# jason-huang03/SPH_Project

Hardware: AMD Instinct MI355X
Metric: particle-updates/sec (higher is better)
Workload: dtype f32

## Files before the change

### sph_project_amd/csrc/sph_api.hip

```cpp
#include "../../include/sph_hip.h"
#include "sph_common.hpp"
#include "sph_comm.hpp"

#include <math.h>
#include <stdarg.h>
#include <stdio.h>
#include <string.h>
#include <string>
#include <vector>
#include <stdlib.h>
#include <utility>
#include <array>
#include <algorithm>
#include "sph_voxel.hpp"
#include "sph_export.hpp"
#include "sph_devobj.hpp"

struct ProfSlot {
    bool on = false;
    int64_t launches = 0;
    double ms = 0.0;
    std::vector<std::pair<hipEvent_t, hipEvent_t>> pending;
};

struct SphHandle : ErrSink {
    SphParams prm = {};
    State st;
    const Launch *L = nullptr;
    int device = 0;
    int n = 0;
    bool n_exact = true;
    int n_fluid = 0;
    int n_nonfluid = 0;
    bool fluid_mass_seen = false, fluid_mass_uniform = true; float fluid_mass0 = 0.0f;
    bool any_rigid_object = false;
    int64_t steps = 0;
    int pbf_bank = 0;
    SphPbfParams pbf = {SPH_PBF_VARIANT_REFERENCE, 1, 50, 1e-3f, 1e-6f};
    SphPbfStats pbf_last = {SPH_PBF_VARIANT_REFERENCE, 0, 0.0f};
    int steps_to_follow = 0;
    bool whole_step = false;
    double total_time = 0.0;
    bool prepared = false;
    bool pose_dirty = false;
    int loop_hint[4] = {0, 0, 0, 0};
    struct LoopPub *loop_pub = nullptr;
    unsigned loop_seq = 0, stats_seq = 0;
    bool loop_flags_clean = false;
    int dev_cus = 256;
    bool pose_given = false;
    bool rigid_volume_done = false;
    bool sort_dirty = false;
    bool in_step = false;
    int n_mark = 0;
    int fresh_state = 0;
    RigidPose pose_h = {};
    RigidBodyDev rb_h[SPH_NOBJ] = {};
    int rb_cap[SPH_NOBJ] = {};
    bool rb_pose_stale = false;
    SphStats last = {};
    ProfSlot prof[SPH_K_COUNT_];
    std::vector<hipEvent_t> ev_pool;
    std::vector<void *> allocs;
    DevScalars *scal_h = nullptr;
    SlabComm comm;
    long long comm_n_global = 0;
    long long comm_nfluid_global = 0;
    int swap_axis = 0;
    int perm[3] = {0, 1, 2};
    int inv[3] = {0, 1, 2};
    float axial = 1.0f;
    int slab_axis = 2;
};

static inline int slab_layers_glob(const Consts &c) { return c.slab_axis == 0 ? c.nx_glob : c.nz_glob; }
static inline void slab_set_window(Consts &c, int z_lo, int z_hi) {
    const int glob = slab_layers_glob(c);
    const int off = z_lo > 0 ? z_lo - 1 : 0;
    const int top = z_hi < glob ? z_hi + 1 : glob;
    if (c.slab_axis == 0) { c.cx_off = off; c.nx = top - off; } else { c.cz_off = off; c.nz = top - off; }
    c.G = c.nx * c.ny * c.nz;
}

static bool set_axis_order(SphHandle *h, const char *order) {
    int p[3], seen = 0;
    for (int k = 0; k < 3; ++k) {
        const char ch = order ? order[k] : 0;
        p[k] = (ch == 'x' || ch == 'X') ? 0 : (ch == 'y' || ch == 'Y') ? 1 : (ch == 'z' || ch == 'Z') ? 2 : -1;
        if (p[k] < 0) return false;
        seen |= 1 << p[k];
    }
    if (seen != 7 || order[3]) return false;
    for (int k = 0; k < 3; ++k) { h->perm[k] = p[k]; h->inv[p[k]] = k; }
    const bool even = (p[0] == 0 && p[1] == 1) || (p[0] == 1 && p[1] == 2) || (p[0] == 2 && p[1] == 0);
    h->axial = even ? 1.0f : -1.0f;
    h->swap_axis = !(p[0] == 0 && p[1] == 1 && p[2] == 2);
    return true;
}

template <class T> static int dalloc(SphHandle *h, T **p, size_t count) {
    void *q = nullptr;
    if (count == 0) count = 1;
    HIPCHK(h, hipMalloc(&q, count * sizeof(T)));
    HIPCHK(h, hipMemset(q, 0, count * sizeof(T)));
    h->allocs.push_back(q);
    *p = (T *)q;
    return SPH_OK;
}

static float host_kernel_W(double hd, float r) {
    float res = 0.0f;
    float k = (float)(8.0 / M_PI);
    k /= (float)(hd * hd * hd);
    float q = r / (float)hd;
    if (q <= 1.0f) {
        if (q <= 0.5f) { float q2 = q * q; float q3 = q2 * q; res = k * (6.0f * q3 - 6.0f * q2 + 1.0f); }
        else res = k * 2.0f * powf(1.0f - q, 3.0f);
    }
    return res;
}

static void fill_consts(SphHandle *h) {
    const SphParams &p = h->prm;
    Consts &c = h->st.c;
    memset(&c, 0, sizeof(c));
    const int *ix = h->perm;
    c.nx = c.nx_glob = p.grid_num[ix[0]]; c.ny = p.grid_num[ix[1]]; c.nz = c.nz_glob = p.grid_num[ix[2]];
    c.cx_off = c.cz_off = 0;
    c.slab_axis = h->slab_axis;
    c.G = c.nx * c.ny * c.nz;
    const double hd = p.support_radius;
    c.grid_size = (float)hd;
    c.h = (float)hd;
    {
        float t = c.h * c.h;
        while (sqrtf(nextafterf(t, 0.0f)) >= c.h) t = nextafterf(t, 0.0f);
        while (sqrtf(t) < c.h) t = nextafterf(t, INFINITY);
        c.h2 = t;
    }
    c.inv_h = 1.0f / c.h;
    float k = (float)(8.0 / M_PI);
    c.kW = k / (float)(hd * hd * hd);
    c.kG = 6.0f * k / (float)(hd * hd * hd);
    c.W0 = host_kernel_W(hd, 0.0f);
    const float d = (float)(2.0 * p.particle_radius);
    c.Wd = host_kernel_W(hd, sqrtf(d * d + 0.0f + 0.0f));
    c.kGh = c.kG * c.inv_h;
    c.inv_h2 = c.inv_h * c.inv_h;
    c.Wd_poly = c.Wd / c.kW;
    const double dd = 2.0 * p.particle_radius;
    c.diameter2 = (float)(dd * dd);
    c.dt = (float)p.dt;
    c.inv_dt = 1.0f / c.dt;
    c.rho0 = (float)p.density_0;
    c.inv_rho0 = 1.0f / c.rho0;
    c.g_upper = (float)p.g_upper;
    c.up_axis = h->inv[1];
    c.gx = (float)p.gravity[ix[0]]; c.gy = (float)p.gravity[ix[1]]; c.gz = (float)p.gravity[ix[2]];
    c.st = (float)p.surface_tension;
    c.cv = (float)(2 * (3 + 2) * p.viscosity);
    c.cvb = (float)(2 * (3 + 2) * p.viscosity_b);
    c.visc_eps = (float)(0.01 * hd * hd);
    c.pad = (float)p.padding;
    c.hix = (float)(p.domain_size[ix[0]] - p.padding);
    c.hiy = (float)(p.domain_size[ix[1]] - p.padding);
    c.hiz = (float)(p.domain_size[ix[2]] - p.padding);
    c.thr_kappa = (float)1e-5 * c.dt;
    c.V0 = (float)p.V0;
    c.force_global = p.force_global;
    c.stat_bank = 0;
    c.run_grouping = 0;
    c.xcd_chunk = 0;
    c.ghosts = 0;
}

static void refresh_counts(SphHandle *h) {
    h->st.c.n = h->n;
    h->st.has_emitter = h->prm.g_upper < 9999.0;
    h->st.c.all_fluid = (h->n_nonfluid == 0 && !h->st.has_emitter && !(h->st.slab_active && h->any_rigid_object)) ? 1 : 0;
    h->st.c.ghosts = h->st.slab_active ? 1 : 0;
    h->st.c.run_grouping = (h->prm.fast_math && !h->st.slab_active && h->st.c.nz >= 40) ? 1 : 0;
    h->st.has_rigid = h->n_nonfluid > 0;
    h->st.uniform_mass = (h->st.c.all_fluid && h->fluid_mass_uniform && !h->st.slab_active && !getenv("SPH_NO_UNIFORM_MASS")) ? 1 : 0;
}

extern "C" const char *sph_last_error(SphHandle *h) { return last_error(h); }

extern "C" const char *sph_kernel_name(int k) {
    static const char *names[SPH_K_COUNT_] = {
        "hash_count", "scan", "scatter", "density", "non_pressure", "pressure_integrate", "rigid_volume",
        "dfsph_density_alpha", "dfsph_rho_adv", "dfsph_correct", "reduce", "pcisph_rho_star",
        "pcisph_pressure_accel", "cg_prepare", "cg_ap", "cg_vector", "misc", "halo", "wcsph_forces",
        "iisph_prepare", "iisph_dij_pj", "iisph_sum_i", "pbf_density_lambda", "pbf_fix_position", "pbf_update",
        "rigid_contact", "rigid_integrate", "rigid_contact_solve", "pbfc_density_lambda", "pbfc_delta"};
    return (k >= 0 && k < SPH_K_COUNT_) ? names[k] : "?";
}

static void slab_comm_destroy(SlabComm &c);
static int slab_settle(SphHandle *h);
static inline int slab_settle_if_needed(SphHandle *h) { return h->n_exact ? SPH_OK : slab_settle(h); }

extern "C" void sph_destroy(SphHandle *h) {
    if (!h) return;
    hipSetDevice(h->device);
    if (h->st.stream) hipStreamSynchronize(h->st.stream);
    slab_comm_destroy(h->comm);
    if (h->st.push.mirror) { hipHostFree(h->st.push.mirror); h->st.push.mirror = nullptr; }
    for (auto &s : h->prof) for (auto &pr : s.pending) { hipEventDestroy(pr.first); hipEventDestroy(pr.second); }
    for (auto e : h->ev_pool) hipEventDestroy(e);
    for (void *p : h->allocs) hipFree(p);
    if (h->scal_h) hipHostFree(h->scal_h);
    if (h->loop_pub) hipHostFree((void *)h->loop_pub);
    if (h->st.list_count_pinned) { hipHostFree((void *)h->st.list_count_pinned); h->st.list_count_pinned = nullptr; }
    if (h->st.list_count_event) { hipEventDestroy(h->st.list_count_event); h->st.list_count_event = nullptr; }
    if (h->st.stream) hipStreamDestroy(h->st.stream);
    delete h;
}

extern "C" int sph_create(const SphParams *params, SphHandle **out) {
    if (!params || !out) return fail(nullptr, SPH_ERR_INVALID, "sph_create: null argument");
    *out = nullptr;
    const SphParams &p = *params;
    if (p.particle_max_num < 0 || p.grid_num[0] <= 0 || p.grid_num[1] <= 0 || p.grid_num[2] <= 0 ||
        !(p.support_radius > 0) || !(p.dt > 0))
        return fail(nullptr, SPH_ERR_INVALID, "sph_create: invalid parameters");
    if ((double)p.grid_num[0] * p.grid_num[1] * p.grid_num[2] > 2.0e9)
        return fail(nullptr, SPH_ERR_INVALID, "sph_create: grid too large");
    if (p.particle_max_num > 0x0fffffff)
        return fail(nullptr, SPH_ERR_CAPACITY, "sph_create: particle_max_num %d exceeds 268435455 per GPU; shard the scene (sph_comm_set_slab)", p.particle_max_num);
    if (p.method < 0 || p.method > SPH_METHOD_PBF) return fail(nullptr, SPH_ERR_INVALID, "sph_create: unknown method %d", p.method);
    int dev = 0;
    { int rc = pick_device("sph_create", p.device, &dev); if (rc) return rc; }
    SphHandle *h = new SphHandle();
    h->prm = p;
    h->device = dev;
    { int cus = 0; if (hipDeviceGetAttribute(&cus, hipDeviceAttributeMultiprocessorCount, dev) == hipSuccess && cus > 0) h->dev_cus = cus; }
#define CHK_CREATE(call)                                                                   \
    do {                                                                                   \
        int rc_ = (call);                                                                  \
        if (rc_ != SPH_OK) { g_create_error = h->err; sph_destroy(h); return rc_; }        \
    } while (0)
#define HIP_CREATE(call)                                                                   \
    do {                                                                                   \
        hipError_t e_ = (call);                                                            \
        if (e_ != hipSuccess) {                                                            \
            fail(nullptr, SPH_ERR_HIP, "%s failed: %s", #call, hipGetErrorString(e_));     \
            sph_destroy(h);                                                                \
            return SPH_ERR_HIP;                                                            \
        }                                                                                  \
    } while (0)
    h->L = p.fast_math ? sph_launch_fast() : sph_launch_strict();
    State &s = h->st;
    HIP_CREATE(hipStreamCreateWithFlags(&s.stream, hipStreamNonBlocking));
    fill_consts(h);
    const size_t cap = (size_t)p.particle_max_num;
    s.cap = p.particle_max_num;
    for (int k = 0; k < 2; ++k) {
        CHK_CREATE(dalloc(h, &s.posv.b[k], cap)); CHK_CREATE(dalloc(h, &s.velm.b[k], cap));
        CHK_CREATE(dalloc(h, &s.meta.b[k], cap)); CHK_CREATE(dalloc(h, &s.pid.b[k], cap));
        CHK_CREATE(dalloc(h, &s.color.b[k], cap)); CHK_CREATE(dalloc(h, &s.rho.b[k], cap));
    }
    const size_t G = (size_t)s.c.G;
    CHK_CREATE(dalloc(h, &s.cell_count, G + SPH_NGRAVE + 1)); CHK_CREATE(dalloc(h, &s.cell_start, G + SPH_NGRAVE + 1));
    CHK_CREATE(dalloc(h, &s.cellid, cap)); CHK_CREATE(dalloc(h, &s.rank, cap)); CHK_CREATE(dalloc(h, &s.tmp_idx, 2 * cap));
    if (h->prm.deterministic && !getenv("SPH_NO_RUN_LISTS")) { CHK_CREATE(dalloc(h, &s.run_head, G + 1)); CHK_CREATE(dalloc(h, &s.run_rec, cap + G + 1)); CHK_CREATE(dalloc(h, &s.sort_inv, cap)); CHK_CREATE(dalloc(h, &s.color_home, cap)); s.color_home_ok = 1; }
    s.scan_blocks = (int)((G + SPH_NGRAVE + 2047) / 2048);
    if (s.scan_blocks < SPH_STAT_SLOTS / 256) s.scan_blocks = SPH_STAT_SLOTS / 256;
    CHK_CREATE(dalloc(h, &s.scan_tile_state, (size_t)s.scan_blocks + 1));
    CHK_CREATE(dalloc(h, &s.scan_partial, 2 * ((size_t)s.scan_blocks + 1) * 8));
    CHK_CREATE(dalloc(h, &s.rho_raw, cap)); CHK_CREATE(dalloc(h, &s.prs, cap)); CHK_CREATE(dalloc(h, &s.ptm, cap));
    CHK_CREATE(dalloc(h, &s.acc, cap));
    CHK_CREATE(dalloc(h, &s.nbr_mask, cap * 9 + 256)); CHK_CREATE(dalloc(h, &s.nbr_mask_hi, cap * 9 + 256));
    CHK_CREATE(dalloc(h, &s.blk_hdr, (cap + 255) / 256 * (20 + 256)));
    if (!getenv("SPH_NO_BLOCK_LIST")) {
        CHK_CREATE(dalloc(h, &s.blk_flag, (cap + 255) / 256)); CHK_CREATE(dalloc(h, &s.blk_list, (cap + 255) / 256)); CHK_CREATE(dalloc(h, &s.blk_count, 1));
    }
    CHK_CREATE(dalloc(h, &s.lane_perm, (cap + 255) / 256 * 256));
    if (p.method == SPH_METHOD_DFSPH) {
        CHK_CREATE(dalloc(h, &s.alpha, cap)); CHK_CREATE(dalloc(h, &s.kappa, cap)); CHK_CREATE(dalloc(h, &s.kappa_v, cap));
        CHK_CREATE(dalloc(h, &s.rho_star, cap)); CHK_CREATE(dalloc(h, &s.rho_deriv, cap)); CHK_CREATE(dalloc(h, &s.kr, cap));
        CHK_CREATE(dalloc(h, &s.kappa_next, cap)); CHK_CREATE(dalloc(h, &s.kappa_v_next, cap));
    }
    if (p.method == SPH_METHOD_PCISPH) {
        CHK_CREATE(dalloc(h, &s.pacc, cap)); CHK_CREATE(dalloc(h, &s.pvel, cap)); CHK_CREATE(dalloc(h, &s.ppos, cap));
        CHK_CREATE(dalloc(h, &s.rho_star, cap)); CHK_CREATE(dalloc(h, &s.acc_np, cap));
        s.np_acc_out = s.acc_np;
    }
    if (p.method == SPH_METHOD_IISPH) {
        CHK_CREATE(dalloc(h, &s.iisph_dii, cap)); CHK_CREATE(dalloc(h, &s.iisph_dij, cap)); CHK_CREATE(dalloc(h, &s.iisph_w, cap));
        CHK_CREATE(dalloc(h, &s.rho_star, cap));
    }
    if (p.method == SPH_METHOD_PBF) {
        CHK_CREATE(dalloc(h, &s.pbf_old, cap)); CHK_CREATE(dalloc(h, &s.pbf_pos, cap)); CHK_CREATE(dalloc(h, &s.pbf_lambda, cap));
        CHK_CREATE(dalloc(h, &s.pbf_recentred, 2));
        s.poly6 = 1;
    }
    if (p.viscosity_implicit) {
        CHK_CREATE(dalloc(h, &s.cg_p, cap)); CHK_CREATE(dalloc(h, &s.cg_Ap, cap)); CHK_CREATE(dalloc(h, &s.cg_x, cap));
        CHK_CREATE(dalloc(h, &s.cg_b, cap)); CHK_CREATE(dalloc(h, &s.cg_r, cap)); CHK_CREATE(dalloc(h, &s.cg_v0, cap));
        CHK_CREATE(dalloc(h, &s.cg_dinv, cap * 9));
        CHK_CREATE(dalloc(h, &s.cg_part, cap * 3));
        CHK_CREATE(dalloc(h, &s.cg_p2, cap));
    }
    s.red_blocks = (int)((cap + 255) / 256) + 1;
    CHK_CREATE(dalloc(h, &s.red_partial, (size_t)s.red_blocks * 8));
    CHK_CREATE(dalloc(h, &s.scal, 1)); CHK_CREATE(dalloc(h, &s.pose, 1));
    HIP_CREATE(hipHostMalloc((void **)&h->scal_h, sizeof(DevScalars), hipHostMallocDefault));
    { void *lp = nullptr; HIP_CREATE(hipHostMalloc(&lp, 128, hipHostMallocDefault)); memset(lp, 0, 128); h->loop_pub = (struct LoopPub *)lp; }
    { int *lc = nullptr; HIP_CREATE(hipHostMalloc((void **)&lc, 64, hipHostMallocDefault)); *lc = 0; s.list_count_pinned = lc; }
    HIP_CREATE(hipEventCreateWithFlags(&s.list_count_event, hipEventDisableTiming));
    memset(h->scal_h, 0, sizeof(DevScalars));
    for (int o = 0; o < SPH_NOBJ; ++o) { h->pose_h.rot[o][0] = h->pose_h.rot[o][4] = h->pose_h.rot[o][8] = 1.0f; }
    s.z_hi = slab_layers_glob(s.c);
    s.visc_rho_raw = (p.method == SPH_METHOD_WCSPH);
    refresh_counts(h);
    *out = h;
    return SPH_OK;
}

static int ensure_orig(SphHandle *h) {
    State &s = h->st;
    if (!s.orig.b[0]) {
        int rc = dalloc(h, &s.orig.b[0], (size_t)s.cap); if (rc) return rc;
        rc = dalloc(h, &s.orig.b[1], (size_t)s.cap); if (rc) return rc;
        HIPCHK(h, hipMemcpyAsync(s.orig.cur(), s.posv.cur(), sizeof(float4) * (size_t)h->n, hipMemcpyDeviceToDevice, s.stream));
    }
    s.has_dynamic_rigid = 1;
    return SPH_OK;
}

extern "C" int sph_append_particles(SphHandle *h, int object_id, int n, const float *pos, const float *vel,
                                    const float *density, const float *pressure, const int32_t *material,
                                    const int32_t *is_dynamic, const int32_t *color) {
    if (!h) return SPH_ERR_INVALID;
    if (n < 0 || object_id < -1 || object_id >= SPH_MAX_OBJECTS) return fail(h, SPH_ERR_INVALID, "append: bad object id / count");
    if (n == 0) return SPH_OK;
    if (!pos || !vel || !density || !material || !is_dynamic) return fail(h, SPH_ERR_INVALID, "append: null array");
    { int rc = slab_settle_if_needed(h); if (rc) return rc; }
    if (h->n + n > h->st.cap) return fail(h, SPH_ERR_CAPACITY, "append: %d + %d exceeds particle_max_num %d", h->n, n, h->st.cap);
    HIPCHK(h, hipSetDevice(h->device));
    State &s = h->st;
    const float V0 = (float)h->prm.V0;
    std::vector<float4> hp(n), hv(n), ho;
    std::vector<int> hm(n), hid(n);
    std::vector<unsigned> hc(n);
    std::vector<float> hr(n), hpr(n);
    bool any_dyn_rigid = false;
    int nfl = 0;
    const int ix0 = h->perm[0], ix1 = h->perm[1], ix2 = h->perm[2];
    for (int k = 0; k < n; ++k) {
        hp[k] = make_float4(pos[3 * k + ix0], pos[3 * k + ix1], pos[3 * k + ix2], V0);
        hv[k] = make_float4(vel[3 * k + ix0], vel[3 * k + ix1], vel[3 * k + ix2], V0 * density[k]);
        hm[k] = META_PACK(object_id, material[k], is_dynamic[k] ? 1 : 0);
        if (h->prepared && material[k] == SPH_MAT_RIGID) { hm[k] |= META_FRESH_BIT; h->fresh_state = 1; }
        hid[k] = h->n + k;
        unsigned r = color ? (unsigned)(color[3 * k] & 0xff) : 0, g = color ? (unsigned)(color[3 * k + 1] & 0xff) : 0,
                 b = color ? (unsigned)(color[3 * k + 2] & 0xff) : 0;
        hc[k] = r | (g << 8) | (b << 16);
        hr[k] = density[k];
        hpr[k] = pressure ? pressure[k] : 0.0f;
        if (material[k] == SPH_MAT_FLUID) {
            nfl++;
            if (!h->fluid_mass_seen) { h->fluid_mass_seen = true; h->fluid_mass0 = hv[k].w; }
            else if (hv[k].w != h->fluid_mass0) h->fluid_mass_uniform = false;
        }
        if (material[k] == SPH_MAT_RIGID && is_dynamic[k]) any_dyn_rigid = true;
    }
    if (any_dyn_rigid) { int rc = ensure_orig(h); if (rc) return rc; }
    HIPCHK(h, hipStreamSynchronize(s.stream));
    const size_t off = (size_t)h->n;
    HIPCHK(h, hipMemcpy(s.posv.cur() + off, hp.data(), sizeof(float4) * n, hipMemcpyHostToDevice));
    HIPCHK(h, hipMemcpy(s.velm.cur() + off, hv.data(), sizeof(float4) * n, hipMemcpyHostToDevice));
    HIPCHK(h, hipMemcpy(s.meta.cur() + off, hm.data(), sizeof(int) * n, hipMemcpyHostToDevice));
    HIPCHK(h, hipMemcpy(s.pid.cur() + off, hid.data(), sizeof(int) * n, hipMemcpyHostToDevice));
    HIPCHK(h, hipMemcpy(s.color.cur() + off, hc.data(), sizeof(unsigned) * n, hipMemcpyHostToDevice));
    if (s.color_home) HIPCHK(h, hipMemcpy(s.color_home + off, hc.data(), sizeof(unsigned) * n, hipMemcpyHostToDevice));
    HIPCHK(h, hipMemcpy(s.rho.cur() + off, hr.data(), sizeof(float) * n, hipMemcpyHostToDevice));
    HIPCHK(h, hipMemcpy(s.prs + off, hpr.data(), sizeof(float) * n, hipMemcpyHostToDevice));
    if (s.orig.cur()) HIPCHK(h, hipMemcpy(s.orig.cur() + off, hp.data(), sizeof(float4) * n, hipMemcpyHostToDevice));
    h->n += n;
    h->n_fluid += nfl;
    h->n_nonfluid += n - nfl;
    if (!h->prepared) h->rigid_volume_done = false;
    if (h->prepared) h->sort_dirty = true;
    s.masks_valid = 0;
    s.perm_n = -1; s.list_n = -1;
    refresh_counts(h);
    return SPH_OK;
}

static void colors_leave_home(SphHandle *h) { h->L->sorted_color(h->st); h->st.color_home_ok = 0; }

extern "C" int sph_set_appended_ids(SphHandle *h, int n, const int32_t *ids) {
// ... 255 lines not shown
    const int m = std::min(n, capacity);
    if (m == 0) return SPH_OK;
    std::vector<double> dev((size_t)m * SPH_CS_ROW);
    HIPCHK(h, hipMemcpyAsync(dev.data(), s.contact_rows, dev.size() * sizeof(double), hipMemcpyDeviceToHost, s.stream));
    HIPCHK(h, hipStreamSynchronize(s.stream));
    for (int r = 0; r < m; ++r)
        memcpy(rows + (size_t)r * SPH_CONTACT_ROW_VALUES, dev.data() + (size_t)r * SPH_CS_ROW, sizeof(double) * SPH_CONTACT_ROW_VALUES);
    return SPH_OK;
}

static void contact_to_scene(const SphHandle *h, const unsigned long long *dev, double *out) {
    const size_t row = SPH_CT_VALUES;
    for (int A = 0; A < SPH_NOBJ; ++A)
        for (int B = 0; B < SPH_CT_PARTNERS; ++B)
            for (int b = 0; b < SPH_CT_BINS; ++b) {
                const int bs = 2 * h->perm[b / 2] + (b & 1);
                const int Bs = B >= 20 ? 20 + (2 * h->perm[(B - 20) / 2] + ((B - 20) & 1)) : B;
                const long long *v = (const long long *)dev + ((size_t)(A * SPH_CT_PARTNERS + B) * SPH_CT_BINS + b) * row;
                double *o = out + ((size_t)(A * SPH_CT_PARTNERS + Bs) * SPH_CT_BINS + bs) * row;
                o[0] = (double)v[0];
                for (int a = 0; a < 3; ++a) {
                    o[1 + a] = (double)v[1 + h->inv[a]] / SPH_WRENCH_SCALE;
                    o[4 + a] = (double)v[4 + h->inv[a]] / SPH_WRENCH_SCALE;
                }
                o[7] = (double)(unsigned long long)v[7] / SPH_WRENCH_SCALE;
            }
}

extern "C" int sph_get_rigid_contacts(SphHandle *h, double *table, int reset) {
    if (!h || !table) return fail(h, SPH_ERR_INVALID, "get_rigid_contacts: null");
    State &s = h->st;
    const size_t words = (size_t)SPH_CT_KEYS * SPH_CT_VALUES;
    if (!s.contact_table) return fail(h, SPH_ERR_INVALID, "get_rigid_contacts: sph_set_rigid_contact was never enabled");
    HIPCHK(h, hipSetDevice(h->device));
    std::vector<unsigned long long> dev(words);
    HIPCHK(h, hipMemcpyAsync(dev.data(), s.contact_table, words * 8, hipMemcpyDeviceToHost, s.stream));
    HIPCHK(h, hipStreamSynchronize(s.stream));
    contact_to_scene(h, dev.data(), table);
    if (s.slab_active && h->comm.nranks > 1) {
        if (h->comm.nranks > 15) return fail(h, SPH_ERR_UNSUPPORTED, "get_rigid_contacts: more than 15 ranks");
        const int per = 12, nd = (SPH_CT_KEYS + per - 1) / per;
        std::vector<double> dig(nd, 0.0);
        for (int k = 0; k < SPH_CT_KEYS; ++k) if (table[(size_t)k * 8] > 0.0) dig[k / per] += (double)(1ll << (4 * (k % per)));
        for (int o = 0; o < nd; o += SHM_RED_MAX) { int rc = sph_comm_allreduce(h, dig.data() + o, std::min(SHM_RED_MAX, nd - o), 0); if (rc) return rc; }
        std::vector<int> keys;
        for (int k = 0; k < SPH_CT_KEYS; ++k) if (((long long)dig[k / per] >> (4 * (k % per))) & 15) keys.push_back(k);
        std::vector<double> sum(keys.size() * 7), mx(keys.size());
        for (size_t q = 0; q < keys.size(); ++q) {
            for (int v = 0; v < 7; ++v) sum[7 * q + v] = table[(size_t)keys[q] * 8 + v];
            mx[q] = table[(size_t)keys[q] * 8 + 7];
        }
        for (size_t o = 0; o < sum.size(); o += SHM_RED_MAX) { int rc = sph_comm_allreduce(h, sum.data() + o, (int)std::min((size_t)SHM_RED_MAX, sum.size() - o), 0); if (rc) return rc; }
        for (size_t o = 0; o < mx.size(); o += SHM_RED_MAX) { int rc = sph_comm_allreduce(h, mx.data() + o, (int)std::min((size_t)SHM_RED_MAX, mx.size() - o), 1); if (rc) return rc; }
        for (size_t q = 0; q < keys.size(); ++q) {
            for (int v = 0; v < 7; ++v) table[(size_t)keys[q] * 8 + v] = sum[7 * q + v];
            table[(size_t)keys[q] * 8 + 7] = mx[q];
        }
    }
    if (reset) HIPCHK(h, hipMemsetAsync(s.contact_table, 0, words * 8, s.stream));
    return SPH_OK;
}

extern "C" int sph_get_rigid_contact_pairs(SphHandle *h, int64_t *pairs) {
    if (!h || !pairs) return fail(h, SPH_ERR_INVALID, "get_rigid_contact_pairs: null");
    *pairs = 0;
    if (!h->st.contact_pairs) return SPH_OK;
    HIPCHK(h, hipSetDevice(h->device));
    unsigned long long r = 0;
    HIPCHK(h, hipMemcpyAsync(&r, h->st.contact_pairs, sizeof(r), hipMemcpyDeviceToHost, h->st.stream));
    HIPCHK(h, hipStreamSynchronize(h->st.stream));
    *pairs = (int64_t)r;
    return SPH_OK;
}

static hipEvent_t get_event(SphHandle *h) {
    if (!h->ev_pool.empty()) { hipEvent_t e = h->ev_pool.back(); h->ev_pool.pop_back(); return e; }
    hipEvent_t e;
    hipEventCreate(&e);
    return e;
}

static void prof_resolve(SphHandle *h) {
    hipStreamSynchronize(h->st.stream);
    for (auto &s : h->prof) {
        for (auto &pr : s.pending) {
            float ms = 0.0f;
            if (hipEventElapsedTime(&ms, pr.first, pr.second) == hipSuccess) { s.ms += ms; s.launches++; }
            h->ev_pool.push_back(pr.first); h->ev_pool.push_back(pr.second);
        }
        s.pending.clear();
    }
}

struct ProfScope {
    SphHandle *h; int k; hipEvent_t e1 = nullptr;
    ProfScope(SphHandle *h_, int k_) : h(h_), k(k_) {
        if (h->prof[k].on) {
            if (h->prof[k].pending.size() > 8192) prof_resolve(h);
            hipEvent_t e0 = get_event(h); e1 = get_event(h);
            hipEventRecord(e0, h->st.stream);
            h->prof[k].pending.push_back({e0, e1});
        }
    }
    ~ProfScope() { if (e1) hipEventRecord(e1, h->st.stream); }
};

extern "C" int sph_profile_enable(SphHandle *h, int kernel_id, int on) {
    if (!h || kernel_id >= SPH_K_COUNT_) return SPH_ERR_INVALID;
    for (int k = 0; k < SPH_K_COUNT_; ++k) if (kernel_id < 0 || kernel_id == k) h->prof[k].on = on != 0;
    return SPH_OK;
}
extern "C" int sph_profile_reset(SphHandle *h) {
    if (!h) return SPH_ERR_INVALID;
    hipSetDevice(h->device);
    prof_resolve(h);
    for (auto &s : h->prof) { s.launches = 0; s.ms = 0.0; }
    return SPH_OK;
}
extern "C" int sph_profile_read(SphHandle *h, int kernel_id, int64_t *launches, double *total_ms) {
    if (!h || kernel_id < 0 || kernel_id >= SPH_K_COUNT_) return SPH_ERR_INVALID;
    hipSetDevice(h->device);
    prof_resolve(h);
    if (launches) *launches = h->prof[kernel_id].launches;
    if (total_ms) *total_ms = h->prof[kernel_id].ms;
    return SPH_OK;
}

extern "C" int sph_device_info(SphHandle *h, char *name256, int *cu_count, int64_t *hbm_bytes) {
    if (!h) return SPH_ERR_INVALID;
    hipDeviceProp_t prop;
    HIPCHK(h, hipGetDeviceProperties(&prop, h->device));
    if (name256) { if (prop.name[0]) snprintf(name256, 256, "%s (%s)", prop.name, prop.gcnArchName); else snprintf(name256, 256, "%s, %d CUs", prop.gcnArchName, prop.multiProcessorCount); }
    if (cu_count) *cu_count = prop.multiProcessorCount;
    if (hbm_bytes) *hbm_bytes = (int64_t)prop.totalGlobalMem;
    return SPH_OK;
}

extern "C" int sph_measure_copy_rate(SphHandle *h, size_t bytes, int reps, double *gb_per_s) {
    if (!h || !gb_per_s || bytes < 4096 || reps < 1) return fail(h, SPH_ERR_INVALID, "measure_copy_rate: bad arguments");
    HIPCHK(h, hipSetDevice(h->device));
    void *a = nullptr, *b = nullptr;
    if (hipMalloc(&a, bytes) != hipSuccess || hipMalloc(&b, bytes) != hipSuccess) {
        if (a) hipFree(a);
        return fail(h, SPH_ERR_HIP, "measure_copy_rate: cannot allocate 2 x %zu bytes", bytes);
    }
    hipStream_t st = h->st.stream;
    hipEvent_t e0 = get_event(h), e1 = get_event(h);
    hipError_t e = hipMemsetAsync(a, 1, bytes, st);
    if (e == hipSuccess) e = hipMemcpyAsync(b, a, bytes, hipMemcpyDeviceToDevice, st);
    if (e == hipSuccess) e = hipEventRecord(e0, st);
    for (int k = 0; k < reps && e == hipSuccess; ++k) e = hipMemcpyAsync((k & 1) ? a : b, (k & 1) ? b : a, bytes, hipMemcpyDeviceToDevice, st);
    if (e == hipSuccess) e = hipEventRecord(e1, st);
    if (e == hipSuccess) e = hipStreamSynchronize(st);
    float ms = 0.0f;
    if (e == hipSuccess) e = hipEventElapsedTime(&ms, e0, e1);
    h->ev_pool.push_back(e0); h->ev_pool.push_back(e1);
    hipFree(a); hipFree(b);
    if (e != hipSuccess || !(ms > 0.0f)) return fail(h, SPH_ERR_HIP, "measure_copy_rate: %s", hipGetErrorString(e));
    *gb_per_s = 2.0 * (double)bytes * reps / ((double)ms * 1e-3) / 1e9;
    return SPH_OK;
}

static int check_async(SphHandle *h) {
    if (h->st.state_error) { const int se = h->st.state_error; h->st.state_error = 0; return fail(h, SPH_ERR_INVALID, "internal state error %d (bit 0: a sort was scanned without a histogram of its own; bit 1: a density launch could not move the arrays its sort left to it)", se); }
    hipError_t e = hipGetLastError();
    if (e != hipSuccess) return fail(h, SPH_ERR_HIP, "kernel launch failed: %s", hipGetErrorString(e));
    return SPH_OK;
}

static SortCarry ph_neighbor_search(SphHandle *h, bool rho_dead = false, bool density_next = false) {
    State &s = h->st;
    SortCarry carry;
    { ProfScope p(h, SPH_K_HASH_COUNT); h->L->hash_count(s); }
    { ProfScope p(h, SPH_K_SCAN); h->L->scan(s); }
    { ProfScope p(h, SPH_K_SCATTER); if (h->prm.deterministic) carry = h->L->scatter_stable(s, rho_dead, density_next && !getenv("SPH_NO_SORT_CARRY")); else h->L->scatter(s); }
    h->sort_dirty = false;
    return carry;
}

static void ph_sort_hashed(SphHandle *h) {
    State &s = h->st;
    { ProfScope p(h, SPH_K_SCAN); h->L->scan(s); }
    { ProfScope p(h, SPH_K_SCATTER); if (h->prm.deterministic) h->L->scatter_stable(s, false, false); else h->L->scatter(s); }
    h->sort_dirty = false;
}

static void ph_rigid_volume(SphHandle *h) {
    if (!h->st.has_rigid) return;
    bool force = false;
    if (h->fresh_state == 2) { h->L->clear_fresh(h->st); h->fresh_state = 0; force = true; }
    else if (h->fresh_state == 1 && h->prm.method != SPH_METHOD_DFSPH) h->fresh_state = 2;
    if (!force && h->rigid_volume_done && !h->st.has_dynamic_rigid) return;
    ProfScope p(h, SPH_K_RIGID_VOLUME);
    h->L->rigid_volume(h->st);
    h->rigid_volume_done = true;
}

static void step_begin(SphHandle *h) {
    State &s = h->st;
    s.c.stat_bank = (int)(h->steps & 1);
}

#include "sph_comm_api.hpp"
#include "sph_steps.hpp"

static int read_scalars(SphHandle *h) {
    { int rc = slab_settle_if_needed(h); if (rc) return rc; }
    if (h->loop_pub) {
        StatsPub *pub = (StatsPub *)((char *)h->loop_pub + 64);
        const unsigned want = ++h->stats_seq;
        const int bank_d = h->steps > 0 ? (int)((h->steps - 1) & 1) : 0;
        hipLaunchKernelGGL(k_publish_stats, dim3(1), dim3(256), 0, h->st.stream, h->st.scal, bank_d, pub, want);
        if (spin_for(h->st, &pub->seq, want)) {
            h->last.pair_interactions = (int64_t)pub->pairs;
            h->last.pair_evaluations = (int64_t)pub->evals;
            h->last.lds_fallback_blocks = (int64_t)pub->fallback;
            return SPH_OK;
        }
    }
    HIPCHK(h, hipMemcpyAsync(h->scal_h, h->st.scal, sizeof(DevScalars), hipMemcpyDeviceToHost, h->st.stream));
    HIPCHK(h, hipStreamSynchronize(h->st.stream));
    unsigned long long pairs = 0, evals = 0, fb = 0;
    const int bank = h->steps > 0 ? (int)((h->steps - 1) & 1) : 0;
    for (int k = 0; k < SPH_STAT_SLOTS; ++k) {
        pairs += h->scal_h->pairs[bank][k]; evals += h->scal_h->evals[bank][k];
        fb += h->scal_h->fallback[bank][k];
    }
    h->last.pair_interactions = (int64_t)pairs;
    h->last.pair_evaluations = (int64_t)evals;
    h->last.lds_fallback_blocks = (int64_t)fb;
    return SPH_OK;
}

static int finish_sync(SphHandle *h) {
    { int rc = slab_settle_if_needed(h); if (rc) return rc; }
    HIPCHK(h, hipStreamSynchronize(h->st.stream));
    return SPH_OK;
}

extern "C" int sph_prepare(SphHandle *h) {
    if (!h) return SPH_ERR_INVALID;
    HIPCHK(h, hipSetDevice(h->device));
    refresh_counts(h);
    State &s = h->st;
    if (s.slab_active && h->prm.method == SPH_METHOD_IISPH)
        return fail(h, SPH_ERR_UNSUPPORTED, "sph_prepare: IISPH runs on one GPU only (no sharded IISPH solve: sph_comm_set_slab)");
    if (s.slab_active && h->prm.method == SPH_METHOD_PBF)
        return fail(h, SPH_ERR_UNSUPPORTED, "sph_prepare: PBF runs on one GPU only (no sharded PBF step: sph_comm_set_slab)");
    if (h->prm.viscosity_implicit && h->prm.method == SPH_METHOD_PBF)
        return fail(h, SPH_ERR_UNSUPPORTED, "sph_prepare: PBF with implicit viscosity is not supported (its CG walks would need the spiky gradient)");
    int rc = pose_refresh(h); if (rc) return rc;
    rc = upload_pose(h); if (rc) return rc;
    { ProfScope p(h, SPH_K_MISC); h->L->prepare_emitter(s); h->L->renew_rigid(s); }
    h->pose_dirty = false;
    if (s.slab_active) {
        double n_own[2] = {(double)h->n, (double)h->n_fluid};
        rc = sph_comm_allreduce(h, n_own, 2, 0); if (rc) return rc;
        h->comm_n_global = (long long)n_own[0];
        h->comm_nfluid_global = (long long)n_own[1];
        double dyn_rigid[1] = {s.orig.cur() ? 1.0 : 0.0};
        rc = sph_comm_allreduce(h, dyn_rigid, 1, 1); if (rc) return rc;
        if (dyn_rigid[0] > 0.0 && !s.orig.cur()) { rc = ensure_orig(h); if (rc) return rc; }
        rc = slab_neighbor_search(h); if (rc) return rc;
    }
    else ph_neighbor_search(h);
    h->rigid_volume_done = false;
    ph_rigid_volume(h);
    if (s.slab_active && s.has_rigid) {
        rc = slab_neighbor_search(h); if (rc) return rc;
    }
    rc = method_prepare(h); if (rc) return rc;
    HIPCHK(h, hipMemsetAsync(s.scal, 0, sizeof(unsigned long long) * SPH_STAT_SLOTS, s.stream));
    HIPCHK(h, hipMemsetAsync((char *)s.scal + offsetof(DevScalars, evals), 0, sizeof(unsigned long long) * SPH_STAT_SLOTS, s.stream));
    HIPCHK(h, hipMemsetAsync((char *)s.scal + offsetof(DevScalars, fallback), 0, sizeof(unsigned long long) * SPH_STAT_SLOTS, s.stream));
    rc = check_async(h); if (rc) return rc;
    HIPCHK(h, hipStreamSynchronize(s.stream));
    h->prepared = true;
    return SPH_OK;
}

static void ph_rigid_integrate(SphHandle *h) {
    if (!h->st.rigid_int_on || h->st.rigid_int.nbodies <= 0) return;
    if (h->st.contact_solve_on) { ProfScope p(h, SPH_K_RIGID_CONTACT_SOLVE); h->L->rigid_contact_solve(h->st); }
    else { ProfScope p(h, SPH_K_RIGID_INTEGRATE); h->L->rigid_integrate(h->st); }
    h->pose_dirty = true;
    h->rb_pose_stale = true;
}

extern "C" int sph_rigid_integrate(SphHandle *h) {
    if (!h) return SPH_ERR_INVALID;
    if (!h->in_step) return fail(h, SPH_ERR_INVALID, "sph_rigid_integrate outside sph_step_begin / sph_step_end");
    if (!h->st.rigid_int_on) return fail(h, SPH_ERR_INVALID, "sph_rigid_integrate: sph_set_rigid_integrator is off");
    { int rc = rigid_int_supported(h, "sph_rigid_integrate"); if (rc) return rc; }
    HIPCHK(h, hipSetDevice(h->device));
    ph_rigid_integrate(h);
    return check_async(h);
}

static int step_first_half(SphHandle *h) {
    if (h->in_step) return fail(h, SPH_ERR_INVALID, "sph_step_begin: the previous step was not ended");
    step_begin(h);
    int rc;
    switch (h->prm.method) {
        case SPH_METHOD_WCSPH: rc = wcsph_step(h); break;
        case SPH_METHOD_DFSPH: rc = dfsph_step_begin(h); break;
        case SPH_METHOD_IISPH: rc = iisph_step(h); break;
        case SPH_METHOD_PBF:
            rc = h->pbf.variant == SPH_PBF_VARIANT_CONSISTENT ? pbfc_step(h) : pbf_step(h); break;
        default: rc = pcisph_step(h); break;
    }
    if (rc) return rc;
    if (h->st.contact_on) { ProfScope p(h, SPH_K_RIGID_CONTACT); h->L->rigid_contact(h->st); }
    h->n_mark = h->n;
    h->in_step = true;
    return SPH_OK;
}

static int step_second_half(SphHandle *h) {
    if (!h->in_step) return fail(h, SPH_ERR_INVALID, "sph_step_end without sph_step_begin");
    State &s = h->st;
    h->in_step = false;
    if (h->pose_dirty || h->fresh_state || h->prm.method != SPH_METHOD_WCSPH) { int rc = slab_settle_if_needed(h); if (rc) return rc; }
    if (h->pose_dirty) { ProfScope p(h, SPH_K_MISC); h->L->renew_rigid(s); h->pose_dirty = false; }
    if (h->n > h->n_mark) {
        ProfScope p(h, SPH_K_MISC);
        h->L->post_insert(s, h->n_mark, h->prm.method != SPH_METHOD_DFSPH);
    }
    if (h->prm.method == SPH_METHOD_DFSPH) {
        int rc = dfsph_step_end(h); if (rc) return rc;
        if (h->fresh_state == 1) { h->fresh_state = 2; ph_rigid_volume(h); }
    } else if (h->fresh_state == 2) {
        ph_rigid_volume(h);
    }
    h->total_time += (double)s.c.dt;
    h->steps++;
    return SPH_OK;
}

static int step_once(SphHandle *h) {
    h->whole_step = true;
    int rc = step_first_half(h);
    h->whole_step = false;
#ifdef SPH_TEST_HOOKS
    {
        static int fail_at = getenv("SPH_TEST_FAIL_STEP") ? atoi(getenv("SPH_TEST_FAIL_STEP")) : -1;
        if (!rc && fail_at >= 0 && h->steps == fail_at) { fail_at = -1; h->in_step = false; rc = fail(h, SPH_ERR_INVALID, "SPH_TEST_FAIL_STEP: injected failure"); }
    }
#endif
    if (!rc) ph_rigid_integrate(h);
    if (!rc) rc = step_second_half(h);
    if (rc && h->st.prehashed) { h->st.prehashed = 0; h->st.cell_count_clean = 0; h->st.hist_taken = 0; h->st.run_lists_filed = 0; }
    return rc;
}

extern "C" int sph_step_begin(SphHandle *h) {
    if (!h) return SPH_ERR_INVALID;
    if (!h->prepared) return fail(h, SPH_ERR_INVALID, "sph_step_begin before sph_prepare");
    HIPCHK(h, hipSetDevice(h->device));
    refresh_counts(h);
    int rc = step_first_half(h); if (rc) return rc;
    rc = slab_settle_if_needed(h); if (rc) return rc;
    h->n_mark = h->n;
    return check_async(h);
}

extern "C" int sph_step_end(SphHandle *h) {
    if (!h) return SPH_ERR_INVALID;
    HIPCHK(h, hipSetDevice(h->device));
    refresh_counts(h);
    int rc = step_second_half(h); if (rc) return rc;
    rc = check_async(h); if (rc) return rc;
    return finish_sync(h);
}

extern "C" int sph_step_async(SphHandle *h, int nsteps) {
    if (!h || nsteps < 0) return SPH_ERR_INVALID;
    if (!h->prepared) return fail(h, SPH_ERR_INVALID, "sph_step before sph_prepare");
    if (h->prm.method != SPH_METHOD_WCSPH && h->prm.method != SPH_METHOD_PBF && h->prm.fixed_iterations <= 0)
        return fail(h, SPH_ERR_UNSUPPORTED, "sph_step_async needs wcsph, pbf or fixed_iterations > 0");
    if (h->prm.method == SPH_METHOD_PBF && h->pbf.variant == SPH_PBF_VARIANT_CONSISTENT && h->prm.fixed_iterations <= 0)
        return fail(h, SPH_ERR_UNSUPPORTED, "sph_step_async: the consistent PBF variant needs fixed_iterations > 0 (its stop test reads back)");
    HIPCHK(h, hipSetDevice(h->device));
    refresh_counts(h);
    for (int k = 0; k < nsteps; ++k) {
        h->steps_to_follow = nsteps - 1 - k;
        int rc = step_once(h);
        h->steps_to_follow = 0;
        if (rc) return rc;
    }
    return check_async(h);
}

extern "C" int sph_synchronize(SphHandle *h) {
    if (!h) return SPH_ERR_INVALID;
    HIPCHK(h, hipSetDevice(h->device));
    if (!h->n_exact) return slab_settle(h);
    return loop_readback(h);
}

extern "C" int sph_step(SphHandle *h, int nsteps) {
    if (!h || nsteps < 0) return SPH_ERR_INVALID;
    if (!h->prepared) return fail(h, SPH_ERR_INVALID, "sph_step before sph_prepare");
    HIPCHK(h, hipSetDevice(h->device));
    refresh_counts(h);
    for (int k = 0; k < nsteps; ++k) { int rc = step_once(h); if (rc) return rc; }
    int rc = check_async(h); if (rc) return rc;
    return finish_sync(h);
}

extern "C" int sph_run_phase(SphHandle *h, int phase) {
    if (!h) return SPH_ERR_INVALID;
    HIPCHK(h, hipSetDevice(h->device));
    { int rc = slab_settle_if_needed(h); if (rc) return rc; }
    refresh_counts(h);
    State &s = h->st;
    switch (phase) {
        case SPH_PH_NEIGHBOR_SEARCH: ph_neighbor_search(h); break;
        case SPH_PH_RIGID_VOLUME: h->rigid_volume_done = false; ph_rigid_volume(h); break;
        case SPH_PH_DENSITY: { ProfScope p(h, SPH_K_DENSITY); h->L->density(s, h->prm.method == SPH_METHOD_WCSPH, {}); } break;
        case SPH_PH_NON_PRESSURE: { int rc = run_non_pressure(h); if (rc) return rc; } break;
        case SPH_PH_PRESSURE_INTEGRATE: { ProfScope p(h, SPH_K_PRESSURE_INTEGRATE); h->L->pressure_integrate(s); } break;
        case SPH_PH_RIGID_CONTACT: {
            if (!s.contact_on) return fail(h, SPH_ERR_INVALID, "SPH_PH_RIGID_CONTACT: sph_set_rigid_contact is off");
            HIPCHK(h, hipMemsetAsync(s.contact_part, 0, sizeof(float4) * (size_t)s.cap, s.stream));
            ProfScope p(h, SPH_K_RIGID_CONTACT); h->L->rigid_contact(s);
        } break;
        case SPH_PH_CG_PREPARE: case SPH_PH_CG_AP: case SPH_PH_CG_UPDATE_XR: case SPH_PH_CG_UPDATE_P: case SPH_PH_CG_END:
            { int rc = cg_run_phase(h, phase); if (rc) return rc; } break;
        default: { int rc = method_run_phase(h, phase); if (rc) return rc; }
    }
    int rc = check_async(h); if (rc) return rc;
    HIPCHK(h, hipStreamSynchronize(s.stream));
    return SPH_OK;
}

extern "C" int sph_particle_num(SphHandle *h) {
    if (!h) return SPH_ERR_INVALID;
    if (!h->n_exact) { hipSetDevice(h->device); const int rc = slab_settle(h); if (rc) return rc; }
    return h->n;
}
extern "C" int sph_fluid_particle_num(SphHandle *h) { return h ? h->n_fluid : SPH_ERR_INVALID; }

extern "C" int sph_get_stats(SphHandle *h, SphStats *out) {
    if (!h || !out) return SPH_ERR_INVALID;
    HIPCHK(h, hipSetDevice(h->device));
    int rc = read_scalars(h); if (rc) return rc;
    h->last.steps = h->steps;
    h->last.particle_num = h->n;
    h->last.fluid_particle_num = h->n_fluid;
    h->last.total_time = h->total_time;
    h->last.hash_launches = h->st.n_hash_launches;
    h->last.prehashed_sorts = h->st.n_prehashed_sorts;
    h->last.list_sorts = h->st.n_list_sorts;
    h->last.carried_sorts = h->st.n_carried_sorts;
    if (h->st.pbf_recentred) {
        unsigned long long r[2];
        HIPCHK(h, hipMemcpy(r, h->st.pbf_recentred, sizeof(r), hipMemcpyDeviceToHost));
        h->last.pbf_recentred = (int64_t)r[h->pbf_bank];
    }
    *out = h->last;
    return SPH_OK;
}

extern "C" int sph_get_cg_scalars(SphHandle *h, float *out) {
    if (!h || !out) return SPH_ERR_INVALID;
    if (!h->prm.viscosity_implicit) return fail(h, SPH_ERR_UNSUPPORTED, "sph_get_cg_scalars: no implicit viscosity on this handle");
    HIPCHK(h, hipSetDevice(h->device));
    State &s = h->st;
    HIPCHK(h, hipStreamSynchronize(s.stream));
    float red[8];
    HIPCHK(h, hipMemcpy(red, &s.scal->red[0], sizeof(red), hipMemcpyDeviceToHost));
    out[0] = red[4]; out[1] = red[5]; out[2] = red[3];
    return SPH_OK;
}

static const float4 *vec_field(SphHandle *h, int field) {
    State &s = h->st;
    switch (field) {
        case SPH_F_POSITION: case SPH_F_REST_VOLUME: return s.posv.cur();
        case SPH_F_VELOCITY: case SPH_F_MASS: return s.velm.cur();
        case SPH_F_ACCELERATION: return s.acc;
        case SPH_F_PRESSURE_ACCEL: return s.pacc;
        case SPH_F_PREDICTED_VEL: return s.pvel;
        case SPH_F_PREDICTED_POS: return h->pbf.variant == SPH_PBF_VARIANT_CONSISTENT ? s.pbf_old : s.ppos;
        case SPH_F_CG_X: return s.cg_x;
        case SPH_F_ORIG_POSITION: return s.orig.cur() ? s.orig.cur() : s.posv.cur();
        case SPH_F_IISPH_DII: case SPH_F_IISPH_AII: return s.iisph_dii;
        case SPH_F_IISPH_DIJ_PJ: case SPH_F_IISPH_SUM_I: return s.iisph_dij;
        case SPH_F_PBF_OLD_POSITION: return h->pbf.variant == SPH_PBF_VARIANT_CONSISTENT ? nullptr : s.pbf_old;
        case SPH_F_RIGID_CONTACT_DN: case SPH_F_RIGID_CONTACT_COUNT: return s.contact_part;
        case SPH_F_NON_PRESSURE_ACCEL: return s.acc_np;
        case SPH_F_CG_B: return s.cg_b;
        case SPH_F_CG_R: return s.cg_r;
        case SPH_F_CG_P: return s.cg_p;
        case SPH_F_CG_AP: return s.cg_Ap;
        case SPH_F_CG_V0: return s.cg_v0;
        default: return nullptr;
    }
}
static const float *scalar_field(SphHandle *h, int field) {
    State &s = h->st;
    switch (field) {
        case SPH_F_DENSITY: return s.rho.cur();
        case SPH_F_PRESSURE: return s.prs;
        case SPH_F_DFSPH_ALPHA: return s.alpha;
        case SPH_F_DFSPH_KAPPA: return s.kappa;
        case SPH_F_DFSPH_KAPPA_V: return s.kappa_v;
        case SPH_F_DENSITY_STAR: return s.rho_star;
        case SPH_F_DENSITY_DERIV: return s.rho_deriv;
        case SPH_F_DFSPH_KAPPA_NEXT: return s.kappa_next;
        case SPH_F_DFSPH_KAPPA_V_NEXT: return s.kappa_v_next;
        case SPH_F_DEBUG_CAPTURE: return s.rho_raw;
        case SPH_F_PBF_LAMBDA: return s.pbf_lambda;
        default: return nullptr;
    }
}

extern "C" int sph_download(SphHandle *h, int field, void *dst, size_t bytes) {
    if (!h || !dst) return SPH_ERR_INVALID;
    HIPCHK(h, hipSetDevice(h->device));
    { int rc = slab_settle_if_needed(h); if (rc) return rc; }
    State &s = h->st;
    const size_t n = (size_t)h->n;
    HIPCHK(h, hipStreamSynchronize(s.stream));
    const bool is_vec3 = field == SPH_F_POSITION || field == SPH_F_VELOCITY || field == SPH_F_ACCELERATION ||
                         field == SPH_F_PRESSURE_ACCEL || field == SPH_F_PREDICTED_VEL || field == SPH_F_PREDICTED_POS ||
                         field == SPH_F_CG_X || field == SPH_F_ORIG_POSITION || field == SPH_F_IISPH_DII || field == SPH_F_IISPH_DIJ_PJ ||
                         field == SPH_F_PBF_OLD_POSITION || field == SPH_F_RIGID_CONTACT_DN || field == SPH_F_NON_PRESSURE_ACCEL ||
                         (field >= SPH_F_CG_B && field <= SPH_F_CG_V0);
    if (is_vec3) {
        const float4 *src = vec_field(h, field);
        if (!src) return fail(h, SPH_ERR_UNSUPPORTED, "download: field %d not allocated for this method", field);
        if (bytes != n * 12) return fail(h, SPH_ERR_INVALID, "download: field %d needs %zu bytes, got %zu", field, n * 12, bytes);
        std::vector<float4> tmp(n);
        HIPCHK(h, hipMemcpy(tmp.data(), src, n * sizeof(float4), hipMemcpyDeviceToHost));
        float *d = (float *)dst;
        const int ix0 = h->inv[0], ix1 = h->inv[1], ix2 = h->inv[2];
        for (size_t i = 0; i < n; ++i) { const float v[3] = {tmp[i].x, tmp[i].y, tmp[i].z}; d[3 * i] = v[ix0]; d[3 * i + 1] = v[ix1]; d[3 * i + 2] = v[ix2]; }
        return SPH_OK;
    }
    if (field == SPH_F_CG_DINV) {
        if (!s.cg_dinv) return fail(h, SPH_ERR_UNSUPPORTED, "download: field %d not allocated for this method", field);
        if (bytes != n * 36) return fail(h, SPH_ERR_INVALID, "download: field %d needs %zu bytes, got %zu", field, n * 36, bytes);
        std::vector<float> tmp(n * 9);
        HIPCHK(h, hipMemcpy(tmp.data(), s.cg_dinv, n * 36, hipMemcpyDeviceToHost));
        float *d = (float *)dst;
        for (size_t i = 0; i < n; ++i)
            for (int a = 0; a < 3; ++a)
                for (int b = 0; b < 3; ++b) d[9 * i + 3 * a + b] = tmp[9 * i + 3 * h->inv[a] + h->inv[b]];
        return SPH_OK;
    }
    if (field == SPH_F_CG_AP_PARTS) {
        if (!s.cg_part) return fail(h, SPH_ERR_UNSUPPORTED, "download: field %d not allocated for this method", field);
        if (bytes != n * 36) return fail(h, SPH_ERR_INVALID, "download: field %d needs %zu bytes, got %zu", field, n * 36, bytes);
        std::vector<float4> tmp(n);
        float *d = (float *)dst;
        const int ix0 = h->inv[0], ix1 = h->inv[1], ix2 = h->inv[2];
        for (int g = 0; g < 3; ++g) {
            HIPCHK(h, hipMemcpy(tmp.data(), s.cg_part + (size_t)g * s.cap, n * sizeof(float4), hipMemcpyDeviceToHost));
            float *dg = d + (size_t)g * n * 3;
            for (size_t i = 0; i < n; ++i) { const float v[3] = {tmp[i].x, tmp[i].y, tmp[i].z}; dg[3 * i] = v[ix0]; dg[3 * i + 1] = v[ix1]; dg[3 * i + 2] = v[ix2]; }
        }
        return SPH_OK;
    }
    if (field == SPH_F_REST_VOLUME || field == SPH_F_MASS || field == SPH_F_IISPH_AII || field == SPH_F_IISPH_SUM_I ||
        field == SPH_F_RIGID_CONTACT_COUNT) {
        if (bytes != n * 4) return fail(h, SPH_ERR_INVALID, "download: size mismatch");
        const float4 *src = vec_field(h, field);
        if (!src) return fail(h, SPH_ERR_UNSUPPORTED, "download: field %d not allocated for this method", field);
        std::vector<float4> tmp(n);
        HIPCHK(h, hipMemcpy(tmp.data(), src, n * sizeof(float4), hipMemcpyDeviceToHost));
        float *d = (float *)dst;
        for (size_t i = 0; i < n; ++i) d[i] = tmp[i].w;
        return SPH_OK;
    }
    if (const float *src = scalar_field(h, field)) {
        if (bytes != n * 4) return fail(h, SPH_ERR_INVALID, "download: size mismatch");
        HIPCHK(h, hipMemcpy(dst, src, n * 4, hipMemcpyDeviceToHost));
        return SPH_OK;
    }
    if (field == SPH_F_MATERIAL || field == SPH_F_OBJECT_ID || field == SPH_F_IS_DYNAMIC || field == SPH_F_GHOST) {
        if (bytes != n * 4) return fail(h, SPH_ERR_INVALID, "download: size mismatch");
        std::vector<int> tmp(n);
        HIPCHK(h, hipMemcpy(tmp.data(), s.meta.cur(), n * 4, hipMemcpyDeviceToHost));
        int32_t *d = (int32_t *)dst;
        for (size_t i = 0; i < n; ++i)
            d[i] = field == SPH_F_MATERIAL ? META_MAT(tmp[i]) : field == SPH_F_OBJECT_ID ? META_OBJ(tmp[i]) :
                   field == SPH_F_GHOST ? META_GHOST(tmp[i]) : META_DYN(tmp[i]);
        return SPH_OK;
    }
    if (field == SPH_F_PARTICLE_ID) {
        if (bytes != n * 4) return fail(h, SPH_ERR_INVALID, "download: size mismatch");
        HIPCHK(h, hipMemcpy(dst, s.pid.cur(), n * 4, hipMemcpyDeviceToHost));
        return SPH_OK;
    }
    if (field == SPH_F_COLOR) {
        if (bytes != n * 12) return fail(h, SPH_ERR_INVALID, "download: size mismatch");
        const unsigned *col = h->L->sorted_color(s); HIPCHK(h, hipStreamSynchronize(s.stream));
        std::vector<unsigned> tmp(n);
        HIPCHK(h, hipMemcpy(tmp.data(), col, n * 4, hipMemcpyDeviceToHost));
        int32_t *d = (int32_t *)dst;
        for (size_t i = 0; i < n; ++i) { d[3 * i] = tmp[i] & 0xff; d[3 * i + 1] = (tmp[i] >> 8) & 0xff; d[3 * i + 2] = (tmp[i] >> 16) & 0xff; }
        return SPH_OK;
    }
    if (field == SPH_F_GRID_ID) {
        if (bytes != n * 4) return fail(h, SPH_ERR_INVALID, "download: size mismatch");
        std::vector<float4> tmp(n);
// ... 112 lines not shown
```

### sph_project_amd/csrc/sph_common.hpp

```cpp
#pragma once
#include <hip/hip_runtime.h>
#include <stdint.h>

#define SPH_NOBJ 20
#define SPH_IISPH_OMEGA 0.2f
#define SPH_IISPH_ETA 0.001
#define SPH_IISPH_MAX_ITER 20
#define SPH_PBF_LAMBDA_EPS 100.0f
#define SPH_PBF_CORR_K 0.001f
#define SPH_PBF_CORR_DQ 0.3f
#define SPH_PBF_ITERATIONS 5

#define META_OBJ(m) (((m) & 0xff) - 1)
#define META_MAT(m) (((m) >> 8) & 0x3)
#define META_DYN(m) (((m) >> 10) & 0x1)
#define META_PACK(obj, mat, dyn) ((((obj) + 1) & 0xff) | (((mat) & 0x3) << 8) | (((dyn) & 1) << 10))
#define META_GHOST(m) (((m) >> 11) & 0x1)
#define META_DEAD(m) (((m) >> 12) & 0x1)
#define META_FRESH(m) (((m) >> 13) & 0x1)
#define META_FRESH_BIT (1 << 13)
#define META_ACTIVE_FLUID(m) ((((m) >> 8) & 0xB) == 1)
#define META_SET_MAT(m, mat) (((m) & ~(0x3 << 8)) | (((mat) & 0x3) << 8))

struct Consts {
    int nx, ny, nz, G;
    int nx_glob, cx_off, nz_glob, cz_off, slab_axis;
    float grid_size;
    float h, h2, inv_h;
    float kW, kG;
    float kGh, Wd_poly;
    float inv_h2;
    float W0, Wd;
    float diameter2;
    float dt, inv_dt, rho0, inv_rho0, g_upper;
    int up_axis;
    float gx, gy, gz;
    float st;
    float cv, cvb, visc_eps;
    float pad, hix, hiy, hiz;
    float thr_kappa;
    float V0;
    float pcisph_k;
    int   n;
    int   all_fluid;
    int   force_global;
    int   ghosts;
    int   stat_bank;
    int   xcd_chunk;
    int   run_grouping;
    const int *n_dev;
};

__device__ __forceinline__ int live_n(const Consts &c) { return c.n_dev ? *c.n_dev : c.n; }

#define SPH_NGRAVE 64
#define HC(k) ((k) * 32)
#define HC_BANK 128
struct SlabDyn {
    int n_app;
    int n_live;
    int n_send[2];
    int n_recv[2];
    int dropped;
    int longest;
    int status;
    unsigned seq;
    int n_btiles;
    unsigned wseq;
};
struct HaloRecHdr {
    unsigned seq;
    int count, status, stride;
};
struct HaloCtl {
    HaloRecHdr rec[2];
    unsigned fld_seq;
    int pad[55];
};
static_assert(sizeof(HaloCtl) == 256, "HaloCtl layout");
#define SLAB_ST_SEND_OVERFLOW 1
#define SLAB_ST_PEER 2
#define SLAB_ST_STRIDE 4
#define SLAB_ST_CAPACITY 8
#define SLAB_ST_TIMEOUT 16
#define SLAB_ST_BOUND 32
// ... 214 lines not shown
#define PNG_SEG 4096
#define PNG_NCNT 14
#define PNG_SIDE 320
#define PNG_WSIDE 672
#define PNG_WINDOW 32768
#define PNG_FAR 4096
#define PNG_NONE 0xFFFFFFFFu
#define PNG_SORT_TILE 4096
#define PNG_ND 5
#define PNG_DIST_LIST {1, 2, 3, 4, 6}
#define PNG_CRC_PIECE 17
static_assert(256 * PNG_CRC_PIECE >= 4 + 2 + 5 + PNG_SEG, "the CRC pieces cover the longest chunk");
#define PNG_CRC_POLY 0xEDB88320u
__host__ __device__ static inline unsigned png_crc_mul(unsigned a, unsigned b) {
    unsigned p = 0u;
    for (int k = 0; k < 32; ++k) {
        if (a & (0x80000000u >> k)) p ^= b;
        b = (b >> 1) ^ (PNG_CRC_POLY & (0u - (b & 1u)));
    }
    return p;
}
struct PngDev {
    int W, H, filter;
    int stride, raw, nseg;
    const unsigned char *rgb;
    unsigned char *flt;
    int *len;
    unsigned *adler;
    unsigned long long *cnt;
    unsigned *sum;
    unsigned crc_pow[8];
    unsigned char *out;
    hipStream_t stream;
    unsigned char *side;
    unsigned *prev;
    unsigned *sort_key[2], *sort_pos[2];
    int *hist;
    int nsort;
};

struct TextDev {
    int kind;
    const unsigned *xyz;
    const unsigned *nrm;
    const int *tri;
    long long nv, nt;
    long long row0;
    int rows;
    int *len;
    int *scan_tmp;
    int *longest;
    unsigned char *out;
    hipStream_t stream;
};

template <class T> struct DBuf {
    T *b[2] = {nullptr, nullptr};
    int c = 0;
    T *cur() const { return b[c]; }
    T *alt() const { return b[1 - c]; }
    void flip() { c = 1 - c; }
};

struct State {
    Consts c = {};
    hipStream_t stream = nullptr;
    int cap = 0;
    DBuf<float4> posv, velm, orig;
    DBuf<int> meta, pid;
    DBuf<unsigned> color;
    DBuf<float> rho;
    int *cell_count = nullptr;
    int *cell_start = nullptr;
    int *cellid = nullptr, *rank = nullptr;
    unsigned long long *run_head = nullptr;
    int2 *run_rec = nullptr;
    unsigned sort_epoch = 0u;
    int run_lists_filed = 0;
    int *sort_inv = nullptr;
    long long n_list_sorts = 0;
    long long n_carried_sorts = 0;
    unsigned *color_home = nullptr;
    int color_home_ok = 0, color_stale = 0;
    int *tmp_idx = nullptr;
    int *scan_partial = nullptr;
    int scan_blocks = 0;
    int *scan_tile_state = nullptr;
    int scan_bank = 0;
    int skip_residual = 0;
    int tile_sums_ready = 0;
    int cell_count_clean = 1;
    int hist_taken = 0;
    int state_error = 0;
    float *rho_raw = nullptr, *prs = nullptr, *ptm = nullptr;
    float4 *acc = nullptr;
    float *alpha = nullptr, *kappa = nullptr, *kappa_v = nullptr, *rho_star = nullptr, *rho_deriv = nullptr;
    float *kappa_next = nullptr, *kappa_v_next = nullptr;
    float2 *kr = nullptr;
    float4 *pacc = nullptr, *pvel = nullptr, *ppos = nullptr, *acc_np = nullptr;
    float4 *iisph_dii = nullptr, *iisph_dij = nullptr, *iisph_w = nullptr;
    float4 *pbf_old = nullptr, *pbf_pos = nullptr; float *pbf_lambda = nullptr; unsigned long long *pbf_recentred = nullptr;
    int poly6 = 0;
    float pbf_eps = 1e-6f;
    int contact_on = 0;
    ContactArgs contact = {};
    unsigned long long *contact_table = nullptr, *contact_pairs = nullptr;
    float4 *contact_part = nullptr;
    int rigid_int_on = 0;
    RigidIntArgs rigid_int = {};
    RigidBodyDev *rigid_bodies = nullptr;
    int contact_solve_on = 0;
    ContactSolveArgs contact_solve = {};
    double *contact_rows = nullptr;
    int *contact_nrows = nullptr;
    float4 *cg_p = nullptr, *cg_Ap = nullptr, *cg_x = nullptr, *cg_b = nullptr, *cg_r = nullptr, *cg_v0 = nullptr;
    float4 *cg_p2 = nullptr;
    int cg_fused_loop = 0;
    float *cg_dinv = nullptr;
    float4 *cg_part = nullptr;
    int cg_nocombine = 0;
    int cg_split = 0;
    int cg_parity = 0;
    int cg_first = 1;
    float *red_partial = nullptr;
    int red_blocks = 0;
    DevScalars *scal = nullptr;
    RigidPose *pose = nullptr;
    int has_dynamic_rigid = 0;
    int has_rigid = 0;
    int *xidx[2] = {};
    int xcur = 0;
    int *halo_tab[8] = {};
    float4 *sendbuf[2] = {}, *recvbuf[2] = {};
    int *halo_counts = nullptr;
    SlabDyn *dyn = nullptr;
    SlabDyn *dyn_cur = nullptr;
    int tables_pending = 0;
    int async_counts = 0;
    struct PushState {
        int on = 0;
        char *inbox = nullptr;
        char *peer[2] = {};
        int rec_cap = 0;
        size_t rec_bytes = 0, fld_bytes = 0;
        unsigned rec_seq = 0, fld_seq = 0;
        long long timeout_ticks = 0;
        SlabDyn *mirror = nullptr;
    } push;
    int *tile_list[2] = {};
    int *tile_cnt = nullptr;
    unsigned char *tile_class = nullptr;
    int tile_plan_n = -1;
    int tile_bound_b = 0;
    HaloSend presend = {};
    HaloFieldSend fieldsend = {};
    int preclassified = 0;
    int prehashed = 0;
    long long n_hash_launches = 0, n_prehashed_sorts = 0;
    int halo_cap = 0;
    int halo_longest = 0;
    int slab_active = 0, z_lo = 0, z_hi = 0, has_down = 0, has_up = 0;
    unsigned *nbr_mask = nullptr;
    unsigned *nbr_mask_hi = nullptr;
    int masks_valid = 0;
    int uniform_mass = 0;
    const int *loop_flag = nullptr;
    int loop_slot = 0;
    int loop_kind = 0;
    float loop_denom = 1.0f; double loop_thr = 0.0;
    unsigned char *lane_perm = nullptr;
    int *blk_flag = nullptr, *blk_list = nullptr, *blk_count = nullptr;
    int list_n = -1;
    volatile int *list_count_pinned = nullptr;
    hipEvent_t list_count_event = nullptr;
    int list_count_known = -1;
    int last_pass_listed = 0;
    int *blk_hdr = nullptr;
    int perm_n = -1;
    int has_emitter = 0;
    int visc_rho_raw = 0;
    int skip_viscosity = 0;
    float4 *np_acc_out = nullptr;
};

struct SortCarry {
    const int *inv = nullptr;
    const float4 *velm_in = nullptr; float4 *velm_out = nullptr;
    const int *meta_in = nullptr; int *meta_out = nullptr;
    const int *pid_in = nullptr; int *pid_out = nullptr;
    int on = 0;
};
template <bool ON> struct SortCarryOf { SortCarry carry; };
template <> struct SortCarryOf<false> {};

struct DensityOpts {
    int tiles = 0;
    bool books_forces = false;
    SortCarry carry = {};
};
struct ForceOpts {
    bool booked_by_density = false;
    bool hash_next = false;
};

struct Launch {
    unsigned *(*sorted_color)(State &);
    void (*hash_count)(State &);
    void (*scan)(State &);
    void (*scatter)(State &);
    SortCarry (*scatter_stable)(State &, bool rho_dead, bool density_next);
    void (*density)(State &, int eos, DensityOpts o);
    void (*non_pressure)(State &, const float4 *visc_vel);
    void (*pressure_integrate)(State &);
    void (*wcsph_forces)(State &, ForceOpts o);
    void (*rigid_volume)(State &);
    void (*renew_rigid)(State &);
    void (*prepare_emitter)(State &);
    void (*post_insert)(State &, int first, int stale_volume);
    void (*clear_fresh)(State &);
    void (*dfsph_density_alpha)(State &);
    void (*dfsph_density_alpha_div)(State &);
    void (*dfsph_rho_adv)(State &, int mode);
    void (*dfsph_correct)(State &, int mode);
    void (*advect_boundary)(State &, bool hash_next);
    void (*pcisph_init)(State &);
    void (*pcisph_rho_star)(State &);
    void (*pcisph_pressure_accel)(State &);
    void (*pcisph_reduce_error)(State &);
    void (*iisph_prepare)(State &);
    void (*iisph_dij_pj)(State &);
    void (*iisph_sum_i)(State &);
    void (*pbf_predict)(State &);
    void (*pbf_density_lambda)(State &);
    void (*pbf_fix_position)(State &);
    void (*pbf_finish)(State &);
    void (*pbfc_predict)(State &);
    void (*pbfc_density_lambda)(State &, int reduce);
    void (*pbfc_delta)(State &, int reduce);
    void (*pbfc_finish)(State &);
    void (*rigid_contact)(State &);
    void (*rigid_integrate)(State &);
    void (*rigid_contact_solve)(State &);
    void (*halo_classify_pack)(State &, int n);
    void (*halo_unpack_append)(State &, int side, int count, int offset);
    void (*halo_build_tables)(State &);
    void (*halo_pack_fields)(State &, int side, int n_send, int n_recv);
    void (*halo_unpack_fields)(State &, int side, int n_recv, int n_send);
    void (*halo_pack_scalar)(State &, int side, int n_send, int n_recv, const float *src);
    void (*halo_unpack_scalar)(State &, int side, int n_recv, int n_send, float *dst);
    void (*halo_pack_vel)(State &, int side, int n_send, int n_recv, const float4 *arr);
    void (*halo_unpack_vel)(State &, int side, int n_recv, int n_send, float4 *arr);
    void (*count_ghosts)(State &, int *out);
    void (*surf_compact)(SurfDev &, const float4 *posv, const int *meta, int n, int object_id);
    void (*surf_bounds)(SurfDev &);
    void (*surf_bin)(SurfDev &);
    void (*surf_flags)(SurfDev &);
    void (*surf_field)(SurfDev &);
    void (*surf_count)(SurfDev &);
    void (*surf_emit)(SurfDev &);
    void (*surf_normals)(SurfDev &, int nv);
    void (*surf_aniso_moments)(SurfDev &, SurfAniso &);
    void (*surf_aniso_volume)(SurfDev &, SurfAniso &);
    void (*surf_field_aniso)(SurfDev &, SurfAniso &);
    void (*surf_normals_aniso)(SurfDev &, SurfAniso &, int nv);
    void (*surf_post_adjacency)(SurfDev &, SurfPost &);
    void (*surf_post_compact)(SurfDev &, SurfPost &);
    void (*surf_post_weights)(SurfDev &, SurfPost &);
    void (*surf_post_smooth)(SurfDev &, SurfPost &, int iters);
    void (*surf_post_nsmooth)(SurfDev &, SurfPost &, int iters);
    void (*render_splat)(RenderDev &);
    void (*render_shade)(RenderDev &);
    void (*render_merge)(RenderDev &, const unsigned long long *, const unsigned char *);
    void (*render_finish)(RenderDev &);
    void (*render_surface_base)(RenderDev &, RenderSurfDev &);
    void (*render_surface_quantise)(RenderDev &, RenderSurfDev &);
    void (*render_surface_smooth)(RenderDev &, RenderSurfDev &, int it);
    void (*render_surface_shade)(RenderDev &, RenderSurfDev &, int plane);
    void (*render_thick_opaque)(RenderDev &, RenderSurfDev &, RenderThickDev &);
    void (*render_thick_splat)(RenderDev &, RenderSurfDev &, RenderThickDev &);
    void (*render_thick_smooth)(RenderDev &, RenderSurfDev &, RenderThickDev &, const unsigned *Q, const unsigned *in, unsigned *out);
    void (*render_thick_shade)(RenderDev &, RenderSurfDev &, RenderThickDev &, const unsigned *Q, const unsigned *T);
    void (*render_foam_splat)(RenderDev &, RenderSurfDev &, RenderFoamDev &);
    void (*render_foam_under)(RenderDev &, RenderSurfDev &, RenderThickDev &, RenderFoamDev &, const unsigned *Q, const unsigned *T);
    void (*render_foam_over)(RenderDev &, RenderFoamDev &);
    void (*render_mesh_depth)(RenderDev &, MeshDev &);
    void (*render_mesh_shade)(RenderDev &, MeshDev &);
    void (*render_mesh_finish)(RenderDev &);
    void (*video_count)(VideoDev &);
    void (*video_scan)(VideoDev &);
    void (*video_write)(VideoDev &);
    void (*png_filter)(PngDev &);
    void (*png_candidates)(PngDev &);
    void (*png_count)(PngDev &);
// ... 36 lines not shown
```

### sph_project_amd/csrc/sph_device.hpp

```cpp
#pragma once
#include "sph_common.hpp"
#include <limits.h>

#ifndef SPH_FAST
#define SPH_FAST 0
#endif

__device__ __forceinline__ float fdiv(float a, float b) {
#if SPH_FAST
    return a * __builtin_amdgcn_rcpf(b);
#else
    return a / b;
#endif
}
__device__ __forceinline__ float fdiv2(float a, float b, float c) {
#if SPH_FAST
    return a * __builtin_amdgcn_rcpf(b * c);
#else
    return (a / b) / c;
#endif
}
__device__ __forceinline__ float fsqrt(float a) {
#if SPH_FAST
    return __builtin_amdgcn_sqrtf(a);
// ... 383 lines not shown
            const unsigned long long hd = rl.head[cell];
            int p = (unsigned)(hd >> 32) == rl.epoch ? (int)(unsigned)(hd & 0xffffffffull) : -1;
            for (int hops = 0; p >= 0 && hops < e - s; ++hops) {
                const int2 rec = rl.rec[p];
                r0 += p < i ? rec.y : 0;
                p = rec.x;
            }
        }
        d0 = s + r0;
    }
    d0 = __shfl(d0, hl, 64);
    if (valid) inv[d0 + (lane - hl)] = i;
}

#define NBR_PAD 40
typedef float v2f __attribute__((ext_vector_type(2)));
template <int ZW_OFF>
__device__ __forceinline__ void lds_load_chunk_imm(unsigned a, v2f (&xy)[8], float (&z)[8]) {
    asm volatile(
        "ds_read_b64 %0, %16\n\tds_read_b32 %8, %16 offset:%17\n\t"
        "ds_read_b64 %1, %16 offset:8\n\tds_read_b32 %9, %16 offset:%17+8\n\t"
        "ds_read_b64 %2, %16 offset:16\n\tds_read_b32 %10, %16 offset:%17+16\n\t"
        "ds_read_b64 %3, %16 offset:24\n\tds_read_b32 %11, %16 offset:%17+24\n\t"
        "ds_read_b64 %4, %16 offset:32\n\tds_read_b32 %12, %16 offset:%17+32\n\t"
        "ds_read_b64 %5, %16 offset:40\n\tds_read_b32 %13, %16 offset:%17+40\n\t"
        "ds_read_b64 %6, %16 offset:48\n\tds_read_b32 %14, %16 offset:%17+48\n\t"
        "ds_read_b64 %7, %16 offset:56\n\tds_read_b32 %15, %16 offset:%17+56\n\t"
        "s_waitcnt lgkmcnt(0)"
        : "=&v"(xy[0]), "=&v"(xy[1]), "=&v"(xy[2]), "=&v"(xy[3]), "=&v"(xy[4]), "=&v"(xy[5]), "=&v"(xy[6]), "=&v"(xy[7]),
          "=&v"(z[0]), "=&v"(z[1]), "=&v"(z[2]), "=&v"(z[3]), "=&v"(z[4]), "=&v"(z[5]), "=&v"(z[6]), "=&v"(z[7])
        : "v"(a), "n"(ZW_OFF)
        : "memory");
}
template <int ZW_OFF>
__device__ __forceinline__ void lds_load_half_imm(unsigned a, v2f (&xy)[4], float (&z)[4]) {
    asm volatile(
        "ds_read_b64 %0, %8\n\tds_read_b32 %4, %8 offset:%9\n\t"
        "ds_read_b64 %1, %8 offset:8\n\tds_read_b32 %5, %8 offset:%9+8\n\t"
        "ds_read_b64 %2, %8 offset:16\n\tds_read_b32 %6, %8 offset:%9+16\n\t"
        "ds_read_b64 %3, %8 offset:24\n\tds_read_b32 %7, %8 offset:%9+24\n\t"
        "s_waitcnt lgkmcnt(0)"
        : "=&v"(xy[0]), "=&v"(xy[1]), "=&v"(xy[2]), "=&v"(xy[3]), "=&v"(z[0]), "=&v"(z[1]), "=&v"(z[2]), "=&v"(z[3])
        : "v"(a), "n"(ZW_OFF)
        : "memory");
}
constexpr int SPH_P1_CHUNK = 4;
constexpr int SPH_P1_TRIP = 4;
typedef __attribute__((address_space(3))) const unsigned long long lds_cu64;
typedef __attribute__((address_space(3))) const int lds_ci32;
__device__ __forceinline__ int lds_ld_i32(const int *p) { return *(lds_ci32 *)p; }
typedef __attribute__((address_space(3))) const unsigned short lds_cu16;
__device__ __forceinline__ int lds_ld_u16(const unsigned short *p) { return (int)*(lds_cu16 *)p; }
__device__ __forceinline__ unsigned lds_addr(const float2 *p) { return (unsigned)(size_t)(lds_cu64 *)p; }
__device__ __forceinline__ float2 lds_ld2a(unsigned byte_addr) {
    const unsigned long long v = *(lds_cu64 *)(size_t)byte_addr;
    return make_float2(__uint_as_float((unsigned)v), __uint_as_float((unsigned)(v >> 32)));
}
template <class P, class = void> struct PassFluidOnly { static constexpr bool value = false; };
template <class P> struct PassFluidOnly<P, decltype((void)P::FLUID_BLOCKS_ONLY)> { static constexpr bool value = P::FLUID_BLOCKS_ONLY; };

template <class P, class = void> struct PassSplit { static constexpr bool value = false; };
template <class P> struct PassSplit<P, decltype((void)P::SPLIT3)> { static constexpr bool value = P::SPLIT3; };

template <class P, class = void> struct PassModes { static constexpr int value = 0b101; };
template <class P> struct PassModes<P, decltype((void)P::MODES)> { static constexpr int value = P::MODES; };
template <class P> constexpr bool pass_builds_masks() { return (PassModes<P>::value & 0b010) != 0; }
template <class P> constexpr bool pass_reuses_masks() { return (PassModes<P>::value & 0b100) != 0; }

template <class P, class = void> struct PassMaskPipe { static constexpr bool value = true; };
template <class P> struct PassMaskPipe<P, decltype((void)P::MASK_PIPELINE)> { static constexpr bool value = P::MASK_PIPELINE; };
template <class P, class = void> struct PassUsesJ0 { static constexpr bool value = true; };
template <class P> struct PassUsesJ0<P, decltype((void)P::USES_J)> { static constexpr bool value = P::USES_J; };
template <class P> constexpr bool pass_mask_pipe() { return PassMaskPipe<P>::value && !(P::HAS_B && PassUsesJ0<P>::value); }
template <class P, class = void> struct PassWrench { static constexpr bool value = false; };
template <class P> struct PassWrench<P, decltype((void)P::HAS_WRENCH)> { static constexpr bool value = P::HAS_WRENCH; };
__device__ __forceinline__ void wrench_init_all(const RigidPose *pose);
__device__ __forceinline__ void wrench_flush_all(DevScalars *scal);
template <class P, class = void> struct PassStatW { static constexpr bool value = false; };
template <class P> struct PassStatW<P, decltype((void)P::STAT_W)> { static constexpr bool value = P::STAT_W; };
template <class P, class = void> struct PassNextHash { static constexpr bool value = false; };
template <class P> struct PassNextHash<P, decltype((void)P::NEXT_HASH)> { static constexpr bool value = P::NEXT_HASH; };
template <class P, class = void> struct PassSortCarry { static constexpr bool value = false; };
template <class P> struct PassSortCarry<P, decltype((void)P::SORT_CARRY)> { static constexpr bool value = P::SORT_CARRY; };
template <class P, class = void> struct PassPrologue { static constexpr bool value = false; };
template <class P> struct PassPrologue<P, decltype((void)P::HAS_PROLOGUE)> { static constexpr bool value = P::HAS_PROLOGUE; };

template <class P, class = void> struct PassC { static constexpr bool value = false; typedef int type; };
template <class P> struct PassC<P, decltype((void)P::HAS_C)> { static constexpr bool value = P::HAS_C; typedef typename P::CT type; };

template <class P>
__device__ __forceinline__ float4 pass_stage(const P &p, const Consts &c, int j, typename P::BT &bj, typename PassC<P>::type &cj) {
    if constexpr (PassC<P>::value) return p.stage(c, j, bj, cj);
    else return p.stage(c, j, bj);
}
template <class P>
__device__ __forceinline__ void pass_pair(const P &p, const Consts &c, typename P::Own &own, float dx, float dy, float dz,
                                          float r2, const float4 &a, const typename P::BT &bj,
                                          const typename PassC<P>::type &cj, int j) {
    if constexpr (PassC<P>::value) p.pair(c, own, dx, dy, dz, r2, a, bj, cj, j);
    else p.pair(c, own, dx, dy, dz, r2, a, bj, j);
}


template <int ZW_OFF, bool LEAN = false>
__device__ __forceinline__ unsigned phase1_mask(const float2 *sXY, int base, int m, float xi, float yi, float zi,
                                                float h2) {
    if (LEAN) {
        unsigned nm = 0;
        const unsigned tile = lds_addr(&sXY[base]);
#pragma unroll 1
        for (int t = 0; __any(t < m); ++t) {
            const float2 xy = lds_ld2a(tile + 8u * t), zw = lds_ld2a(tile + 8u * t + ZW_OFF);
            const float dx = xi - xy.x, dy = yi - xy.y, dz = zi - zw.x;
            const float r2 = dx * dx + dy * dy + dz * dz;
            nm |= (t < m && r2 < h2) ? 1u << t : 0u;
        }
        return nm;
    }
    unsigned mask = 0;
    int S = 0;
    int t0 = 0;
    do {
        if constexpr (SPH_P1_CHUNK == 8) {
            v2f xy[8];
            float zz[8];
            lds_load_chunk_imm<ZW_OFF>(lds_addr(&sXY[base + t0]), xy, zz);
#pragma unroll
            for (int u = 0; u < 8; ++u) {
                const float dx = xi - xy[u].x, dy = yi - xy[u].y, dz = zi - zz[u];
                const float r2 = dx * dx + dy * dy + dz * dz;
                asm("v_cmp_gt_f32 vcc, %2, %1\n\tv_addc_co_u32 %0, vcc, %0, %0, vcc"
                    : "+v"(mask) : "v"(r2), "s"(h2) : "vcc");
            }
        } else {
#pragma unroll
            for (int hh = 0; hh < SPH_P1_TRIP / 4; ++hh) {
                v2f xy[4];
                float zz[4];
                lds_load_half_imm<ZW_OFF>(lds_addr(&sXY[base + t0 + 4 * hh]), xy, zz);
#pragma unroll
                for (int u = 0; u < 4; ++u) {
                    const float dx = xi - xy[u].x, dy = yi - xy[u].y, dz = zi - zz[u];
                    const float r2 = dx * dx + dy * dy + dz * dz;
                    asm("v_cmp_gt_f32 vcc, %2, %1\n\tv_addc_co_u32 %0, vcc, %0, %0, vcc"
                        : "+v"(mask) : "v"(r2), "s"(h2) : "vcc");
                }
            }
        }
        t0 += SPH_P1_CHUNK == 8 ? 8 : SPH_P1_TRIP;
    } while (__any(t0 < m));
    S = t0;
    unsigned nm = S > 0 ? __brev(mask) >> (32 - S) : 0u;
    nm &= m >= 32 ? 0xffffffffu : ((1u << m) - 1u);
    return nm;
}

template <int ZW_OFF, int MASKMODE, class P>
__device__ __forceinline__ void process_chunk(const Consts &c, const P &p, typename P::Own &own, int i, float xi, float yi, float zi,
                                              int js, int je, int cs, int ce, const float2 *sXY, const float2 *sZW,
                                              const typename P::BT *sB, const typename PassC<P>::type *sC, unsigned &npairs,
                                              unsigned long long &w01) {
    const int lo = js > cs ? js : cs, hi = je < ce ? je : ce;
    int k = lo > js ? (lo - js) >> 5 : 0;
    for (; __any(lo < hi && js + 32 * k < hi); ++k) {
        const int b0r = js + 32 * k;
        const int b0 = b0r > lo ? b0r : lo;
// ... 22 lines not shown
    }
}

constexpr bool SPH_P2_PAIR2_MEDIUM = true;
template <class P> constexpr bool pass_is_medium();
template <class P> constexpr bool pass_pair2() {
    return SPH_P2_PAIR2_MEDIUM && pass_is_medium<P>();
}

template <class P, class = void> struct PassUsesJ { static constexpr bool value = true; };
template <class P> struct PassUsesJ<P, decltype((void)P::USES_J)> { static constexpr bool value = P::USES_J; };

template <class P, int ZW_OFF, class M>
__device__ __forceinline__ void merged_phase2(const Consts &c, const P &p, typename P::Own &own, float xi, float yi,
                                              float zi, M m0, M m1, M m2, unsigned a0,
                                              unsigned a1, unsigned a2, const float2 *sXY,
                                              const typename P::BT *sB, const typename PassC<P>::type *sC,
                                              const int *s_loff3) {
    constexpr bool UJ = PassUsesJ<P>::value;
    int q0 = 0, q1 = 1, q2 = 2;
    if (m0 == 0) { m0 = m1; a0 = a1; q0 = q1; m1 = m2; a1 = a2; q1 = q2; m2 = 0; }
    if (m0 == 0) { m0 = m1; a0 = a1; q0 = q1; m1 = 0; }
    if (m1 == 0) { m1 = m2; a1 = a2; q1 = q2; m2 = 0; }
    M cur = m0;
    unsigned ca = a0;
    int cq = q0;
    const unsigned tile = lds_addr(sXY);
    if constexpr (pass_pair2<P>()) {
    while (cur) {
        const int t = (sizeof(M) == 8 ? __ffsll((long long)cur) : __ffs((int)cur)) - 1;
        cur &= cur - 1;
        const bool two = cur != 0;
        const int t2 = two ? (sizeof(M) == 8 ? __ffsll((long long)cur) : __ffs((int)cur)) - 1 : t;
        if (two) cur &= cur - 1;
        const unsigned ad = ca + ((unsigned)t << 3), ad2 = ca + ((unsigned)t2 << 3);
        const float2 xy = lds_ld2a(tile + ad), zw = lds_ld2a(tile + ad + ZW_OFF);
        const float2 xy2 = lds_ld2a(tile + ad2), zw2 = lds_ld2a(tile + ad2 + ZW_OFF);
        typename P::BT bj = typename P::BT(), bj2 = typename P::BT();
        if (P::HAS_B) { bj = sB[ad >> 3]; bj2 = sB[ad2 >> 3]; }
        typename PassC<P>::type cj = typename PassC<P>::type(), cj2 = typename PassC<P>::type();
        if (PassC<P>::value) { cj = sC[ad >> 3]; cj2 = sC[ad2 >> 3]; }
        {
            const float dx = xi - xy.x, dy = yi - xy.y, dz = zi - zw.x;
            int j = 0;
            if (UJ) j = (int)(ad >> 3) - s_loff3[cq];
            pass_pair(p, c, own, dx, dy, dz, dx * dx + dy * dy + dz * dz, make_float4(xy.x, xy.y, zw.x, zw.y), bj, cj, j);
        }
        if (two) {
            const float dx = xi - xy2.x, dy = yi - xy2.y, dz = zi - zw2.x;
            int j = 0;
            if (UJ) j = (int)(ad2 >> 3) - s_loff3[cq];
            pass_pair(p, c, own, dx, dy, dz, dx * dx + dy * dy + dz * dz, make_float4(xy2.x, xy2.y, zw2.x, zw2.y), bj2, cj2, j);
        }
        if (cur == 0) { cur = m1; ca = a1; m1 = m2; a1 = a2; m2 = 0; if (UJ) { cq = q1; q1 = q2; } }
    }
    } else {
    while (cur) {
        const int t = (sizeof(M) == 8 ? __ffsll((long long)cur) : __ffs((int)cur)) - 1;
        cur &= cur - 1;
        const unsigned ad = ca + ((unsigned)t << 3);
        const float2 xy = lds_ld2a(tile + ad);
        const float2 zw = lds_ld2a(tile + ad + ZW_OFF);
        typename P::BT bj = typename P::BT();
        if (P::HAS_B) bj = sB[ad >> 3];
        typename PassC<P>::type cj = typename PassC<P>::type();
        if (PassC<P>::value) cj = sC[ad >> 3];
        const float dx = xi - xy.x, dy = yi - xy.y, dz = zi - zw.x;
        const float r2 = dx * dx + dy * dy + dz * dz;
        int j = 0;
        if (UJ) j = (int)(ad >> 3) - s_loff3[cq];
        pass_pair(p, c, own, dx, dy, dz, r2, make_float4(xy.x, xy.y, zw.x, zw.y), bj, cj, j);
        if (cur == 0) { cur = m1; ca = a1; m1 = m2; a1 = a2; m2 = 0; if (UJ) { cq = q1; q1 = q2; } }
    }
    }
}

#define BLK_HDR_INTS 20
#define NBR_CS_SPAN 124
#define NBR_CS_PITCH (NBR_CS_SPAN + 4)
#define NBR_BLOCK 256

struct BlockPrepTables { int *tab[8]; };
struct TilePlanOut { int *list_b, *list_i, *cnt; unsigned char *cls; int lo_layers, hi_layers; int bound_b; int *status; volatile int *mirror_nb; };
__device__ __forceinline__ void block_prep_tile(const Consts &c, int n, const float4 p, int meta_i, const int *__restrict__ cell_start,
                                                int *__restrict__ blk_hdr, unsigned char *__restrict__ perm, int *__restrict__ blk_flag,
                                                unsigned *__restrict__ cellw, int (*s_cnt)[64], int *s_c) {
    const int tid = threadIdx.x, lane = tid & 63, w = tid >> 6;
    const int i0 = blockIdx.x * 256;
    const int i = i0 + tid;
    const int nvalid = (n - i0) < 256 ? (n - i0) : 256;
    int key = 63;
    int my_lin = 0, my_dz0 = 0, my_dz = 0;
    unsigned my_dom = 0u;
    if (i < n) {
        const int cxg = cell_coord(p.x, c.grid_size, c.nx_glob);
        const int k = (int)((p.x / c.grid_size - (float)cxg) * 62.0f);
        const int cx = cell_coord_x(c, p.x);
        key = k < 0 ? 0 : (k > 62 ? 62 : k);
        {
            const int cy = cell_coord(p.y, c.grid_size, c.ny);
            const int cz = cell_coord_z(c, p.z);
            const int lin = (cx * c.ny + cy) * c.nz + cz;
            if (tid == 0) s_c[0] = lin;
            if (tid == nvalid - 1) s_c[1] = lin;
            const int z0 = cz > 0 ? cz - 1 : 0;
            const int z1 = cz < c.nz - 1 ? cz + 1 : c.nz - 1;
            my_lin = lin; my_dz0 = z0 - cz; my_dz = z1 - z0;
            const unsigned by = (cy > 0 ? 1u : 0u) | 2u | (cy < c.ny - 1 ? 4u : 0u);
            my_dom = (cx > 0 ? by : 0u) | (by << 3) | (cx < c.nx - 1 ? by << 6 : 0u);
        }
    }
    (&s_cnt[0][0])[tid] = 0;
    if (blk_flag) {
        const int anyf = __syncthreads_or((i < n && META_ACTIVE_FLUID(meta_i)) ? 1 : 0);
        if (tid == 0) blk_flag[blockIdx.x] = anyf ? 1 : 0;
    }
    unsigned long long peers = ~0ull;
#pragma unroll
    for (int bit = 0; bit < 6; ++bit) {
        const bool on = (key >> bit) & 1;
        const unsigned long long bal = __ballot(on);
        peers &= on ? bal : ~bal;
    }
    const unsigned long long below = (1ull << lane) - 1ull;
    const int rank_in_wave = __popcll(peers & below);
    __syncthreads();
    if (cellw && i < n) {
        const int e0 = (my_lin - s_c[0]) + my_dz0 + 1;
        cellw[i] = (unsigned)(e0 & 0xff) | ((unsigned)(my_dz + 1) << 8) | (my_dom << 11);
    }
    if ((peers & below) == 0ull) s_cnt[w][key] = __popcll(peers);
    if (tid < 9) {
        const int cfirst = s_c[0], clast = s_c[1];
        const int shift = (tid / 3 - 1) * c.ny * c.nz + (tid % 3 - 1) * c.nz;
        int lo = cfirst + shift - 1, hi = clast + shift + 1;
        int rs = 0, re = 0;
        if (clast >= cfirst && hi >= 0 && lo <= c.G - 1) {
            lo = lo < 0 ? 0 : lo;
            hi = hi > c.G - 1 ? c.G - 1 : hi;
            rs = cell_start[lo];
            re = cell_start[hi + 1];
        }
        int *h = blk_hdr + (size_t)blockIdx.x * BLK_HDR_INTS;
        if (tid == 0) { h[0] = cfirst; h[1] = clast; }
        h[2 + tid] = rs;
        h[11 + tid] = re - rs;
    }
    __syncthreads();
    if (perm) {
        const int tot = s_cnt[0][lane] + s_cnt[1][lane] + s_cnt[2][lane] + s_cnt[3][lane];
        const int incl = wave_incl_scan(tot);
        int dest = __shfl(incl - tot, key, 64) + rank_in_wave;
        for (int k = 0; k < w; ++k) dest += s_cnt[k][key];
        perm[i0 + dest] = (unsigned char)tid;
    }
}

__global__ void __launch_bounds__(256)
k_block_prep(const Consts c, const float4 *__restrict__ posv, const int *__restrict__ meta,
             const int *__restrict__ cell_start, int *__restrict__ blk_hdr, unsigned char *__restrict__ perm,
             int *__restrict__ blk_flag, const int *__restrict__ xidx, BlockPrepTables tabs, TilePlanOut plan, unsigned *__restrict__ cellw) {
    __shared__ int s_cnt[4][64];
    __shared__ int s_c[2];
    const int tid = threadIdx.x;
    const int i0 = blockIdx.x * 256;
    const int i = i0 + tid;
    const int n = live_n(c);
    if (plan.list_b && tid == 64 && i0 < n) {
        const int layer = c.ny * c.nz;
        const int r1 = plan.lo_layers > 0 ? cell_start[(plan.lo_layers < c.nx ? plan.lo_layers : c.nx) * layer] : 0;
        const int r2 = plan.hi_layers > 0 ? cell_start[(c.nx - plan.hi_layers > 0 ? c.nx - plan.hi_layers : 0) * layer] : n;
        const int nt = (n + 255) >> 8;
        int t1 = (r1 + 255) >> 8, t2 = r2 >> 8;
        if (t2 > nt) t2 = nt;
        if (t2 < t1) t2 = t1 = nt;
        const int t = (int)blockIdx.x, ni = t2 - t1;
        if (t < t1) plan.list_b[t] = t;
        else if (t >= t2) plan.list_b[t1 + (t - t2)] = t;
        else plan.list_i[t - t1] = t1 + xcd_remap(t - t1, ni);
        plan.cls[t] = (t < t1 || t >= t2) ? 1 : 0;
        if (t == 0) {
            plan.cnt[0] = nt - ni; plan.cnt[1] = ni;
            if (nt - ni > plan.bound_b && plan.status) atomicOr(plan.status, SLAB_ST_BOUND);
            if (plan.mirror_nb) *plan.mirror_nb = nt - ni;
        }
    }
    if (i0 >= n) {
        if (blk_flag && tid == 0) blk_flag[blockIdx.x] = 0;
        return;
    }
    float4 p = make_float4(0.f, 0.f, 0.f, 0.f);
    int meta_i = 0;
    if (i < n) {
        if (xidx) {
            const int x = xidx[i];
            const int kind = (int)(((unsigned)x) >> 28);
            if (kind >= 1 && kind <= 8) tabs.tab[kind - 1][x & 0x0fffffff] = i;
        }
        p = posv[i];
        if (blk_flag) meta_i = meta[i];
    }
    block_prep_tile(c, n, p, meta_i, cell_start, blk_hdr, perm, blk_flag, cellw, s_cnt, s_c);
}

__global__ void __launch_bounds__(256)
k_gather_prep(const Consts c, int n, const int *__restrict__ inv, SortArrays a, const int *__restrict__ cell_start,
              int *__restrict__ blk_hdr, unsigned char *__restrict__ perm, int *__restrict__ blk_flag, unsigned *__restrict__ cellw) {
    __shared__ int s_cnt[4][64];
    __shared__ int s_c[2];
    const int d = blockIdx.x * 256 + threadIdx.x;
    float4 p = make_float4(0.f, 0.f, 0.f, 0.f);
    int meta_i = 0;
    if (d < n) {
        const int i = inv[d];
        p = a.posv_in[i];
        a.posv_out[d] = p;
        if (a.velm_in) {
            meta_i = a.meta_in[i];
            a.velm_out[d] = a.velm_in[i];
            a.meta_out[d] = meta_i;
            a.pid_out[d] = a.pid_in[i];
        }
        if (a.color_in) a.color_out[d] = a.color_in[i];
        if (a.rho_in) a.rho_out[d] = a.rho_in[i];
        if (a.orig_in) a.orig_out[d] = a.orig_in[i];
    }
    block_prep_tile(c, n, p, meta_i, cell_start, blk_hdr, perm, blk_flag, cellw, s_cnt, s_c);
}

__global__ void __launch_bounds__(256)
k_color_from_home(int n, const int *__restrict__ pid, const unsigned *__restrict__ home, unsigned *__restrict__ color) {
    const int i = blockIdx.x * 256 + threadIdx.x;
    if (i < n) color[i] = home[pid[i]];
}

__global__ void __launch_bounds__(256)
k_compact_blocks(const int *__restrict__ flag, int nb, int *__restrict__ list, int *__restrict__ count, volatile int *count_host) {
    __shared__ int s_w[4];
    const int per = (nb + 255) / 256;
    const int lo = threadIdx.x * per, hi = lo + per < nb ? lo + per : nb;
    int mine = 0;
    for (int b = lo; b < hi; ++b) mine += flag[b] ? 1 : 0;
    int tot;
    int at = block_excl_scan_256(mine, s_w, tot);
    for (int b = lo; b < hi; ++b) if (flag[b]) list[at++] = b;
    if (threadIdx.x == 0) { *count = tot; if (count_host) *count_host = tot; }
}

constexpr int SPH_NBR_LIGHT_CAP = 1280;
constexpr int SPH_NBR_HEAVY_BUDGET = 40960;
constexpr int SPH_NBR_MEDIUM_BYTES = 28;
constexpr int SPH_HEAVY_SB = 3;
constexpr int SPH_MEDIUM_SB = 3;
template <class P> constexpr int pass_slot_bytes() {
    return 16 + (P::HAS_B ? (int)sizeof(typename P::BT) : 0) + (PassC<P>::value ? (int)sizeof(typename PassC<P>::type) : 0);
}
template <class P, class = void> struct PassMediumOk { static constexpr bool value = false; };
template <class P> struct PassMediumOk<P, decltype((void)P::MEDIUM_OK)> { static constexpr bool value = P::MEDIUM_OK; };
template <class P> constexpr bool pass_is_medium() {
    return SPH_FAST && P::HAS_B && !pass_builds_masks<P>() &&
           (pass_slot_bytes<P>() <= SPH_NBR_MEDIUM_BYTES || (PassMediumOk<P>::value && pass_slot_bytes<P>() <= 32));
}
template <class P, class = void> struct PassFiveWg { static constexpr bool value = false; };
template <class P> struct PassFiveWg<P, decltype((void)P::FIVE_WG)> { static constexpr bool value = P::FIVE_WG; };
constexpr int SPH_FIVE_WG_SB = 2;
constexpr int SPH_LDS_GRANULE = 1280;
template <class P> constexpr int nbr_tile_cap() {
    const int per_slot = pass_slot_bytes<P>();
    const int budget = (pass_is_medium<P>() || PassFiveWg<P>::value) ? 32768 : SPH_NBR_HEAVY_BUDGET;
    const int pad = (PassFiveWg<P>::value && pass_reuses_masks<P>()) ? 0 : NBR_PAD;
    const int reserve = PassFiveWg<P>::value ? SPH_LDS_GRANULE : 1536;
    const int slots = (budget - 9 * NBR_CS_PITCH * 2 - reserve) / per_slot - pad;
    return slots > SPH_NBR_LIGHT_CAP ? SPH_NBR_LIGHT_CAP : slots / 8 * 8;
}
__device__ __forceinline__ int run_of(int grouping, int g, int q) {
    const int i = g * 3 + q;
    return grouping ? (int)((0x861543720ull >> (4 * i)) & 15ull) : i;
}

template <int CAP>
__device__ __forceinline__ void nbr_plan(const int *__restrict__ hdr, int g, int qa, int fg, int (&rs_)[3], int (&ln_)[3], int (&lo_)[3],
                                         int &total, int &qb, unsigned &rm, bool &overflow, int grouping) {
    total = 0; qb = 3; rm = 7u; overflow = false;
#pragma unroll
    for (int q = 0; q < 3; ++q) {
        const int k = run_of(grouping, g, q);
        rs_[q] = hdr[2 + k];
        ln_[q] = hdr[11 + k] > 0 ? hdr[11 + k] : 0;
    }
    const int ulen = rs_[2] + ln_[2] - rs_[0];
    const bool chain = !grouping && ln_[0] > 0 && ln_[1] > 0 && ln_[2] > 0 && rs_[1] >= rs_[0] && rs_[1] <= rs_[0] + ln_[0] &&
                       rs_[2] >= rs_[1] && rs_[2] <= rs_[1] + ln_[1] && ulen >= ln_[2];
    if (qa == 0 && chain && ulen <= CAP && fg != 1 && fg != 5) {
        lo_[0] = lo_[1] = lo_[2] = -rs_[0];
        total = ulen;
    } else if (qa == 0 && ln_[0] + ln_[1] + ln_[2] <= CAP && fg != 1) {
        lo_[0] = -rs_[0]; lo_[1] = ln_[0] - rs_[1]; lo_[2] = ln_[0] + ln_[1] - rs_[2];
        total = ln_[0] + ln_[1] + ln_[2];
    } else {
        rm = 0u; qb = qa;
#pragma unroll
        for (int q = 0; q < 3; ++q) {
            lo_[q] = INT_MIN;
            if (q >= qa && q == qb && !overflow) {
                if (fg != 1 && total + ln_[q] <= CAP) { lo_[q] = total - rs_[q]; total += ln_[q]; qb = q + 1; rm |= 1u << q; }
                else if (q == qa) { overflow = true; qb = q + 1; rm |= 1u << q; }
            }
        }
    }
}
#ifdef SPH_TIMELINE
#define NBR_STAMP(k) do { if (timeline && threadIdx.x == 0) timeline[(size_t)blockIdx.x * 16 + (k)] = __builtin_readcyclecounter(); } while (0)
#else
#define NBR_STAMP(k) do { } while (0)
#endif
template <class P, int MASKMODE> constexpr int nbr_lds_bytes() {
    return (nbr_tile_cap<P>() + ((MASKMODE == 2 || pass_reuses_masks<P>()) ? 0 : NBR_PAD)) * (16 + (P::HAS_B ? (int)sizeof(typename P::BT) : 0) + (PassC<P>::value ? (int)sizeof(typename PassC<P>::type) : 0)) + 9 * NBR_CS_PITCH * 2 + 64;
}
constexpr int SPH_NBR_WAVES_LIGHT = SPH_FAST ? 6 : 4;
constexpr int SPH_NBR_WAVES_HEAVY = SPH_FAST ? 4 : 3;
template <class P, class = void> struct PassMaxWaves { static constexpr int value = 8; };
template <class P> struct PassMaxWaves<P, decltype((void)P::MAX_WAVES)> { static constexpr int value = P::MAX_WAVES; };
template <class P, int MASKMODE> constexpr int nbr_waves_per_simd() {
    const int w = P::HAS_B ? ((pass_is_medium<P>() || PassFiveWg<P>::value) ? 5 : SPH_NBR_WAVES_HEAVY) : (sizeof(typename P::Own) <= 8 ? SPH_NBR_WAVES_LIGHT : 4);
    return w < PassMaxWaves<P>::value ? w : PassMaxWaves<P>::value;
}
__device__ __forceinline__ int split_lo(int ny, int y) { return ny == 3 ? y : (y == 0 ? 0 : 2); }
__device__ __forceinline__ int split_hi(int ny, int y) { return ny == 3 ? y + 1 : (y == 0 ? 2 : 3); }
template <class P, int MASKMODE>
__global__ void __launch_bounds__(P::BLOCK, (nbr_waves_per_simd<P, MASKMODE>()))
k_nbr_pass(const Consts c, const int *__restrict__ cell_start, const P p, DevScalars *__restrict__ scal,
           int nblocks, unsigned *__restrict__ nbr_mask, unsigned *__restrict__ nbr_mask_hi, int mask_stride,
           const int *__restrict__ blk_hdr, const unsigned char *__restrict__ lane_perm,
           unsigned long long *__restrict__ timeline, const int *__restrict__ stop_flag,
           const int *__restrict__ blk_list, const int *__restrict__ blk_count, const unsigned char *__restrict__ tile_skip) {
    const int stop_now = stop_flag ? *stop_flag : 0;
    const int list_len = blk_list ? *blk_count : INT_MAX;
    const int b_listed = blk_list ? blk_list[blockIdx.x] : 0;
    if (stop_now) return;
    if ((int)blockIdx.x >= list_len) {
        if constexpr (PassPrologue<P>::value) { if (blockIdx.x == 0 && blockIdx.y == 0) p.prologue(scal); }
        return;
    }
    constexpr int BLOCK = P::BLOCK;
    constexpr int CAP = nbr_tile_cap<P>();
    constexpr int NS = (CAP + BLOCK - 1) / BLOCK;
    constexpr int GROUPS = 3, RPG = 3;
    static_assert(P::GROUPS == 3 && BLOCK == 256, "lane permutation is stored as one byte per particle");
    typedef typename P::Own Own;
    typedef typename P::BT BT;
    constexpr int PAD = (MASKMODE == 2 || pass_reuses_masks<P>()) ? 0 : NBR_PAD;
    __shared__ float2 sT[2 * (CAP + PAD)];
    float2 *const sXY = sT;
    float2 *const sZW = sT + (CAP + PAD);
    constexpr int ZW_OFF = (CAP + PAD) * 8;
    __shared__ BT sB[P::HAS_B ? CAP + PAD : 1];
    __shared__ typename PassC<P>::type sC[PassC<P>::value ? CAP + PAD : 1];
    __shared__ unsigned short s_cs[9][NBR_CS_PITCH];
    __shared__ int s_loff[9];

    const int tid = threadIdx.x;
    NBR_STAMP(0);
    const int b = blk_list ? b_listed : xcd_remap(blockIdx.x, nblocks, c.xcd_chunk);
    const int i0 = b * BLOCK;
    const int who_early = lane_perm ? (int)lane_perm[i0 + tid] : tid;
    const int *hdr = blk_hdr + (size_t)b * BLK_HDR_INTS;
    const int cfirst = hdr[0], clast = hdr[1];
    const int skip_tile = tile_skip ? (int)tile_skip[b] : 0;
    const int n_live = live_n(c);
    int carry_d = 0;
    unsigned carry_src = 0u;
    if constexpr (PassSortCarry<P>::value) {
        if (p.carry.on) {
            carry_d = i0 + tid;
            carry_src = (unsigned)p.carry.inv[carry_d < c.n ? carry_d : c.n - 1];
        }
    }
    if constexpr (PassWrench<P>::value) wrench_init_all(p.pose);
    if constexpr (PassPrologue<P>::value) { if (!p.prologue(scal)) return; }
    if (i0 >= n_live) {
        if constexpr (P::HAS_REDUCE) {
            if (tid == 0) {
                const int bs = red_slot(blk_list, b);
                if constexpr (PassSplit<P>::value) {
                    if (gridDim.y > 1) {
                        if (float *o = p.split_out(split_lo((int)gridDim.y, (int)blockIdx.y))) o[bs] = 0.0f;
                        if (gridDim.y == 2 && blockIdx.y == 0) { if (float *o = p.split_out(1)) o[bs] = 0.0f; }
                    } else p.red_out[bs] = 0.0f;
                }
                else p.red_out[bs] = 0.0f;
            }
        }
        return;
    }
    const int who = who_early;
    const int i = i0 + who;
    const bool valid = i < n_live;

    const int span = clast - cfirst;
    bool cs_lds = span >= 0 && span <= NBR_CS_SPAN;
#pragma unroll
    for (int k = 0; k < 9; ++k) cs_lds = cs_lds && hdr[11 + k] < 65536;
    const int ic = valid ? i : i0;
    const unsigned cw = reinterpret_cast<const unsigned *>(blk_hdr + (size_t)((mask_stride + 255) >> 8) * BLK_HDR_INTS)[ic];
    const float4 pi = p.posv[ic];
    Own own;
    bool active = p.begin(c, ic, pi, own) && valid;
    float4 carry_v = make_float4(0.f, 0.f, 0.f, 0.f);
    int carry_m = 0, carry_p = 0;
    if constexpr (PassSortCarry<P>::value) {
        if (p.carry.on) { carry_v = p.carry.velm_in[carry_src]; carry_m = p.carry.meta_in[carry_src]; carry_p = p.carry.pid_in[carry_src]; }
    }
    unsigned mk0[3] = {0u, 0u, 0u};
    if (MASKMODE == 2 && pass_mask_pipe<P>()) {
        const int g0 = (PassSplit<P>::value && gridDim.y > 1) ? split_lo((int)gridDim.y, (int)blockIdx.y) : 0;
#pragma unroll
        for (int q = 0; q < 3; ++q) mk0[q] = nbr_mask[(size_t)run_of(c.run_grouping, g0, q) * mask_stride + i];
    }
    typedef typename PassC<P>::type CT;
    const int g_first = (PassSplit<P>::value && gridDim.y > 1) ? split_lo((int)gridDim.y, (int)blockIdx.y) : 0;
    (void)g_first;
    if (cs_lds && tid < NBR_CS_PITCH) {
        const int tc = tid < span + 4 ? tid : span + 3;
        int cs_[9];
#pragma unroll
        for (int k = 0; k < 9; ++k) {
            int cell = cfirst + (k / 3 - 1) * c.ny * c.nz + (k % 3 - 1) * c.nz - 1 + tc;
            cell = cell < 0 ? 0 : (cell > c.G ? c.G : cell);
            cs_[k] = cell_start[cell];
        }
        if (tid < span + 4) {
#pragma unroll
            for (int k = 0; k < 9; ++k) s_cs[k][tid] = (unsigned short)(cs_[k] - hdr[2 + k]);
        }
    }
    const int e0 = (int)(cw & 0xffu);
    const int e1 = e0 + (int)((cw >> 8) & 7u);
    const unsigned dom = cw >> 11;
    if (skip_tile) return;
    if constexpr (PassSortCarry<P>::value) {
        asm volatile("" :: "v"(cw), "v"(pi.w), "v"(carry_v.x), "v"(carry_m), "v"(carry_p));
    }
    const int any_active = __syncthreads_or(active ? 1 : 0);
    if constexpr (PassSortCarry<P>::value) {
        if (p.carry.on && carry_d < c.n) { p.carry.velm_out[carry_d] = carry_v; p.carry.meta_out[carry_d] = carry_m; p.carry.pid_out[carry_d] = carry_p; }
    }
// ... 294 lines not shown
```

### sph_project_amd/csrc/sph_kernels.hip

```cpp
#include "sph_common.hpp"

#if SPH_FAST
#define SPH_LAUNCH_FN sph_launch_fast
#define SPH_NS sph_fast_ns
#else
#define SPH_LAUNCH_FN sph_launch_strict
#define SPH_NS sph_strict_ns
#endif

#include <vector>
#include <cstdio>
#include <cstdint>
namespace SPH_NS {
#include "sph_device.hpp"
#include "sph_halo_defs.hpp"
#include "sph_passes.hpp"
#include "sph_solvers.hpp"
#include "sph_cg.hpp"
#include "sph_halo.hpp"

inline int cdiv(int a, int b) { return (a + b - 1) / b; }

static int *tile_sum_bank(State &s) {
    if (s.slab_active) return nullptr;
    return s.scan_partial + (size_t)s.scan_bank * (s.scan_blocks + 1) * SCAN_PARTIAL_STRIDE;
}
static void clear_histogram(State &s) {
    hipMemsetAsync(s.cell_count, 0, sizeof(int) * (size_t)(s.c.G + SPH_NGRAVE + 1), s.stream);
    hipMemsetAsync(s.scan_partial + (size_t)s.scan_bank * (s.scan_blocks + 1) * SCAN_PARTIAL_STRIDE, 0, sizeof(int) * (size_t)(s.scan_blocks + 1) * SCAN_PARTIAL_STRIDE, s.stream);
}

static RunList run_list_of(State &s, bool open_epoch) {
    if (!s.run_head || s.slab_active) { s.run_lists_filed = 0; return RunList{nullptr, nullptr, 0, 0u}; }
    if (open_epoch) { if (++s.sort_epoch == 0u) s.sort_epoch = 1u; }
    return RunList{s.run_head, s.run_rec, s.cap, s.sort_epoch};
}

void l_hash_count(State &s) {
    const int n = s.c.n;
    if (s.prehashed) {
        s.prehashed = 0;
        s.cell_count_clean = 0;
        s.n_prehashed_sorts++;
        return;
    }
    if (!s.cell_count_clean) clear_histogram(s);
    s.cell_count_clean = 0;
    int *ts = tile_sum_bank(s);
    s.tile_sums_ready = ts != nullptr;
    s.hist_taken = 1;
    s.run_lists_filed = 0;
    if (n == 0) return;
    s.n_hash_launches++;
    const RunList rl = run_list_of(s, true);
    hipLaunchKernelGGL(k_hash_count, dim3(cdiv(n, 256)), dim3(256), 0, s.stream, s.c, s.posv.cur(), s.cellid,
                       s.rank, s.cell_count, s.slab_active ? s.meta.cur() : nullptr, ts, rl);
    s.run_lists_filed = rl.head != nullptr;
}

void l_scan(State &s) {
    if (!s.hist_taken) s.state_error |= 1;
    s.hist_taken = 0;
    const int G = s.c.G + (s.slab_active ? SPH_NGRAVE : 0);
    int nb = cdiv(G, SCAN_TILE);
    if (nb < SPH_STAT_SLOTS / SCAN_TPB) nb = SPH_STAT_SLOTS / SCAN_TPB;
    int *part = s.scan_partial + (size_t)s.scan_bank * (s.scan_blocks + 1) * SCAN_PARTIAL_STRIDE;
    int *part_next = s.scan_partial + (size_t)(1 - s.scan_bank) * (s.scan_blocks + 1) * SCAN_PARTIAL_STRIDE;
    if (!s.tile_sums_ready) hipLaunchKernelGGL(k_scan_reduce, dim3(nb), dim3(SCAN_TPB), 0, s.stream, s.cell_count, G, part);
    hipLaunchKernelGGL(k_scan_final, dim3(nb), dim3(SCAN_TPB), 0, s.stream, s.cell_count, G, part,
                       s.cell_start, s.c.n, s.scal, 1 - s.c.stat_bank, s.c.n_dev, part_next,
                       s.slab_active ? nullptr : s.scan_tile_state);
    s.cell_count_clean = 1;
    s.scan_bank = 1 - s.scan_bank;
    s.tile_sums_ready = 0;
}

void l_block_prep(State &s, bool launch = true) {
    const int n = s.c.n;
    if (n == 0) return;
    const bool lst = !s.c.all_fluid && s.blk_list;
    BlockPrepTables tabs;
    for (int k = 0; k < 8; ++k) tabs.tab[k] = s.halo_tab[k];
    const int *xi = (s.slab_active && s.tables_pending) ? s.xidx[s.xcur] : nullptr;
    s.tables_pending = 0;
    TilePlanOut plan{nullptr, nullptr, nullptr, nullptr, 0, 0, 0, nullptr, nullptr};
    s.tile_plan_n = -1;
    if (s.slab_active && s.tile_list[0]) {
        const int nt = cdiv(n, 256);
        int known = s.push.mirror ? ((volatile SlabDyn *)s.push.mirror)->n_btiles : -1;
        if (known < 0) known = nt;
        s.tile_bound_b = std::min(nt, known + known / 4 + 64);
        plan = TilePlanOut{s.tile_list[0], s.tile_list[1], s.tile_cnt, s.tile_class, s.has_down ? 3 : 0, s.has_up ? 3 : 0, s.tile_bound_b,
                           s.dyn_cur ? &s.dyn_cur->status : nullptr, s.push.mirror ? &((volatile SlabDyn *)s.push.mirror)->n_btiles : nullptr};
        s.tile_plan_n = n;
    }
    if (launch)
    hipLaunchKernelGGL(k_block_prep, dim3(cdiv(n, 256)), dim3(256), 0, s.stream, s.c, s.posv.cur(), s.meta.cur(), s.cell_start,
                       s.blk_hdr, s.lane_perm, lst ? s.blk_flag : nullptr, xi, tabs, plan,
                       reinterpret_cast<unsigned *>(s.blk_hdr + (size_t)((s.cap + 255) / 256) * BLK_HDR_INTS));
    if (lst) {
        hipLaunchKernelGGL(k_compact_blocks, dim3(1), dim3(256), 0, s.stream, s.blk_flag, cdiv(n, 256), s.blk_list, s.blk_count, s.list_count_pinned);
        s.list_count_known = -1;
        if (s.list_count_event) hipEventRecord(s.list_count_event, s.stream);
    }
    s.list_n = lst ? n : -1;
    s.perm_n = n;
}

unsigned *l_sorted_color(State &s) {
    if (s.color_stale) {
        s.color_stale = 0;
        if (s.c.n > 0) hipLaunchKernelGGL(k_color_from_home, dim3(cdiv(s.c.n, 256)), dim3(256), 0, s.stream, s.c.n, s.pid.cur(), s.color_home, s.color.cur());
    }
    return s.color.cur();
}

SortCarry l_scatter_impl(State &s, bool stable, bool rho_dead, bool density_next) {
    const int n = s.c.n;
    SortCarry carry;
    if (n == 0) return carry;
    SortArrays a;
    a.G = s.c.G;
    a.posv_in = s.posv.cur(); a.posv_out = s.posv.alt();
    a.velm_in = s.velm.cur(); a.velm_out = s.velm.alt();
    a.meta_in = s.meta.cur(); a.meta_out = s.meta.alt();
    a.pid_in = s.pid.cur(); a.pid_out = s.pid.alt();
    a.color_out = s.color.alt();
    a.rho_in = s.rho.cur(); a.rho_out = s.rho.alt();
    a.orig_in = s.orig.cur(); a.orig_out = s.orig.alt();
    a.xidx_in = s.slab_active ? s.xidx[s.xcur] : nullptr; a.xidx_out = s.slab_active ? s.xidx[1 - s.xcur] : nullptr;
    const bool by_lists = stable && s.run_lists_filed && s.run_head && s.sort_inv && !s.slab_active;
    a.color_in = by_lists ? s.color.cur() : l_sorted_color(s);
    s.run_lists_filed = 0;
    const bool skip_rho = by_lists && rho_dead && s.c.all_fluid;
    carry.on = by_lists && density_next && s.c.all_fluid && !s.tile_list[0];
    if (by_lists) {
        if (s.color_home && s.color_home_ok) { a.color_in = nullptr; s.color_stale = 1; }
        if (skip_rho) a.rho_in = nullptr;
        if (carry.on) {
            carry.inv = s.sort_inv;
            carry.velm_in = a.velm_in; carry.velm_out = a.velm_out;
            carry.meta_in = a.meta_in; carry.meta_out = a.meta_out;
            carry.pid_in = a.pid_in; carry.pid_out = a.pid_out;
            a.velm_in = nullptr; a.meta_in = nullptr; a.pid_in = nullptr;
        }
        hipLaunchKernelGGL(k_sort_rank, dim3(cdiv(n, 256)), dim3(256), 0, s.stream, n, s.cellid, s.cell_start,
                           RunList{s.run_head, s.run_rec, s.cap, s.sort_epoch}, s.sort_inv);
        const bool lst = !s.c.all_fluid && s.blk_list;
        hipLaunchKernelGGL(k_gather_prep, dim3(cdiv(n, 256)), dim3(256), 0, s.stream, s.c, n, s.sort_inv, a, s.cell_start,
                           s.blk_hdr, s.lane_perm, lst ? s.blk_flag : nullptr,
                           reinterpret_cast<unsigned *>(s.blk_hdr + (size_t)((s.cap + 255) / 256) * BLK_HDR_INTS));
        s.n_list_sorts++;
    } else if (stable) {
        hipLaunchKernelGGL(k_scatter_index, dim3(cdiv(n, 256)), dim3(256), 0, s.stream, n, s.cellid, s.rank,
                           s.cell_start, (int2 *)s.tmp_idx, s.c.n_dev);
        hipLaunchKernelGGL(k_scatter<true>, dim3(cdiv(n, 256)), dim3(256), 0, s.stream, n, s.cellid, s.rank,
                           s.cell_start, (const int2 *)s.tmp_idx, a, s.c.n_dev);
    } else {
        hipLaunchKernelGGL(k_scatter<false>, dim3(cdiv(n, 256)), dim3(256), 0, s.stream, n, s.cellid, s.rank,
                           s.cell_start, (const int2 *)s.tmp_idx, a, s.c.n_dev);
    }
    s.posv.flip(); s.velm.flip(); s.meta.flip(); s.pid.flip(); s.color.flip(); s.rho.flip();
#ifdef SPH_TEST_HOOKS
    if (skip_rho) hipMemsetAsync(s.rho.cur(), 0xFF, sizeof(float) * (size_t)n, s.stream);
    if (carry.on) {
        hipMemsetAsync(s.velm.cur(), 0xFF, sizeof(float4) * (size_t)n, s.stream);
        hipMemsetAsync(s.meta.cur(), 0xFF, sizeof(int) * (size_t)n, s.stream);
        hipMemsetAsync(s.pid.cur(), 0xFF, sizeof(int) * (size_t)n, s.stream);
    }
#endif
    s.masks_valid = 0;
    if (!s.slab_active) l_block_prep(s, !by_lists);
    else s.perm_n = s.list_n = -1;
    if (s.orig.cur()) s.orig.flip();
    if (s.slab_active) s.xcur = 1 - s.xcur;
    return carry;
}
void l_scatter(State &s) { l_scatter_impl(s, false, false, false); }
SortCarry l_scatter_stable(State &s, bool rho_dead, bool density_next) { return l_scatter_impl(s, true, rho_dead, density_next); }

int list_grid(State &s, int nb) {
    if (!s.list_count_pinned) return nb;
    if (s.list_count_known < 0 && s.list_count_event) {
        const hipError_t q = hipEventQuery(s.list_count_event);
        if (q == hipSuccess) s.list_count_known = *s.list_count_pinned;
        else if (q == hipErrorNotReady && hipPeekAtLastError() == hipErrorNotReady) (void)hipGetLastError();
    }
    const int g = s.list_count_known >= 0 ? s.list_count_known : nb;
    return g < 1 ? 1 : (g > nb ? nb : g);
}

template <class P> void launch_pass(State &s, const P &p, int mask_mode = 0, int tiles = 0, int split = 0) {
    const int n = s.c.n;
    if (n == 0) return;
    const int nb = cdiv(n, P::BLOCK);
    if (s.c.force_global == 1) mask_mode = 0;
    if (mask_mode == 2 && !s.masks_valid) mask_mode = 0;
    if (s.perm_n != n) l_block_prep(s);
    if (!(PassModes<P>::value & (1 << mask_mode))) mask_mode = 0;
    const unsigned char *perm = mask_mode == 2 ? s.lane_perm : nullptr;
    const bool use_list = PassFluidOnly<P>::value && !s.c.all_fluid && s.list_n == n && s.c.force_global == 0;
    const int *bl = use_list ? s.blk_list : nullptr, *bc = use_list ? s.blk_count : nullptr;
    int nb_launch = nb;
    const unsigned char *skip = nullptr;
    if (tiles && s.tile_plan_n == n && !use_list) {
        if (tiles == 1) { bl = s.tile_list[0]; bc = s.tile_cnt; nb_launch = s.tile_bound_b > 0 ? s.tile_bound_b : 1; }
        else skip = s.tile_class;
    }
    if (use_list) nb_launch = list_grid(s, nb);
    if (P::HAS_REDUCE) s.last_pass_listed = use_list ? 1 : 0;
    unsigned long long *tl = (s.c.force_global == 20 && (size_t)nb * 16 * 8 <= (size_t)s.cap * 4) ? (unsigned long long *)s.tmp_idx : nullptr;
    if (tl) hipMemsetAsync(tl, 0, (size_t)nb * 16 * 8, s.stream);
    constexpr int MODES = PassModes<P>::value;
    if (!(MODES & (1 << mask_mode))) mask_mode = 0;
    const int gy = (PassSplit<P>::value && split) ? split : 1;
#define SPH_LAUNCH_NBR(M) hipLaunchKernelGGL((k_nbr_pass<P, M>), dim3(nb_launch, gy), dim3(P::BLOCK), 0, s.stream, s.c, s.cell_start, p, s.scal, nb, s.nbr_mask, s.nbr_mask_hi, s.cap, s.blk_hdr, perm, tl, s.loop_flag, bl, bc, skip)
    if (mask_mode == 1) {
        if constexpr ((MODES & 0b010) != 0) { SPH_LAUNCH_NBR(1); s.masks_valid = 1; }
    } else if (mask_mode == 2) {
        if constexpr ((MODES & 0b100) != 0) { SPH_LAUNCH_NBR(2); }
    } else {
        SPH_LAUNCH_NBR(0);
    }
#undef SPH_LAUNCH_NBR
    if (tl) {
        static int shown = 0;
        hipStreamSynchronize(s.stream);
        std::vector<unsigned long long> hbuf((size_t)nb * 16);
        hipMemcpy(hbuf.data(), tl, hbuf.size() * 8, hipMemcpyDeviceToHost);
        if (shown++ % 8 < 2) {
            double d[16] = {0}; double cnt[16] = {0};
            unsigned long long tmin = ~0ull, tmax = 0;
            for (int b = 0; b < nb; ++b) {
                const unsigned long long *t = &hbuf[(size_t)b * 16];
                int prev = 0;
                for (int k = 1; k < 16; ++k) if (t[k]) { d[k] += (double)(t[k] - t[prev]); cnt[k] += 1; prev = k; }
                if (t[0] && t[0] < tmin) tmin = t[0];
                if (t[15] > tmax) tmax = t[15];
            }
            double life = 0; for (int b = 0; b < nb; ++b) life += (double)(hbuf[(size_t)b * 16 + 15] - hbuf[(size_t)b * 16]);
            fprintf(stderr, "timeline mode %d BT %d: kernel %.1f kclk, workgroup lifetime %.1f kclk; mean clk per stamp:", mask_mode, (int)sizeof(typename P::BT), (tmax - tmin) * 1e-3, life / nb * 1e-3);
            for (int k = 1; k < 16; ++k) fprintf(stderr, " [%d]%.0f", k, cnt[k] ? d[k] / cnt[k] : 0.0);
            fprintf(stderr, "\n");
        }
    }
}

void l_density(State &s, int eos, DensityOpts o) {
    HaloFieldSend fs = s.fieldsend;
    if (!eos) fs.on = 0;
    s.fieldsend.on = 0;
    const int sp = o.books_forces ? 1 + 3 : 1, se = o.books_forces ? 2 : 1;
    SortCarry carry = o.carry;
    if (carry.on && (!s.c.all_fluid || o.tiles != 0 || s.c.n == 0)) { s.state_error |= 2; carry.on = 0; }
#ifdef SPH_TEST_HOOKS
    if (getenv("SPH_TEST_DROP_CARRY")) carry.on = 0;
#endif
    if (carry.on) s.n_carried_sorts++;
    if (s.c.all_fluid) {
        if (eos) { DensityPass<true, true> p{{carry}, s.posv.cur(), s.meta.cur(), s.rho_raw, s.rho.cur(), s.prs, s.ptm, fs, sp, se}; launch_pass(s, p, 1, o.tiles); }
        else { DensityPass<true, false> p{{carry}, s.posv.cur(), s.meta.cur(), s.rho_raw, s.rho.cur(), s.prs, s.ptm, fs, sp, se}; launch_pass(s, p, 1, o.tiles); }
    } else {
        if (eos) { DensityPass<false, true> p{{}, s.posv.cur(), s.meta.cur(), s.rho_raw, s.rho.cur(), s.prs, s.ptm, fs, sp, se}; launch_pass(s, p, 1, o.tiles); }
        else { DensityPass<false, false> p{{}, s.posv.cur(), s.meta.cur(), s.rho_raw, s.rho.cur(), s.prs, s.ptm, fs, sp, se}; launch_pass(s, p, 1, o.tiles); }
    }
}

void l_non_pressure(State &s, const float4 *visc_vel) {
    const float *rho_src = s.visc_rho_raw ? s.rho_raw : s.rho.cur();
    if (s.poly6) {
        if (s.c.all_fluid) {
            NonPressurePass<true, Poly6Kernel> p{s.posv.cur(), s.velm.cur(), s.meta.cur(), rho_src, s.velm.alt(), s.scal, s.pose, s.c.rho0, s.skip_viscosity, s.np_acc_out, visc_vel};
            launch_pass(s, p, 2);
        } else {
            NonPressurePass<false, Poly6Kernel> p{s.posv.cur(), s.velm.cur(), s.meta.cur(), rho_src, s.velm.alt(), s.scal, s.pose, s.c.rho0, s.skip_viscosity, s.np_acc_out, visc_vel};
            launch_pass(s, p, 2);
        }
    } else if (s.c.all_fluid) {
        NonPressurePass<true> p{s.posv.cur(), s.velm.cur(), s.meta.cur(), rho_src, s.velm.alt(), s.scal, s.pose, s.c.rho0, s.skip_viscosity, s.np_acc_out, visc_vel};
        launch_pass(s, p, 2);
    } else {
        NonPressurePass<false> p{s.posv.cur(), s.velm.cur(), s.meta.cur(), rho_src, s.velm.alt(), s.scal, s.pose, s.c.rho0, s.skip_viscosity, s.np_acc_out, visc_vel};
        launch_pass(s, p, 2);
    }
    s.velm.flip();
}

__global__ void __launch_bounds__(256)
k_emitter_advance(const Consts c, float4 *posv, const float4 *velm, int *meta, const RigidPose *pose) {
    int i = blockIdx.x * 256 + threadIdx.x;
    if (i >= live_n(c)) return;
    const int m = meta[i];
    if (META_MAT(m) == 1) return;
    float4 p = posv[i];
    if (up_coord(c, p) > c.g_upper) {
        const int obj = META_OBJ(m);
        if (obj >= 0 && pose->material[obj] == 1) {
            const float4 v = velm[i];
            p.x += c.dt * v.x; p.y += c.dt * v.y; p.z += c.dt * v.z;
            posv[i] = p;
            if (up_coord(c, p) <= c.g_upper) meta[i] = META_SET_MAT(m, 1);
        }
    }
}

void l_pressure_integrate(State &s) {
    if (s.c.all_fluid) {
        PressurePass<true> p{s.posv.cur(), s.meta.cur(), s.ptm, s.prs, s.rho.cur(), s.velm.cur(), s.acc, s.posv.alt(), s.scal, s.pose, s.c.rho0, 1};
        launch_pass(s, p, 2);
    } else {
        PressurePass<false> p{s.posv.cur(), s.meta.cur(), s.ptm, s.prs, s.rho.cur(), s.velm.cur(), s.acc, s.posv.alt(), s.scal, s.pose, s.c.rho0, 1};
        launch_pass(s, p, 2);
    }
    s.posv.flip();
    s.masks_valid = 0;
    if (s.has_emitter && s.c.n > 0)
        hipLaunchKernelGGL(k_emitter_advance, dim3(cdiv(s.c.n, 256)), dim3(256), 0, s.stream, s.c, s.posv.cur(),
                           s.velm.cur(), s.meta.cur(), s.pose);
}

void l_wcsph_forces(State &s, ForceOpts o) {
    NextHash nh{0, s.cellid, s.rank, s.cell_count, tile_sum_bank(s), RunList{nullptr, nullptr, 0, 0u}};
    if (o.hash_next && s.c.all_fluid && !s.slab_active && s.cell_count_clean && o.booked_by_density && s.c.n > 0) nh.on = 1;
    if (nh.on) nh.rl = run_list_of(s, true);
    if (!o.booked_by_density) {
        if (s.c.all_fluid) {
            WcsphForcePass<true, false, true> p{s.posv.cur(), s.velm.cur(), s.meta.cur(), s.rho_raw, s.ptm, s.prs, s.rho.cur(), s.velm.alt(), s.acc, s.posv.alt(), s.scal, s.pose, s.c.rho0, s.presend, nh};
            launch_pass(s, p, 2);
        } else {
            WcsphForcePass<false, false, true> p{s.posv.cur(), s.velm.cur(), s.meta.cur(), s.rho_raw, s.ptm, s.prs, s.rho.cur(), s.velm.alt(), s.acc, s.posv.alt(), s.scal, s.pose, s.c.rho0, s.presend, nh};
            launch_pass(s, p, 2);
        }
    } else
#if SPH_FAST
    if (s.c.all_fluid && s.uniform_mass && !s.slab_active) {
        WcsphForcePass<true, true> p{s.posv.cur(), s.velm.cur(), s.meta.cur(), s.rho_raw, s.ptm, s.prs, s.rho.cur(), s.velm.alt(), s.acc, s.posv.alt(), s.scal, s.pose, s.c.rho0, s.presend, nh};
        launch_pass(s, p, 2);
    } else
#endif
    if (s.c.all_fluid) {
        WcsphForcePass<true> p{s.posv.cur(), s.velm.cur(), s.meta.cur(), s.rho_raw, s.ptm, s.prs, s.rho.cur(), s.velm.alt(), s.acc, s.posv.alt(), s.scal, s.pose, s.c.rho0, s.presend, nh};
        launch_pass(s, p, 2);
    } else {
        WcsphForcePass<false> p{s.posv.cur(), s.velm.cur(), s.meta.cur(), s.rho_raw, s.ptm, s.prs, s.rho.cur(), s.velm.alt(), s.acc, s.posv.alt(), s.scal, s.pose, s.c.rho0, s.presend, nh};
        launch_pass(s, p, 2);
    }
    if (s.presend.on) { s.presend.on = 0; s.preclassified = 1; }
    if (nh.on) { s.prehashed = 1; s.cell_count_clean = 0; s.tile_sums_ready = nh.tile_sum != nullptr; s.hist_taken = 1; s.run_lists_filed = nh.rl.head != nullptr; }
    s.velm.flip();
    s.posv.flip();
    s.masks_valid = 0;
    if (s.has_emitter && s.c.n > 0)
        hipLaunchKernelGGL(k_emitter_advance, dim3(cdiv(s.c.n, 256)), dim3(256), 0, s.stream, s.c, s.posv.cur(),
                           s.velm.cur(), s.meta.cur(), s.pose);
}

void l_rigid_volume(State &s) {
    if (s.poly6) { RigidVolumePass<Poly6Kernel> p{s.posv.cur(), s.velm.cur(), s.meta.cur()}; launch_pass(s, p); return; }
    RigidVolumePass<> p{s.posv.cur(), s.velm.cur(), s.meta.cur()};
    launch_pass(s, p);
}

__global__ void __launch_bounds__(256)
k_renew_rigid(const Consts c, float4 *posv, float4 *velm, const float4 *orig, const int *meta, const RigidPose *pose) {
    int i = blockIdx.x * 256 + threadIdx.x;
    if (i >= live_n(c)) return;
    const int m = meta[i];
    if (META_MAT(m) != 2 || !META_DYN(m)) return;
    const int o = META_OBJ(m);
    if (o < 0 || !pose->is_dynamic[o]) return;
    const float4 q0 = orig[i];
    const float qx = q0.x - pose->com0[o][0], qy = q0.y - pose->com0[o][1], qz = q0.z - pose->com0[o][2];
    const float *R = pose->rot[o];
    const float px = R[0] * qx + R[1] * qy + R[2] * qz;
    const float py = R[3] * qx + R[4] * qy + R[5] * qz;
    const float pz = R[6] * qx + R[7] * qy + R[8] * qz;
    float4 p = posv[i], v = velm[i];
    p.x = pose->com[o][0] + px; p.y = pose->com[o][1] + py; p.z = pose->com[o][2] + pz;
    const float wx = pose->angvel[o][0], wy = pose->angvel[o][1], wz = pose->angvel[o][2];
    v.x = pose->vel[o][0] + (wy * pz - wz * py);
    v.y = pose->vel[o][1] + (wz * px - wx * pz);
    v.z = pose->vel[o][2] + (wx * py - wy * px);
    posv[i] = p; velm[i] = v;
}

void l_renew_rigid(State &s) {
    if (!s.has_dynamic_rigid || s.c.n == 0 || !s.orig.cur()) return;
    s.masks_valid = 0;
    hipLaunchKernelGGL(k_renew_rigid, dim3(cdiv(s.c.n, 256)), dim3(256), 0, s.stream, s.c, s.posv.cur(),
                       s.velm.cur(), s.orig.cur(), s.meta.cur(), s.pose);
}

__global__ void __launch_bounds__(256) k_prepare_emitter(const Consts c, const float4 *posv, int *meta) {
    int i = blockIdx.x * 256 + threadIdx.x;
    if (i >= live_n(c)) return;
    const int m = meta[i];
    if (META_MAT(m) == 1 && up_coord(c, posv[i]) > c.g_upper) meta[i] = META_SET_MAT(m, 2);
}

void l_prepare_emitter(State &s) {
    if (!s.has_emitter || s.c.n == 0) return;
    hipLaunchKernelGGL(k_prepare_emitter, dim3(cdiv(s.c.n, 256)), dim3(256), 0, s.stream, s.c, s.posv.cur(),
                       s.meta.cur());
}

__global__ void __launch_bounds__(256)
k_post_insert(const Consts c, int first, float4 *posv, float4 *velm, const int *meta, int stale_volume) {
    const int i = first + blockIdx.x * 256 + threadIdx.x;
    if (i >= live_n(c)) return;
    const int m = meta[i];
    float4 p = posv[i], v = velm[i];
    if (META_MAT(m) == 1) {
        if (META_DYN(m)) { enforce_boundary(c, p.x, p.y, p.z, v.x, v.y, v.z); posv[i] = p; velm[i] = v; }
    } else if (stale_volume && META_MAT(m) == 2 && up_coord(c, p) <= c.g_upper) {
        const float V = 1.0f / c.W0;
        p.w = V; v.w = c.rho0 * V;
        posv[i] = p; velm[i] = v;
    }
}
void l_post_insert(State &s, int first, int stale_volume) {
    if (s.c.n <= first) return;
    hipLaunchKernelGGL(k_post_insert, dim3(cdiv(s.c.n - first, 256)), dim3(256), 0, s.stream, s.c, first, s.posv.cur(),
                       s.velm.cur(), s.meta.cur(), stale_volume);
}
__global__ void __launch_bounds__(256) k_clear_fresh(int n, int *meta) {
    const int i = blockIdx.x * 256 + threadIdx.x;
    if (i < n) { const int m = meta[i]; if (m & META_FRESH_BIT) meta[i] = m & ~META_FRESH_BIT; }
}
void l_clear_fresh(State &s) {
    if (s.c.n > 0) hipLaunchKernelGGL(k_clear_fresh, dim3(cdiv(s.c.n, 256)), dim3(256), 0, s.stream, s.c.n, s.meta.cur());
}

// ... 73 lines not shown
```

### sph_project_amd/csrc/sph_passes.hpp

```cpp
#pragma once
#include "sph_device.hpp"

typedef float WrenchRows[4][SPH_NOBJ][6];
__device__ __forceinline__ WrenchRows &wrench_rows() {
    __shared__ WrenchRows s_rows;
    return s_rows;
}
typedef float WrenchCom[SPH_NOBJ][3];
__device__ __forceinline__ WrenchCom &wrench_com() {
    __shared__ WrenchCom s_com;
    return s_com;
}
__device__ __forceinline__ void wrench_init_all(const RigidPose *pose) {
    float *r = &wrench_rows()[0][0][0];
    for (int k = threadIdx.x; k < 4 * SPH_NOBJ * 6; k += 256) r[k] = 0.0f;
    if (threadIdx.x < SPH_NOBJ * 3) (&wrench_com()[0][0])[threadIdx.x] = (&pose->com[0][0])[threadIdx.x];
}
__device__ __forceinline__ void wrench_flush_all(DevScalars *scal) {
    const int k = threadIdx.x;
    if (k >= SPH_NOBJ * 6) return;
    const WrenchRows &w = wrench_rows();
    const int obj = k / 6, q = k % 6;
    const float v = ((w[0][obj][q] + w[1][obj][q]) + w[2][obj][q]) + w[3][obj][q];
    if (v != 0.0f)
        atomicAdd((unsigned long long *)(scal->wrench + (q < 3 ? 0 : SPH_NOBJ * 3) + obj * 3 + q % 3),
                  (unsigned long long)__double2ll_rn((double)v * SPH_WRENCH_SCALE));
}
__device__ __forceinline__ void add_wrench(DevScalars *, int obj, float fx, float fy, float fz, float tx, float ty, float tz) {
    float *r = wrench_rows()[threadIdx.x >> 6][obj];
    atomicAdd(r + 0, fx); atomicAdd(r + 1, fy); atomicAdd(r + 2, fz);
    atomicAdd(r + 3, tx); atomicAdd(r + 4, ty); atomicAdd(r + 5, tz);
}

template <bool AF, bool EOS>
struct DensityPass : SortCarryOf<AF> {
    static constexpr int MODES = 0b011;
    static constexpr bool FLUID_BLOCKS_ONLY = true;
    static constexpr int BLOCK = 256, GROUPS = 3;
    static constexpr bool USES_J = !AF;
    static constexpr bool HAS_B = false, COUNT_PAIRS = true;
    static constexpr int PAIR_WEIGHT = 1;
    static constexpr bool HAS_REDUCE = false;
    typedef int BT;
    struct Own { float sum; };
    const float4 *posv; const int *meta;
    float *rho_raw, *rho, *prs, *ptm;
    HaloFieldSend fs;
    static constexpr bool STAT_W = true;
    int stat_pairs, stat_evals;
    static constexpr bool SORT_CARRY = AF;

    __device__ float4 loadA(int j) const { return posv[j]; }
    __device__ BT loadB(int) const { return 0; }
    __device__ float4 stage(const Consts &, int j, BT &) const { return posv[j]; }
    __device__ bool begin(const Consts &c, int i, const float4 &, Own &o) const {
        o.sum = 0.0f;
        if (AF && !c.ghosts) return true;
        return META_ACTIVE_FLUID(meta[i]);
    }
    __device__ void pair(const Consts &c, Own &o, float, float, float, float r2, const float4 &a, const BT &,
                         int) const {
#if SPH_FAST
        const float q2 = r2 * c.inv_h2, q = __builtin_amdgcn_sqrtf(q2), t = 1.0f - q;
        const float lo = 1.0f - (6.0f * q2) * t, hi = 2.0f * (t * t * t);
        o.sum += a.w * (q <= 0.5f ? lo : hi);
#else
        o.sum += a.w * kernW(c, geom(c, r2));
#endif
    }
    __device__ float finish(const Consts &c, int i, const float4 &pi, Own &o) const {
        float den = pi.w * c.W0;
#if SPH_FAST
        den += c.kW * o.sum;
#else
        den += o.sum;
#endif
        den *= c.rho0;
        if (EOS) {
            rho_raw[i] = den;
            float rc = fmaxf(den, c.rho0);
            rho[i] = rc;
#if SPH_FAST
            const float x = rc * c.inv_rho0, x2 = x * x, x4 = x2 * x2;
            float pr = 50000.0f * (x4 * x2 * x - 1.0f);
#else
            float pr = 50000.0f * (powf(rc / c.rho0, 7.0f) - 1.0f);
#endif
            prs[i] = pr;
            const float pt = pr / (rc * rc);
            ptm[i] = pt;
            if (fs.on) {
                const int x = fs.xidx[i], kind = HALO_KIND(x), k = HALO_IDX(x);
                if (kind == HALO_SEND || kind == HALO_SEND + 1) {
                    const int side = kind - HALO_SEND;
                    if (fs.out[side] && k < fs.dyn->n_send[side]) fs.out[side][k] = make_float4(den, rc, pr, pt);
                } else if (kind == HALO_ECHO_SEND || kind == HALO_ECHO_SEND + 1) {
                    const int side = kind - HALO_ECHO_SEND;
                    if (fs.out[side] && k < fs.dyn->n_recv[side]) fs.out[side][fs.dyn->n_send[side] + k] = make_float4(den, rc, pr, pt);
                }
            }
        } else {
            rho[i] = den;
        }
        return 0.0f;
    }
    __device__ void passive(const Consts &, int, const float4 &) const {}
};

struct CubicKernel {
    static __device__ __forceinline__ float W(const Consts &c, const Geom &g) { return kernW(c, g); }
    static __device__ __forceinline__ float W0(const Consts &c) { return c.W0; }
    static __device__ __forceinline__ float Wd(const Consts &c) { return c.Wd; }
    static __device__ __forceinline__ void grad(const Consts &c, float dx, float dy, float dz, const Geom &g, float &gx, float &gy, float &gz) {
        kernGrad(c, dx, dy, dz, g, gx, gy, gz);
    }
    static __device__ __forceinline__ float gradScale(const Consts &c, const Geom &g) { return kernGradScale(c, g); }
    static __device__ __forceinline__ float Wpoly(const Consts &, const Geom &g) { return kernWpoly(g); }
    static __device__ __forceinline__ float Wd_poly(const Consts &c) { return c.Wd_poly; }
    static __device__ __forceinline__ float Wscale(const Consts &c) { return c.kW; }
};

#define SPH_POLY6_FAC 1.5666814710608448f
#define SPH_SPIKY_FAC -14.323944878270580f
__device__ __forceinline__ float poly6W(const Consts &c, float rn) {
    if (!(rn > 0.0f && rn < c.h)) return 0.0f;
#if SPH_FAST
    const float x = (c.h * c.h - rn * rn) * (c.inv_h * c.inv_h * c.inv_h);
#else
    const float x = (c.h * c.h - rn * rn) / (c.h * c.h * c.h);
#endif
    return SPH_POLY6_FAC * x * x * x;
}
__device__ __forceinline__ float spikyScale(const Consts &c, float rn) {
// ... 194 lines not shown
    __device__ float4 stage(const Consts &, int j, BT &bj) const { return stage_impl(j, bj); }
    __device__ bool begin(const Consts &c, int i, const float4 &pi, Own &o) const {
        bool ok = true;
        if (!AF) { const int m = meta[i]; ok = META_ACTIVE_FLUID(m) && META_DYN(m); }
        else if (c.ghosts) ok = !META_GHOST(meta[i]);
        o.x = pi.x; o.y = pi.y; o.z = pi.z; o.m0 = rho0 * pi.w;
        o.pt = ptm[i]; o.p = prs[i];
        const float r = rho[i];
        o.rho2 = r * r;
        o.ax = o.ay = o.az = 0.0f;
        return ok;
    }
    __device__ void pair(const Consts &c, Own &o, float dx, float dy, float dz, float r2, const float4 &a,
                         const BT &bj, int j) const {
        const Geom g = geom(c, r2);
#if SPH_FAST
        if (AF || bj >= 0.0f) {
            const float k = (-a.w * (o.pt + bj)) * kernGradScale(c, g);
            o.ax += k * dx; o.ay += k * dy; o.az += k * dz;
            return;
        }
#endif
        float gx, gy, gz;
        kernGrad(c, dx, dy, dz, g, gx, gy, gz);
        if (AF || bj >= 0.0f) {
            const float cc = -a.w * (o.pt + bj);
            o.ax += cc * gx; o.ay += cc * gy; o.az += cc * gz;
        } else {
            const float cc = fdiv(-a.w * o.p, o.rho2);
            o.ax += cc * gx; o.ay += cc * gy; o.az += cc * gz;
            if (bj <= -2.0f) {
                const int obj = (int)(-bj) - 2;
                const float cf = fdiv(a.w * o.p, o.rho2);
                const float fx = (cf * gx) * o.m0, fy = (cf * gy) * o.m0, fz = (cf * gz) * o.m0;
                const float rx = o.x - wrench_com()[obj][0], ry = o.y - wrench_com()[obj][1], rz = o.z - wrench_com()[obj][2];
                add_wrench(scal, obj, fx, fy, fz, ry * fz - rz * fy, rz * fx - rx * fz, rx * fy - ry * fx);
            }
        }
    }
    __device__ float finish(const Consts &c, int i, const float4 &pi, Own &o) const {
        acc[i] = make_float4(o.ax, o.ay, o.az, 0.0f);
        if (!integrate) return 0.0f;
        const float4 v = velm[i];
        float vx = v.x + c.dt * o.ax, vy = v.y + c.dt * o.ay, vz = v.z + c.dt * o.az;
        float x = pi.x + c.dt * vx, y = pi.y + c.dt * vy, z = pi.z + c.dt * vz;
        enforce_boundary(c, x, y, z, vx, vy, vz);
        posv_out[i] = make_float4(x, y, z, pi.w);
        velm[i] = make_float4(vx, vy, vz, v.w);
        return 0.0f;
    }
    __device__ void passive(const Consts &, int i, const float4 &pi) const {
        acc[i] = make_float4(0.f, 0.f, 0.f, 0.f);
        if (integrate) posv_out[i] = pi;
    }
};

template <bool AF, bool UM = false, bool CNT = false>
struct WcsphForcePass {
    static constexpr bool HAS_WRENCH = !AF;
    static constexpr int BLOCK = 256, GROUPS = 3;
    static constexpr bool USES_J = !AF;
    static constexpr bool HAS_B = true;
    static constexpr bool COUNT_PAIRS = CNT;
    static constexpr int MAX_WAVES = CNT ? (SPH_FAST ? 4 : 3) : 8;
    static constexpr bool MASK_PIPELINE = AF;
    static constexpr int PAIR_WEIGHT = 3;
    static constexpr bool HAS_REDUCE = false;
    static constexpr bool FIVE_WG = SPH_FAST && AF && UM && !CNT;
    static constexpr bool HAS_C = !FIVE_WG;
    typedef float4 BT;
    typedef float CT;
    struct Own {
        float vx, vy, vz, m, rho, st_m, sx, sy, sz, ax, ay, az;
        float pt, p, rho2, px, py, pz, x, y, z, m0;
        float cvm, cstm;
        int dyn;
        int lin_new;
    };
    static constexpr bool NEXT_HASH = AF;
    const float4 *posv, *velm; const int *meta; const float *rho_raw, *ptm, *prs, *rho;
    float4 *vel_out, *acc, *posv_out; DevScalars *scal; const RigidPose *pose; float rho0;
    HaloSend hs;
    NextHash nh;
    __device__ int cell_of(const Consts &c, float x, float y, float z) const {
        return (cell_coord_x(c, x) * c.ny + cell_coord(y, c.grid_size, c.ny)) * c.nz + cell_coord_z(c, z);
    }

    __device__ float4 loadA(int j) const { return posv[j]; }
    __device__ float4 stage(const Consts &, int j, BT &bj, CT &cj) const {
        const float4 p = ldg_idx(posv, j);
        const float4 v = ldg_idx(velm, j);
        if (AF) {
            bj = make_float4(v.x, v.y, v.z, ldg_idx(rho_raw, j));
            cj = ldg_idx(ptm, j);
            return make_float4(p.x, p.y, p.z, v.w);
        }
        const int m = meta[j];
        const bool fl = META_MAT(m) == 1;
        bj = make_float4(v.x, v.y, v.z, fl ? rho_raw[j] : (META_DYN(m) ? -2.0f - (float)META_OBJ(m) : -1.0f));
        cj = fl ? ptm[j] : 0.0f;
        return make_float4(p.x, p.y, p.z, fl ? v.w : rho0 * p.w);
    }
    __device__ float4 stage(const Consts &c, int j, BT &bj) const {
        CT cj;
        const float4 a = stage(c, j, bj, cj);
        return make_float4(a.x, a.y, a.z, cj);
    }
    __device__ bool begin(const Consts &c, int i, const float4 &pi, Own &o) const {
        o.dyn = 1;
        bool ok = true;
        if (AF && c.ghosts) ok = !META_GHOST(meta[i]);
        if (!AF) {
            const int m = meta[i];
            ok = META_ACTIVE_FLUID(m);
            if (!ok) return false;
            o.dyn = META_DYN(m);
        }
        const float4 v = velm[i];
        o.vx = v.x; o.vy = v.y; o.vz = v.z; o.m = v.w;
        o.rho = rho_raw[i];
#if SPH_FAST
        o.st_m = (fdiv(c.st, v.w) * c.rho0) * c.kW;
#else
        o.st_m = fdiv(c.st, v.w);
#endif
        o.cvm = c.cv * ((v.w + v.w) * 0.5f); o.cstm = o.st_m * v.w;
        if (FIVE_WG) {
            o.m = __int_as_float(__builtin_amdgcn_readfirstlane(__float_as_int(o.m)));
            o.cvm = __int_as_float(__builtin_amdgcn_readfirstlane(__float_as_int(o.cvm)));
            o.cstm = __int_as_float(__builtin_amdgcn_readfirstlane(__float_as_int(o.cstm)));
        }
        o.sx = o.sy = o.sz = 0.0f;
        o.ax = o.ay = o.az = 0.0f;
        o.x = pi.x; o.y = pi.y; o.z = pi.z; o.m0 = rho0 * pi.w;
        o.pt = ptm[i]; o.p = prs[i];
        const float r = rho[i];
        o.rho2 = r * r;
        o.px = o.py = o.pz = 0.0f;
        return ok;
    }
    __device__ void pair(const Consts &c, Own &o, float dx, float dy, float dz, float r2, const float4 &a,
                         const BT &bj, const CT &cj, int j) const {
        const Geom g = geom(c, r2);
#if SPH_FAST
        const float gs = kernGradScale(c, g);
        const float v_xy = (o.vx - bj.x) * dx + (o.vy - bj.y) * dy + (o.vz - bj.z) * dz;
        if (AF || bj.w >= 0.0f) {
            const float w = r2 > c.diameter2 ? kernWpoly(g) : c.Wd_poly;
            const float cw = (UM ? o.cstm : o.st_m * a.w) * w;
            const float cvm = UM ? o.cvm : c.cv * ((o.m + a.w) * 0.5f);
            const float cc = fdiv2(cvm, bj.w, r2 + c.visc_eps) * v_xy;
            const float k = cc * gs - cw;
            o.ax += k * dx; o.ay += k * dy; o.az += k * dz;
            const float cp = (-(UM ? o.m : a.w) * (o.pt + cj)) * gs;
            o.px += cp * dx; o.py += cp * dy; o.pz += cp * dz;
        } else {
            const float k = (fdiv2(c.cvb * a.w, o.rho, r2 + c.visc_eps) * v_xy) * gs;
            const float acx = k * dx, acy = k * dy, acz = k * dz;
            o.ax += acx; o.ay += acy; o.az += acz;
            const float cp = fdiv(-a.w * o.p, o.rho2) * gs;
            o.px += cp * dx; o.py += cp * dy; o.pz += cp * dz;
            if (bj.w <= -2.0f) {
                const int obj = (int)(-bj.w) - 2;
                float fx = fdiv(-acx * o.m, c.rho0), fy = fdiv(-acy * o.m, c.rho0), fz = fdiv(-acz * o.m, c.rho0);
                float rx = a.x - wrench_com()[obj][0], ry = a.y - wrench_com()[obj][1], rz = a.z - wrench_com()[obj][2];
                float tx = ry * fz - rz * fy, ty = rz * fx - rx * fz, tz = rx * fy - ry * fx;
// ... 127 lines not shown
```

### sph_project_amd/csrc/sph_steps.hpp

```cpp
#pragma once
#include <sched.h>

static int read_red(SphHandle *h, int slot, float *out) {
    HIPCHK(h, hipMemcpyAsync(&h->scal_h->red[slot], &h->st.scal->red[slot], sizeof(float), hipMemcpyDeviceToHost, h->st.stream));
    HIPCHK(h, hipStreamSynchronize(h->st.stream));
    *out = h->scal_h->red[slot];
    return SPH_OK;
}

static int implicit_viscosity_non_pressure(SphHandle *h);

struct LoopPub { float red[8]; int flags[4]; unsigned seq; unsigned pad[3]; };
static_assert(sizeof(LoopPub) == 64, "LoopPub layout");
__global__ void __launch_bounds__(64) k_publish_loop(DevScalars *scal, LoopPub *pub, unsigned seq) {
    const int t = threadIdx.x;
    const int stop = scal->flags[0];
    if (t < 8) __hip_atomic_store(&pub->red[t], scal->red[t], __ATOMIC_RELAXED, __HIP_MEMORY_SCOPE_SYSTEM);
    else if (t < 12) __hip_atomic_store(&pub->flags[t - 8], scal->flags[t - 8], __ATOMIC_RELAXED, __HIP_MEMORY_SCOPE_SYSTEM);
    __threadfence_system();
    __syncthreads();
    if (t == 0) {
        if (stop) { scal->flags[0] = 0; scal->flags[1] = 0; }
        __hip_atomic_store(&pub->seq, seq, __ATOMIC_RELEASE, __HIP_MEMORY_SCOPE_SYSTEM);
    }
// ... 45 lines not shown
        h->loop_flags_clean = false;
    }
    hipError_t e = hipMemcpyAsync(h->scal_h->red, s.scal->red, 8 * sizeof(float) + 4 * sizeof(int), hipMemcpyDeviceToHost, s.stream);
    if (e == hipSuccess) e = hipStreamSynchronize(s.stream);
    if (e != hipSuccess) return fail(h, SPH_ERR_HIP, "solver loop read-back failed: %s", hipGetErrorString(e));
    return SPH_OK;
}

static long long dfsph_particle_num(SphHandle *h) { return h->st.slab_active ? h->comm_n_global : (long long)h->n; }

struct SkipResidual {
    State &s;
    SkipResidual(SphHandle *h) : s(h->st) {
        s.skip_residual = (h->prm.fixed_iterations > 0 && !s.slab_active) ? 1 : 0;
    }
    ~SkipResidual() { s.skip_residual = 0; }
};

struct SolveSpec {
    int slot;
    int kind;
    double thr;
    float denom;
    int max_itr;
    float fixed_err;
    int32_t *iter;
    float *err;
    void (*batch_end)(State &);
};

template <class Pre, class Body>
static int run_solve(SphHandle *h, const SolveSpec &sp, Pre pre, Body body, int *launched = nullptr) {
    State &s = h->st;
    SkipResidual skip(h);
    pre();
    const int fixed = h->prm.fixed_iterations;
    int n = 0;
    if (fixed > 0) {
        for (; n < fixed; ++n) { int rc = body(); if (rc) return rc; }
        *sp.iter = fixed; *sp.err = sp.fixed_err;
    } else {
        if (!h->loop_flags_clean) HIPCHK(h, hipMemsetAsync(&s.scal->flags[0], 0, 2 * sizeof(int), s.stream));
        h->loop_flags_clean = false;
        s.loop_flag = &s.scal->flags[0];
        s.loop_slot = sp.slot; s.loop_kind = sp.kind; s.loop_denom = sp.denom; s.loop_thr = sp.thr;
        const int hint = h->loop_hint[sp.slot];
        int batch = hint > 3 ? hint - 1 : 2, rc = SPH_OK;
        bool predicted = hint > 3;
        static_assert(offsetof(DevScalars, flags) == offsetof(DevScalars, red) + 8 * sizeof(float), "red / flags layout");
        while (n < sp.max_itr) {
            const int nb = std::min(batch, sp.max_itr - n);
            for (int k = 0; k < nb && !rc; ++k) rc = body();
            if (rc) break;
            if (sp.batch_end) sp.batch_end(s);
            n += nb;
            rc = loop_readback(h);
            if (rc || h->scal_h->flags[0]) break;
            if (predicted) { batch = 2; predicted = false; }
            else if (batch < 8) batch *= 2;
        }
        s.loop_flag = nullptr;
        if (rc) return rc;
        *sp.iter = h->loop_hint[sp.slot] = h->scal_h->flags[1];
        *sp.err = sp.denom > 0 ? h->scal_h->red[sp.slot] / sp.denom : 0.0f;
    }
    if (launched) *launched = n;
    return SPH_OK;
}

static int run_non_pressure(SphHandle *h) {
    if (h->prm.viscosity_implicit) {
        int rc = implicit_viscosity_non_pressure(h);
        return rc;
    }
    ProfScope p(h, SPH_K_NON_PRESSURE);
    h->L->non_pressure(h->st, nullptr);
    return SPH_OK;
}

static int wcsph_step(SphHandle *h) {
    State &s = h->st;
    const bool fused = !h->prm.viscosity_implicit;
    SortCarry carry;
    if (s.slab_active) { int rc = slab_neighbor_search(h, fused); if (rc) return rc; }
    else carry = ph_neighbor_search(h, true, true);
    ph_rigid_volume(h);
    const bool books = fused && !getenv("SPH_FORCES_COUNT_OWN");
    const bool overlap = s.slab_active && s.push.on && s.tile_list[0] && s.c.all_fluid && s.tile_plan_n == s.c.n && (s.has_down || s.has_up);
    if (overlap) {
        const int hint = slab_field_hint(h);
        { ProfScope p(h, SPH_K_DENSITY); h->L->density(s, 1, {1, books}); }
        { ProfScope p(h, SPH_K_HALO); h->L->halo_push_fields(s, 2, nullptr, nullptr, hint); }
        { ProfScope p(h, SPH_K_DENSITY); h->L->density(s, 1, {2, books}); }
        { ProfScope p(h, SPH_K_HALO); h->L->halo_pull_fields(s, 2, nullptr, nullptr, hint); }
    } else if (s.slab_active && s.push.on) {
        const int hint = slab_field_hint(h);
        h->L->halo_fieldsend_begin(s);
        { ProfScope p(h, SPH_K_DENSITY); h->L->density(s, 1, {0, books}); }
        { ProfScope p(h, SPH_K_HALO); h->L->halo_pull_fields(s, 2, nullptr, nullptr, hint); }
    } else {
        { ProfScope p(h, SPH_K_DENSITY); h->L->density(s, 1, {0, books, carry}); }
        if (s.slab_active) { int rc = slab_exchange_fields(h); if (rc) return rc; }
    }
    if (fused) {
        const SlabComm &cm = h->comm;
        const bool rebalance_next = cm.rebalance_every > 0 && (h->steps + 1) % cm.rebalance_every == 0 && !h->any_rigid_object;
        if (s.slab_active && s.push.on && h->steps_to_follow > 0 && !rebalance_next && !s.has_emitter && !h->any_rigid_object &&
            !h->sort_dirty)
            h->L->halo_presend_begin(s);
        const bool hash_next = !s.slab_active && s.c.all_fluid && h->steps_to_follow > 0 && !s.has_emitter && !h->any_rigid_object &&
                               !h->sort_dirty;
        ProfScope p(h, SPH_K_WCSPH_FORCES); h->L->wcsph_forces(s, {books, hash_next});
        return SPH_OK;
    }
    int rc = run_non_pressure(h); if (rc) return rc;
    { ProfScope p(h, SPH_K_PRESSURE_INTEGRATE); h->L->pressure_integrate(s); }
    return SPH_OK;
}

static int dfsph_divergence(SphHandle *h, bool first_derivative_done = false) {
    State &s = h->st;
    const SolveSpec sp{.slot = 0, .kind = 1, .thr = 0.001 * h->prm.density_0 / (double)s.c.dt,
                       .denom = (float)dfsph_particle_num(h), .max_itr = 1000, .fixed_err = 0.0f,
                       .iter = &h->last.iter_divergence, .err = &h->last.err_divergence, .batch_end = nullptr};
    int launched = 0;
    int rc = run_solve(h, sp, [&] {
        if (!first_derivative_done) { ProfScope p(h, SPH_K_DFSPH_RHO_ADV); h->L->dfsph_rho_adv(s, 0); }
    }, [&]() -> int {
        std::swap(s.kappa_v, s.kappa_v_next);
        if (s.slab_active) { int rc = slab_exchange_scalar(h, s.kappa_v); if (rc) return rc; }
        { ProfScope p(h, SPH_K_DFSPH_CORRECT); h->L->dfsph_correct(s, 0); }
        if (s.slab_active) { int rc = slab_exchange_vel(h); if (rc) return rc; }
        { ProfScope p(h, SPH_K_DFSPH_RHO_ADV); h->L->dfsph_rho_adv(s, 0); }
        return s.slab_active ? slab_finish_reduction(h, 0) : SPH_OK;
    }, &launched);
    if (rc) return rc;
    if ((launched - h->last.iter_divergence) & 1) std::swap(s.kappa_v, s.kappa_v_next);
    return SPH_OK;
}

static int dfsph_density(SphHandle *h) {
    State &s = h->st;
    const SolveSpec sp{.slot = 1, .kind = 1, .thr = 0.0001, .denom = (float)dfsph_particle_num(h), .max_itr = 1000,
                       .fixed_err = 0.0f, .iter = &h->last.iter_density, .err = &h->last.err_density, .batch_end = nullptr};
    int launched = 0;
    int rc = run_solve(h, sp, [&] { ProfScope p(h, SPH_K_DFSPH_RHO_ADV); h->L->dfsph_rho_adv(s, 1); }, [&]() -> int {
        std::swap(s.kappa, s.kappa_next);
        if (s.slab_active) { int rc = slab_exchange_scalar(h, s.kappa); if (rc) return rc; }
        { ProfScope p(h, SPH_K_DFSPH_CORRECT); h->L->dfsph_correct(s, 1); }
        if (s.slab_active) { int rc = slab_exchange_vel(h); if (rc) return rc; }
        { ProfScope p(h, SPH_K_DFSPH_RHO_ADV); h->L->dfsph_rho_adv(s, 1); }
        return s.slab_active ? slab_finish_reduction(h, 1) : SPH_OK;
    }, &launched);
    if (rc) return rc;
    if ((launched - h->last.iter_density) & 1) std::swap(s.kappa, s.kappa_next);
    return SPH_OK;
}

static int dfsph_step_begin(SphHandle *h) {
    State &s = h->st;
    if (h->sort_dirty) {
        if (s.slab_active) { int rc = slab_neighbor_search(h); if (rc) return rc; }
        else ph_neighbor_search(h);
        ph_rigid_volume(h);
        { ProfScope p(h, SPH_K_DFSPH_DENSITY_ALPHA); h->L->dfsph_density_alpha(s); }
        if (s.slab_active) { int rc = slab_exchange_scalar(h, s.rho.cur()); if (rc) return rc; }
    }
    int rc = run_non_pressure(h); if (rc) return rc;
    if (s.slab_active) { rc = slab_exchange_vel(h); if (rc) return rc; }
    rc = dfsph_density(h); if (rc) return rc;
// ... 239 lines not shown
```

Before: 5.239 billion.

## Overlap WCSPH density and force passes across two streams via tile split

```diff
diff --git a/sph_project_amd/csrc/sph_api.hip b/sph_project_amd/csrc/sph_api.hip
--- a/sph_project_amd/csrc/sph_api.hip
+++ b/sph_project_amd/csrc/sph_api.hip
@@ -39,6 +39,11 @@
     SphPbfParams pbf = {SPH_PBF_VARIANT_REFERENCE, 1, 50, 1e-3f, 1e-6f};
     SphPbfStats pbf_last = {SPH_PBF_VARIANT_REFERENCE, 0, 0.0f};
     int steps_to_follow = 0;
+    float walk_frac = 0.0f;
+    int walk_min_tiles = 0;
+    int walk_reserve_forced = -1;
+    int walk_grid2 = 0, walk_cut_last = 0;
+    bool walk_report = false;
     bool whole_step = false;
     double total_time = 0.0;
     bool prepared = false;
@@ -204,6 +209,7 @@
     if (!h) return;
     hipSetDevice(h->device);
     if (h->st.stream) hipStreamSynchronize(h->st.stream);
+    if (h->st.walk_stream) hipStreamSynchronize(h->st.walk_stream);
     slab_comm_destroy(h->comm);
     if (h->st.push.mirror) { hipHostFree(h->st.push.mirror); h->st.push.mirror = nullptr; }
     for (auto &s : h->prof) for (auto &pr : s.pending) { hipEventDestroy(pr.first); hipEventDestroy(pr.second); }
@@ -213,6 +219,9 @@
     if (h->loop_pub) hipHostFree((void *)h->loop_pub);
     if (h->st.list_count_pinned) { hipHostFree((void *)h->st.list_count_pinned); h->st.list_count_pinned = nullptr; }
     if (h->st.list_count_event) { hipEventDestroy(h->st.list_count_event); h->st.list_count_event = nullptr; }
+    for (hipEvent_t &e : h->st.walk_ev) if (e) { hipEventDestroy(e); e = nullptr; }
+    if (h->st.walk_mirror) { hipHostFree(h->st.walk_mirror); h->st.walk_mirror = nullptr; }
+    if (h->st.walk_stream) { hipStreamDestroy(h->st.walk_stream); h->st.walk_stream = nullptr; }
     if (h->st.stream) hipStreamDestroy(h->st.stream);
     delete h;
 }
@@ -309,6 +318,17 @@
     { void *lp = nullptr; HIP_CREATE(hipHostMalloc(&lp, 128, hipHostMallocDefault)); memset(lp, 0, 128); h->loop_pub = (struct LoopPub *)lp; }
     { int *lc = nullptr; HIP_CREATE(hipHostMalloc((void **)&lc, 64, hipHostMallocDefault)); *lc = 0; s.list_count_pinned = lc; }
     HIP_CREATE(hipEventCreateWithFlags(&s.list_count_event, hipEventDisableTiming));
+    if (p.method == SPH_METHOD_WCSPH && !p.viscosity_implicit && s.sort_inv && !getenv("SPH_NO_WALK_OVERLAP")) {
+        h->walk_frac = SPH_WALK_CUT;
+        h->walk_min_tiles = SPH_WALK_MIN_TILES;
+#ifdef SPH_TEST_HOOKS
+        if (const char *e = getenv("SPH_TEST_WALK_OVERLAP")) { h->walk_frac = (float)atof(e); h->walk_min_tiles = 1; }
+        if (const char *e = getenv("SPH_TEST_WALK_MIN_TILES")) h->walk_min_tiles = atoi(e);
+        if (const char *e = getenv("SPH_TEST_WALK_RESERVE")) h->walk_reserve_forced = atoi(e);
+        h->walk_report = getenv("SPH_TEST_WALK_REPORT") != nullptr;
+#endif
+        if (!(h->walk_frac > 0.0f) || (int)((cap + 255) / 256) < h->walk_min_tiles) h->walk_frac = 0.0f;
+    }
     memset(h->scal_h, 0, sizeof(DevScalars));
     for (int o = 0; o < SPH_NOBJ; ++o) { h->pose_h.rot[o][0] = h->pose_h.rot[o][4] = h->pose_h.rot[o][8] = 1.0f; }
     s.z_hi = slab_layers_glob(s.c);
@@ -730,6 +750,7 @@
 
 static void prof_resolve(SphHandle *h) {
     hipStreamSynchronize(h->st.stream);
+    if (h->st.walk_stream) hipStreamSynchronize(h->st.walk_stream);
     for (auto &s : h->prof) {
         for (auto &pr : s.pending) {
             float ms = 0.0f;
@@ -741,16 +762,16 @@
 }
 
 struct ProfScope {
-    SphHandle *h; int k; hipEvent_t e1 = nullptr;
-    ProfScope(SphHandle *h_, int k_) : h(h_), k(k_) {
+    SphHandle *h; int k; hipEvent_t e1 = nullptr; hipStream_t st;
+    ProfScope(SphHandle *h_, int k_, hipStream_t stream = nullptr) : h(h_), k(k_), st(stream ? stream : h_->st.stream) {
         if (h->prof[k].on) {
             if (h->prof[k].pending.size() > 8192) prof_resolve(h);
             hipEvent_t e0 = get_event(h); e1 = get_event(h);
-            hipEventRecord(e0, h->st.stream);
+            hipEventRecord(e0, st);
             h->prof[k].pending.push_back({e0, e1});
         }
     }
-    ~ProfScope() { if (e1) hipEventRecord(e1, h->st.stream); }
+    ~ProfScope() { if (e1) hipEventRecord(e1, st); }
 };
 
 extern "C" int sph_profile_enable(SphHandle *h, int kernel_id, int on) {
@@ -809,19 +830,42 @@
     return SPH_OK;
 }
 
+static int walk_check_short(SphHandle *h) {
+    State &s = h->st;
+    if (!s.walk_mirror || !__atomic_load_n(s.walk_mirror + 1, __ATOMIC_ACQUIRE)) return SPH_OK;
+    s.walk_mirror[1] = 0; s.walk_mirror[0] = -1;
+    return fail(h, SPH_ERR_INVALID, "walk overlap: a force launch's grid fell short of its tiles (the stretch of deferred tiles outgrew its bound); the state is invalid -- SPH_NO_WALK_OVERLAP=1 avoids the path");
+}
+
 static int check_async(SphHandle *h) {
     if (h->st.state_error) { const int se = h->st.state_error; h->st.state_error = 0; return fail(h, SPH_ERR_INVALID, "internal state error %d (bit 0: a sort was scanned without a histogram of its own; bit 1: a density launch could not move the arrays its sort left to it)", se); }
+    { int rc = walk_check_short(h); if (rc) return rc; }
     hipError_t e = hipGetLastError();
     if (e != hipSuccess) return fail(h, SPH_ERR_HIP, "kernel launch failed: %s", hipGetErrorString(e));
     return SPH_OK;
 }
 
-static SortCarry ph_neighbor_search(SphHandle *h, bool rho_dead = false, bool density_next = false) {
+static int walk_ensure(SphHandle *h) {
+    State &s = h->st;
+    if (s.walk_mirror) return SPH_OK;
+    if (!s.walk_stream) HIPCHK(h, hipStreamCreateWithFlags(&s.walk_stream, hipStreamNonBlocking));
+    for (hipEvent_t &e : s.walk_ev) if (!e) HIPCHK(h, hipEventCreateWithFlags(&e, hipEventDisableTiming | hipEventDisableSystemFence));
+    void *q = nullptr;
+    if (!s.velm_third) { HIPCHK(h, hipMalloc(&q, sizeof(float4) * (size_t)(s.cap > 0 ? s.cap : 1))); h->allocs.push_back(q); s.velm_third = (float4 *)q; }
+    if (!s.walk_first) { HIPCHK(h, hipMalloc(&q, 2 * sizeof(int))); h->allocs.push_back(q); s.walk_first = (int *)q; }
+    const int none[2] = {INT_MAX, INT_MAX};
+    HIPCHK(h, hipMemcpy(s.walk_first, none, sizeof(none), hipMemcpyHostToDevice));
+    HIPCHK(h, hipHostMalloc((void **)&s.walk_mirror, 64, hipHostMallocDefault));
+    s.walk_mirror[0] = -1; s.walk_mirror[1] = 0; s.walk_mirror[2] = 0;
+    return SPH_OK;
+}
+
+static SortCarry ph_neighbor_search(SphHandle *h, bool rho_dead = false, bool density_next = false, int walk_cut = 0) {
     State &s = h->st;
     SortCarry carry;
     { ProfScope p(h, SPH_K_HASH_COUNT); h->L->hash_count(s); }
     { ProfScope p(h, SPH_K_SCAN); h->L->scan(s); }
-    { ProfScope p(h, SPH_K_SCATTER); if (h->prm.deterministic) carry = h->L->scatter_stable(s, rho_dead, density_next && !getenv("SPH_NO_SORT_CARRY")); else h->L->scatter(s); }
+    { ProfScope p(h, SPH_K_SCATTER); if (h->prm.deterministic) carry = h->L->scatter_stable(s, rho_dead, density_next && !getenv("SPH_NO_SORT_CARRY"), walk_cut); else h->L->scatter(s); }
     h->sort_dirty = false;
     return carry;
 }
@@ -829,7 +873,7 @@
 static void ph_sort_hashed(SphHandle *h) {
     State &s = h->st;
     { ProfScope p(h, SPH_K_SCAN); h->L->scan(s); }
-    { ProfScope p(h, SPH_K_SCATTER); if (h->prm.deterministic) h->L->scatter_stable(s, false, false); else h->L->scatter(s); }
+    { ProfScope p(h, SPH_K_SCATTER); if (h->prm.deterministic) h->L->scatter_stable(s, false, false, 0); else h->L->scatter(s); }
     h->sort_dirty = false;
 }
 
@@ -883,7 +927,7 @@
 static int finish_sync(SphHandle *h) {
     { int rc = slab_settle_if_needed(h); if (rc) return rc; }
     HIPCHK(h, hipStreamSynchronize(h->st.stream));
-    return SPH_OK;
+    return walk_check_short(h);
 }
 
 extern "C" int sph_prepare(SphHandle *h) {
@@ -1043,7 +1087,17 @@
     if (!h) return SPH_ERR_INVALID;
     HIPCHK(h, hipSetDevice(h->device));
     if (!h->n_exact) return slab_settle(h);
-    return loop_readback(h);
+    int rc = loop_readback(h);
+    if (!rc) rc = walk_check_short(h);
+#ifdef SPH_TEST_HOOKS
+    if (!rc && h->walk_report && h->st.walk_mirror && *h->st.walk_mirror >= 0) {
+        const int T = (h->st.c.n + 255) / 256, def = *h->st.walk_mirror;
+        fprintf(stderr, "walk overlap: step %lld tiles %d cut %d deferred %d (leave the first force launch at its top: %.2f %% of T); second force launch "
+                "%d workgroups for %d tiles (surplus %d = %.2f %% of T)\n", (long long)h->steps, T, h->walk_cut_last, def, 100.0 * def / T, h->walk_grid2,
+                T - h->walk_cut_last + def, h->walk_grid2 - (T - h->walk_cut_last + def), 100.0 * (h->walk_grid2 - (T - h->walk_cut_last + def)) / T);
+    }
+#endif
+    return rc;
 }
 
 extern "C" int sph_step(SphHandle *h, int nsteps) {
@@ -1093,6 +1147,7 @@
     if (!h || !out) return SPH_ERR_INVALID;
     HIPCHK(h, hipSetDevice(h->device));
     int rc = read_scalars(h); if (rc) return rc;
+    rc = walk_check_short(h); if (rc) return rc;
     h->last.steps = h->steps;
     h->last.particle_num = h->n;
     h->last.fluid_particle_num = h->n_fluid;
@@ -1171,6 +1226,7 @@
     State &s = h->st;
     const size_t n = (size_t)h->n;
     HIPCHK(h, hipStreamSynchronize(s.stream));
+    { int rc = walk_check_short(h); if (rc) return rc; }
     const bool is_vec3 = field == SPH_F_POSITION || field == SPH_F_VELOCITY || field == SPH_F_ACCELERATION ||
                          field == SPH_F_PRESSURE_ACCEL || field == SPH_F_PREDICTED_VEL || field == SPH_F_PREDICTED_POS ||
                          field == SPH_F_CG_X || field == SPH_F_ORIG_POSITION || field == SPH_F_IISPH_DII || field == SPH_F_IISPH_DIJ_PJ ||
diff --git a/sph_project_amd/csrc/sph_common.hpp b/sph_project_amd/csrc/sph_common.hpp
--- a/sph_project_amd/csrc/sph_common.hpp
+++ b/sph_project_amd/csrc/sph_common.hpp
@@ -1,6 +1,7 @@
 #pragma once
 #include <hip/hip_runtime.h>
 #include <stdint.h>
+#include <type_traits>
 
 #define SPH_NOBJ 20
 #define SPH_IISPH_OMEGA 0.2f
@@ -381,6 +382,13 @@
     long long n_carried_sorts = 0;
     unsigned *color_home = nullptr;
     int color_home_ok = 0, color_stale = 0;
+    hipStream_t walk_stream = nullptr;
+    hipEvent_t walk_ev[3] = {};
+    float4 *velm_third = nullptr;
+    int *walk_first = nullptr;
+    unsigned walk_seq = 0u;
+    int *walk_mirror = nullptr;
+    unsigned walk_pub_seq = 0u;
     int *tmp_idx = nullptr;
     int *scan_partial = nullptr;
     int scan_blocks = 0;
@@ -488,18 +496,43 @@
     const int *meta_in = nullptr; int *meta_out = nullptr;
     const int *pid_in = nullptr; int *pid_out = nullptr;
     int on = 0;
+    int walk_cut = 0;
+    const int *walk_first = nullptr;
 };
 template <bool ON> struct SortCarryOf { SortCarry carry; };
 template <> struct SortCarryOf<false> {};
+
+struct TileRange {
+    int first = 0, end = 0;
+    const int *split = nullptr;
+    int side = 0;
+};
+struct NoTileRange {};
+
+constexpr float SPH_WALK_CUT = 0.35f;
+constexpr int SPH_WALK_MIN_TILES = 3 * 1536;
+struct WalkOverlap {
+    int cut = 0;
+    const int *first = nullptr;
+    hipStream_t side = nullptr;
+    hipEvent_t done[2] = {nullptr, nullptr};
+    int reserve = 0;
+    int *mirror = nullptr;
+    unsigned seq = 0u;
+};
+constexpr unsigned SPH_WALK_MAX_LAG = 16u;
 
 struct DensityOpts {
     int tiles = 0;
     bool books_forces = false;
     SortCarry carry = {};
+    WalkOverlap walk = {};
 };
 struct ForceOpts {
     bool booked_by_density = false;
     bool hash_next = false;
+    WalkOverlap walk = {};
+    float4 *vel_out = nullptr;
 };
 
 struct Launch {
@@ -507,7 +540,7 @@
     void (*hash_count)(State &);
     void (*scan)(State &);
     void (*scatter)(State &);
-    SortCarry (*scatter_stable)(State &, bool rho_dead, bool density_next);
+    SortCarry (*scatter_stable)(State &, bool rho_dead, bool density_next, int walk_cut);
     void (*density)(State &, int eos, DensityOpts o);
     void (*non_pressure)(State &, const float4 *visc_vel);
     void (*pressure_integrate)(State &);
diff --git a/sph_project_amd/csrc/sph_device.hpp b/sph_project_amd/csrc/sph_device.hpp
--- a/sph_project_amd/csrc/sph_device.hpp
+++ b/sph_project_amd/csrc/sph_device.hpp
@@ -489,6 +489,8 @@
 template <class P> struct PassNextHash<P, decltype((void)P::NEXT_HASH)> { static constexpr bool value = P::NEXT_HASH; };
 template <class P, class = void> struct PassSortCarry { static constexpr bool value = false; };
 template <class P> struct PassSortCarry<P, decltype((void)P::SORT_CARRY)> { static constexpr bool value = P::SORT_CARRY; };
+template <class P, class = void> struct PassTileRange { static constexpr bool value = false; };
+template <class P> struct PassTileRange<P, decltype((void)P::TILE_RANGE)> { static constexpr bool value = P::TILE_RANGE; };
 template <class P, class = void> struct PassPrologue { static constexpr bool value = false; };
 template <class P> struct PassPrologue<P, decltype((void)P::HAS_PROLOGUE)> { static constexpr bool value = P::HAS_PROLOGUE; };
 
@@ -677,9 +679,18 @@
 
 struct BlockPrepTables { int *tab[8]; };
 struct TilePlanOut { int *list_b, *list_i, *cnt; unsigned char *cls; int lo_layers, hi_layers; int bound_b; int *status; volatile int *mirror_nb; };
+struct WalkPlanOut { int *first = nullptr; int *reset = nullptr; int cut = 0; int limit = 0; };
+__global__ void __launch_bounds__(64) k_walk_publish(const int *__restrict__ first, int cut, int reserve, int *mirror, unsigned seq) {
+    if (threadIdx.x != 0) return;
+    const int f = *first;
+    const int deferred = f < cut ? cut - f : 0;
+    __hip_atomic_store(mirror, deferred, __ATOMIC_RELAXED, __HIP_MEMORY_SCOPE_SYSTEM);
+    if (deferred > reserve) __hip_atomic_store(mirror + 1, 1, __ATOMIC_RELAXED, __HIP_MEMORY_SCOPE_SYSTEM);
+    __hip_atomic_store(reinterpret_cast<unsigned *>(mirror + 2), seq, __ATOMIC_RELEASE, __HIP_MEMORY_SCOPE_SYSTEM);
+}
 __device__ __forceinline__ void block_prep_tile(const Consts &c, int n, const float4 p, int meta_i, const int *__restrict__ cell_start,
                                                 int *__restrict__ blk_hdr, unsigned char *__restrict__ perm, int *__restrict__ blk_flag,
-                                                unsigned *__restrict__ cellw, int (*s_cnt)[64], int *s_c) {
+                                                unsigned *__restrict__ cellw, int (*s_cnt)[64], int *s_c, const WalkPlanOut walk = WalkPlanOut{}) {
     const int tid = threadIdx.x, lane = tid & 63, w = tid >> 6;
     const int i0 = blockIdx.x * 256;
     const int i = i0 + tid;
@@ -740,6 +751,7 @@
         if (tid == 0) { h[0] = cfirst; h[1] = clast; }
         h[2 + tid] = rs;
         h[11 + tid] = re - rs;
+        if (walk.first && (int)blockIdx.x < walk.cut && re > walk.limit) atomicMin(walk.first, (int)blockIdx.x);
     }
     __syncthreads();
     if (perm) {
@@ -800,10 +812,12 @@
 
 __global__ void __launch_bounds__(256)
 k_gather_prep(const Consts c, int n, const int *__restrict__ inv, SortArrays a, const int *__restrict__ cell_start,
-              int *__restrict__ blk_hdr, unsigned char *__restrict__ perm, int *__restrict__ blk_flag, unsigned *__restrict__ cellw) {
+              int *__restrict__ blk_hdr, unsigned char *__restrict__ perm, int *__restrict__ blk_flag, unsigned *__restrict__ cellw,
+              const WalkPlanOut walk) {
     __shared__ int s_cnt[4][64];
     __shared__ int s_c[2];
     const int d = blockIdx.x * 256 + threadIdx.x;
+    if (walk.reset && d == 0) *walk.reset = INT_MAX;
     float4 p = make_float4(0.f, 0.f, 0.f, 0.f);
     int meta_i = 0;
     if (d < n) {
@@ -820,7 +834,7 @@
         if (a.rho_in) a.rho_out[d] = a.rho_in[i];
         if (a.orig_in) a.orig_out[d] = a.orig_in[i];
     }
-    block_prep_tile(c, n, p, meta_i, cell_start, blk_hdr, perm, blk_flag, cellw, s_cnt, s_c);
+    block_prep_tile(c, n, p, meta_i, cell_start, blk_hdr, perm, blk_flag, cellw, s_cnt, s_c, walk);
 }
 
 __global__ void __launch_bounds__(256)
@@ -932,6 +946,14 @@
     const int stop_now = stop_flag ? *stop_flag : 0;
     const int list_len = blk_list ? *blk_count : INT_MAX;
     const int b_listed = blk_list ? blk_list[blockIdx.x] : 0;
+    int t_first = 0, t_count = nblocks;
+    if constexpr (PassTileRange<P>::value) {
+        const int split = p.range.split ? *p.range.split : INT_MAX;
+        const int t_end = p.range.end > 0 ? (p.range.side == 1 && split < p.range.end ? split : p.range.end) : nblocks;
+        t_first = (p.range.side == 2 && split < p.range.first) ? split : p.range.first;
+        t_count = t_end - t_first;
+        if ((int)blockIdx.x >= t_count) return;
+    }
     if (stop_now) return;
     if ((int)blockIdx.x >= list_len) {
         if constexpr (PassPrologue<P>::value) { if (blockIdx.x == 0 && blockIdx.y == 0) p.prologue(scal); }
@@ -956,7 +978,7 @@
 
     const int tid = threadIdx.x;
     NBR_STAMP(0);
-    const int b = blk_list ? b_listed : xcd_remap(blockIdx.x, nblocks, c.xcd_chunk);
+    const int b = blk_list ? b_listed : t_first + xcd_remap(blockIdx.x, t_count, c.xcd_chunk);
     const int i0 = b * BLOCK;
     const int who_early = lane_perm ? (int)lane_perm[i0 + tid] : tid;
     const int *hdr = blk_hdr + (size_t)b * BLK_HDR_INTS;
diff --git a/sph_project_amd/csrc/sph_kernels.hip b/sph_project_amd/csrc/sph_kernels.hip
--- a/sph_project_amd/csrc/sph_kernels.hip
+++ b/sph_project_amd/csrc/sph_kernels.hip
@@ -9,6 +9,7 @@
 #endif
 
 #include <vector>
+#include <hip/hip_ext.h>
 #include <cstdio>
 #include <cstdint>
 namespace SPH_NS {
@@ -115,7 +116,7 @@
     return s.color.cur();
 }
 
-SortCarry l_scatter_impl(State &s, bool stable, bool rho_dead, bool density_next) {
+SortCarry l_scatter_impl(State &s, bool stable, bool rho_dead, bool density_next, int walk_cut = 0) {
     const int n = s.c.n;
     SortCarry carry;
     if (n == 0) return carry;
@@ -144,12 +145,22 @@
             carry.pid_in = a.pid_in; carry.pid_out = a.pid_out;
             a.velm_in = nullptr; a.meta_in = nullptr; a.pid_in = nullptr;
         }
+        WalkPlanOut walk;
+        if (carry.on && walk_cut > 0 && walk_cut <= cdiv(n, 256) && s.walk_first) {
+            const int bank = (int)(s.walk_seq++ & 1u);
+            walk = WalkPlanOut{s.walk_first + bank, s.walk_first + (1 - bank), walk_cut, walk_cut * 256};
+            carry.walk_cut = walk_cut; carry.walk_first = walk.first;
+        }
         hipLaunchKernelGGL(k_sort_rank, dim3(cdiv(n, 256)), dim3(256), 0, s.stream, n, s.cellid, s.cell_start,
                            RunList{s.run_head, s.run_rec, s.cap, s.sort_epoch}, s.sort_inv);
         const bool lst = !s.c.all_fluid && s.blk_list;
+        unsigned *const cellw = reinterpret_cast<unsigned *>(s.blk_hdr + (size_t)((s.cap + 255) / 256) * BLK_HDR_INTS);
+        if (walk.first)
+            hipExtLaunchKernelGGL(k_gather_prep, dim3(cdiv(n, 256)), dim3(256), 0, s.stream, nullptr, s.walk_ev[0], 0, s.c, n, (const int *)s.sort_inv, a,
+                                  (const int *)s.cell_start, s.blk_hdr, s.lane_perm, lst ? s.blk_flag : (int *)nullptr, cellw, walk);
+        else
         hipLaunchKernelGGL(k_gather_prep, dim3(cdiv(n, 256)), dim3(256), 0, s.stream, s.c, n, s.sort_inv, a, s.cell_start,
-                           s.blk_hdr, s.lane_perm, lst ? s.blk_flag : nullptr,
-                           reinterpret_cast<unsigned *>(s.blk_hdr + (size_t)((s.cap + 255) / 256) * BLK_HDR_INTS));
+                           s.blk_hdr, s.lane_perm, lst ? s.blk_flag : nullptr, cellw, walk);
         s.n_list_sorts++;
     } else if (stable) {
         hipLaunchKernelGGL(k_scatter_index, dim3(cdiv(n, 256)), dim3(256), 0, s.stream, n, s.cellid, s.rank,
@@ -177,7 +188,7 @@
     return carry;
 }
 void l_scatter(State &s) { l_scatter_impl(s, false, false, false); }
-SortCarry l_scatter_stable(State &s, bool rho_dead, bool density_next) { return l_scatter_impl(s, true, rho_dead, density_next); }
+SortCarry l_scatter_stable(State &s, bool rho_dead, bool density_next, int walk_cut) { return l_scatter_impl(s, true, rho_dead, density_next, walk_cut); }
 
 int list_grid(State &s, int nb) {
     if (!s.list_count_pinned) return nb;
@@ -190,7 +201,8 @@
     return g < 1 ? 1 : (g > nb ? nb : g);
 }
 
-template <class P> void launch_pass(State &s, const P &p, int mask_mode = 0, int tiles = 0, int split = 0) {
+template <class P> void launch_pass(State &s, const P &p, int mask_mode = 0, int tiles = 0, int split = 0, int grid = 0, hipStream_t stream = nullptr,
+                                    hipEvent_t done = nullptr) {
     const int n = s.c.n;
     if (n == 0) return;
     const int nb = cdiv(n, P::BLOCK);
@@ -208,13 +220,18 @@
         else skip = s.tile_class;
     }
     if (use_list) nb_launch = list_grid(s, nb);
+    if (grid > 0) nb_launch = grid;
+    if (!stream) stream = s.stream;
     if (P::HAS_REDUCE) s.last_pass_listed = use_list ? 1 : 0;
     unsigned long long *tl = (s.c.force_global == 20 && (size_t)nb * 16 * 8 <= (size_t)s.cap * 4) ? (unsigned long long *)s.tmp_idx : nullptr;
     if (tl) hipMemsetAsync(tl, 0, (size_t)nb * 16 * 8, s.stream);
     constexpr int MODES = PassModes<P>::value;
     if (!(MODES & (1 << mask_mode))) mask_mode = 0;
     const int gy = (PassSplit<P>::value && split) ? split : 1;
-#define SPH_LAUNCH_NBR(M) hipLaunchKernelGGL((k_nbr_pass<P, M>), dim3(nb_launch, gy), dim3(P::BLOCK), 0, s.stream, s.c, s.cell_start, p, s.scal, nb, s.nbr_mask, s.nbr_mask_hi, s.cap, s.blk_hdr, perm, tl, s.loop_flag, bl, bc, skip)
+#define SPH_NBR_ARGS s.c, (const int *)s.cell_start, p, s.scal, nb, s.nbr_mask, s.nbr_mask_hi, s.cap, (const int *)s.blk_hdr, perm, tl, s.loop_flag, bl, bc, skip
+#define SPH_LAUNCH_NBR(M) do { \
+        if (done) hipExtLaunchKernelGGL((k_nbr_pass<P, M>), dim3(nb_launch, gy), dim3(P::BLOCK), 0, stream, nullptr, done, 0, SPH_NBR_ARGS); \
+        else hipLaunchKernelGGL((k_nbr_pass<P, M>), dim3(nb_launch, gy), dim3(P::BLOCK), 0, stream, SPH_NBR_ARGS); } while (0)
     if (mask_mode == 1) {
         if constexpr ((MODES & 0b010) != 0) { SPH_LAUNCH_NBR(1); s.masks_valid = 1; }
     } else if (mask_mode == 2) {
@@ -223,6 +240,7 @@
         SPH_LAUNCH_NBR(0);
     }
 #undef SPH_LAUNCH_NBR
+#undef SPH_NBR_ARGS
     if (tl) {
         static int shown = 0;
         hipStreamSynchronize(s.stream);
@@ -257,7 +275,14 @@
     if (getenv("SPH_TEST_DROP_CARRY")) carry.on = 0;
 #endif
     if (carry.on) s.n_carried_sorts++;
-    if (s.c.all_fluid) {
+    const int nt = cdiv(s.c.n, 256);
+    if (s.c.all_fluid && eos && o.walk.cut > 0 && o.walk.cut <= nt && o.walk.side && o.tiles == 0) {
+        DensityPass<true, true> p{{carry}, s.posv.cur(), s.meta.cur(), s.rho_raw, s.rho.cur(), s.prs, s.ptm, fs, sp, se};
+        p.range = TileRange{0, o.walk.cut, nullptr, 0};
+        launch_pass(s, p, 1, 0, 0, o.walk.cut, nullptr, o.walk.done[0]);
+        p.range = TileRange{o.walk.cut, nt, nullptr, 0};
+        if (nt > o.walk.cut) launch_pass(s, p, 1, 0, 0, nt - o.walk.cut, o.walk.side);
+    } else if (s.c.all_fluid) {
         if (eos) { DensityPass<true, true> p{{carry}, s.posv.cur(), s.meta.cur(), s.rho_raw, s.rho.cur(), s.prs, s.ptm, fs, sp, se}; launch_pass(s, p, 1, o.tiles); }
         else { DensityPass<true, false> p{{carry}, s.posv.cur(), s.meta.cur(), s.rho_raw, s.rho.cur(), s.prs, s.ptm, fs, sp, se}; launch_pass(s, p, 1, o.tiles); }
     } else {
@@ -323,6 +348,25 @@
     NextHash nh{0, s.cellid, s.rank, s.cell_count, tile_sum_bank(s), RunList{nullptr, nullptr, 0, 0u}};
     if (o.hash_next && s.c.all_fluid && !s.slab_active && s.cell_count_clean && o.booked_by_density && s.c.n > 0) nh.on = 1;
     if (nh.on) nh.rl = run_list_of(s, true);
+    const int nt = cdiv(s.c.n, 256);
+    const bool walk = o.walk.cut > 0 && o.walk.cut <= nt && o.walk.side && o.walk.first && o.vel_out && o.booked_by_density &&
+                      s.c.all_fluid && !s.slab_active;
+    float4 *const vel_out = walk ? o.vel_out : s.velm.alt();
+    auto launch_forces = [&](auto &p) {
+        if (!walk) { launch_pass(s, p, 2); return; }
+        if constexpr (std::is_same<decltype(p.range), TileRange>::value) {
+            p.range = TileRange{0, o.walk.cut, o.walk.first, 1};
+            launch_pass(s, p, 2, 0, 0, o.walk.cut, nullptr, o.walk.mirror ? nullptr : o.walk.done[0]);
+            p.range = TileRange{o.walk.cut, nt, o.walk.first, 2};
+            const int reserve = o.walk.reserve < 0 ? 0 : (o.walk.reserve > o.walk.cut ? o.walk.cut : o.walk.reserve);
+            const int grid2 = nt - o.walk.cut + reserve;
+            launch_pass(s, p, 2, 0, 0, grid2 > 0 ? grid2 : 1, o.walk.side, o.walk.done[1]);
+            if (o.walk.mirror && o.walk.done[0])
+                hipExtLaunchKernelGGL(k_walk_publish, dim3(1), dim3(64), 0, s.stream, nullptr, o.walk.done[0], 0, o.walk.first, o.walk.cut, reserve, o.walk.mirror, o.walk.seq);
+            else if (o.walk.mirror)
+                hipLaunchKernelGGL(k_walk_publish, dim3(1), dim3(64), 0, s.stream, o.walk.first, o.walk.cut, reserve, o.walk.mirror, o.walk.seq);
+        }
+    };
     if (!o.booked_by_density) {
         if (s.c.all_fluid) {
             WcsphForcePass<true, false, true> p{s.posv.cur(), s.velm.cur(), s.meta.cur(), s.rho_raw, s.ptm, s.prs, s.rho.cur(), s.velm.alt(), s.acc, s.posv.alt(), s.scal, s.pose, s.c.rho0, s.presend, nh};
@@ -334,20 +378,21 @@
     } else
 #if SPH_FAST
     if (s.c.all_fluid && s.uniform_mass && !s.slab_active) {
-        WcsphForcePass<true, true> p{s.posv.cur(), s.velm.cur(), s.meta.cur(), s.rho_raw, s.ptm, s.prs, s.rho.cur(), s.velm.alt(), s.acc, s.posv.alt(), s.scal, s.pose, s.c.rho0, s.presend, nh};
-        launch_pass(s, p, 2);
+        WcsphForcePass<true, true> p{s.posv.cur(), s.velm.cur(), s.meta.cur(), s.rho_raw, s.ptm, s.prs, s.rho.cur(), vel_out, s.acc, s.posv.alt(), s.scal, s.pose, s.c.rho0, s.presend, nh};
+        launch_forces(p);
     } else
 #endif
     if (s.c.all_fluid) {
-        WcsphForcePass<true> p{s.posv.cur(), s.velm.cur(), s.meta.cur(), s.rho_raw, s.ptm, s.prs, s.rho.cur(), s.velm.alt(), s.acc, s.posv.alt(), s.scal, s.pose, s.c.rho0, s.presend, nh};
-        launch_pass(s, p, 2);
+        WcsphForcePass<true> p{s.posv.cur(), s.velm.cur(), s.meta.cur(), s.rho_raw, s.ptm, s.prs, s.rho.cur(), vel_out, s.acc, s.posv.alt(), s.scal, s.pose, s.c.rho0, s.presend, nh};
+        launch_forces(p);
     } else {
         WcsphForcePass<false> p{s.posv.cur(), s.velm.cur(), s.meta.cur(), s.rho_raw, s.ptm, s.prs, s.rho.cur(), s.velm.alt(), s.acc, s.posv.alt(), s.scal, s.pose, s.c.rho0, s.presend, nh};
         launch_pass(s, p, 2);
     }
     if (s.presend.on) { s.presend.on = 0; s.preclassified = 1; }
     if (nh.on) { s.prehashed = 1; s.cell_count_clean = 0; s.tile_sums_ready = nh.tile_sum != nullptr; s.hist_taken = 1; s.run_lists_filed = nh.rl.head != nullptr; }
-    s.velm.flip();
+    if (walk) { s.velm_third = s.velm.b[s.velm.c]; s.velm.b[s.velm.c] = vel_out; }
+    else s.velm.flip();
     s.posv.flip();
     s.masks_valid = 0;
     if (s.has_emitter && s.c.n > 0)
diff --git a/sph_project_amd/csrc/sph_passes.hpp b/sph_project_amd/csrc/sph_passes.hpp
--- a/sph_project_amd/csrc/sph_passes.hpp
+++ b/sph_project_amd/csrc/sph_passes.hpp
@@ -49,6 +49,8 @@
     static constexpr bool STAT_W = true;
     int stat_pairs, stat_evals;
     static constexpr bool SORT_CARRY = AF;
+    static constexpr bool TILE_RANGE = AF;
+    typename std::conditional<AF, TileRange, NoTileRange>::type range;
 
     __device__ float4 loadA(int j) const { return posv[j]; }
     __device__ BT loadB(int) const { return 0; }
@@ -409,6 +411,8 @@
     float4 *vel_out, *acc, *posv_out; DevScalars *scal; const RigidPose *pose; float rho0;
     HaloSend hs;
     NextHash nh;
+    static constexpr bool TILE_RANGE = AF;
+    typename std::conditional<AF, TileRange, NoTileRange>::type range;
     __device__ int cell_of(const Consts &c, float x, float y, float z) const {
         return (cell_coord_x(c, x) * c.ny + cell_coord(y, c.grid_size, c.ny)) * c.nz + cell_coord_z(c, z);
     }
diff --git a/sph_project_amd/csrc/sph_steps.hpp b/sph_project_amd/csrc/sph_steps.hpp
--- a/sph_project_amd/csrc/sph_steps.hpp
+++ b/sph_project_amd/csrc/sph_steps.hpp
@@ -151,10 +151,56 @@
     State &s = h->st;
     const bool fused = !h->prm.viscosity_implicit;
     SortCarry carry;
+    const bool books = fused && !getenv("SPH_FORCES_COUNT_OWN");
+    int walk_cut = 0;
+    if (h->walk_frac > 0.0f && fused && books && !s.slab_active && s.c.all_fluid && !s.has_emitter && !h->any_rigid_object && !s.has_rigid &&
+        s.c.force_global == 0) {
+        const int nt = (s.c.n + 255) / 256;
+        if (nt >= h->walk_min_tiles) walk_cut = std::min(nt, std::max(1, (int)(h->walk_frac * (float)nt + 0.5f)));
+        if (walk_cut > 0) { int rc = walk_ensure(h); if (rc) return rc; }
+    }
     if (s.slab_active) { int rc = slab_neighbor_search(h, fused); if (rc) return rc; }
-    else carry = ph_neighbor_search(h, true, true);
+    else carry = ph_neighbor_search(h, true, true, walk_cut);
     ph_rigid_volume(h);
-    const bool books = fused && !getenv("SPH_FORCES_COUNT_OWN");
+    if (carry.on && carry.walk_cut > 0) {
+        WalkOverlap walk{carry.walk_cut, carry.walk_first, s.walk_stream};
+        float4 *const force_vel_out = s.velm_third;
+        walk.seq = ++s.walk_pub_seq;
+        if (walk.seq > SPH_WALK_MAX_LAG) {
+            const unsigned want = walk.seq - SPH_WALK_MAX_LAG;
+            const volatile unsigned *pub = reinterpret_cast<const volatile unsigned *>(s.walk_mirror + 2);
+            for (unsigned spins = 0; (int)(__atomic_load_n(pub, __ATOMIC_ACQUIRE) - want) < 0; ++spins) {
+                if ((spins & 4095u) == 4095u) {
+                    const hipError_t q0 = hipStreamQuery(s.stream), q1 = hipStreamQuery(s.walk_stream);
+                    if (hipPeekAtLastError() == hipErrorNotReady) (void)hipGetLastError();
+                    if (q0 != hipErrorNotReady && q1 != hipErrorNotReady) break;
+                }
+                __builtin_ia32_pause();
+            }
+        }
+        const int seen = __atomic_load_n(s.walk_mirror, __ATOMIC_RELAXED);
+        walk.reserve = seen < 0 ? carry.walk_cut : seen + seen / 4 + 64;
+        if (h->walk_reserve_forced >= 0) walk.reserve = h->walk_reserve_forced;
+        walk.reserve = std::min(walk.reserve, carry.walk_cut);
+        walk.mirror = s.walk_mirror;
+        h->walk_grid2 = (s.c.n + 255) / 256 - carry.walk_cut + walk.reserve; h->walk_cut_last = carry.walk_cut;
+#ifdef SPH_TEST_HOOKS
+        hipMemsetAsync(force_vel_out, 0xFF, sizeof(float4) * (size_t)s.c.n, s.stream);
+        HIPCHK(h, hipEventRecord(s.walk_ev[0], s.stream));
+#endif
+        HIPCHK(h, hipStreamWaitEvent(s.walk_stream, s.walk_ev[0], 0));
+        walk.done[0] = s.walk_ev[1];
+        { ProfScope p(h, SPH_K_DENSITY), p2(h, SPH_K_DENSITY, s.walk_stream); h->L->density(s, 1, {0, books, carry, walk}); }
+        HIPCHK(h, hipStreamWaitEvent(s.walk_stream, s.walk_ev[1], 0));
+        const bool hash_next = h->steps_to_follow > 0 && !h->sort_dirty;
+        const bool hand_over = h->steps_to_follow > 0;
+        walk.done[0] = hand_over ? s.walk_ev[2] : nullptr;
+        walk.done[1] = hand_over ? nullptr : s.walk_ev[2];
+        { ProfScope p(h, SPH_K_WCSPH_FORCES), p2(h, SPH_K_WCSPH_FORCES, s.walk_stream); h->L->wcsph_forces(s, {books, hash_next, walk, force_vel_out}); }
+        HIPCHK(h, hipStreamWaitEvent(hand_over ? s.walk_stream : s.stream, s.walk_ev[2], 0));
+        if (hand_over) std::swap(s.stream, s.walk_stream);
+        return SPH_OK;
+    }
     const bool overlap = s.slab_active && s.push.on && s.tile_list[0] && s.c.all_fluid && s.tile_plan_n == s.c.n && (s.has_down || s.has_up);
     if (overlap) {
         const int hint = slab_field_hint(h);
```

Result: slower. 5.121 billion (-2.2%).
